# santi-pdp/segan_pytorch

Measured on AMD Instinct MI355X. Metric: 16384-sample waveform chunks/sec (GAN step), higher is better.
Workload: dtype f32

## Files before the change

include/segan_hip.h:

```cpp
#ifndef SEGAN_HIP_H
#define SEGAN_HIP_H

#include <stddef.h>
#include <stdint.h>

#ifdef __cplusplus
extern "C" {
#endif

#define SEGAN_ABI_VERSION 15

#define SEGAN_PAD_REFLECT 0
#define SEGAN_PAD_ZERO 1

#define SEGAN_ACT_NONE 0
#define SEGAN_ACT_TANH 1

typedef struct segan_src {
  const float* p0;
  const float* p1;
  int32_t C0;
  int32_t C1;
  const float* scale;
  const float* shift;
  const float* slope;
} segan_src;

int segan_abi_version(void);
const char* segan_last_error(void);

int segan_set_reserved_slots(int n);

size_t segan_packed_f_bytes(int M, int N, int S);
size_t segan_packed_t_bytes(int M, int N, int S);

int segan_pack_weights(const float* w, float* wf, float* wt, int M, int N, int K, int S,
                       int pad_t, void* stream);

#define SEGAN_PREC_FP32 0
#define SEGAN_PREC_BF16 1
#define SEGAN_PREC_BF16X3 3
#define SEGAN_PREC_FP32_BLOCKED 4
size_t segan_packed_bf_bytes(int M, int N, int S, int tform, int planes);
int segan_pack_weights_bf(const float* w, void* out, int M, int N, int K, int S, int tform,
                          int pad_t, int planes, void* stream);

size_t segan_bf16_scratch_bytes(int op, int B, int N, int M, int L, int K, int S, int pad, int planes);
size_t segan_corr_scratch_bytes(void);
void segan_debug_last_corr(int* out6);
void segan_debug_last_wgrad(int* out6);

int segan_conv1d_fwd(const segan_src* x, const void* wf, const float* bias, float* out, int B,
                     int N, int M, int L, int K, int S, int padL, int mode, int roll,
                     int precision, void* scratch, size_t scratch_bytes, void* stream);

int segan_conv1d_dgrad(const float* da, const void* wt, const float* w, float* dx, float* halo,
                       int B, int N, int M, int L, int K, int S, int padL, int roll, int precision,
                       void* scratch, size_t scratch_bytes, void* stream);

#define SEGAN_WGRAD_DETERMINISTIC 1
size_t segan_wgrad_scratch_bytes(int B, int M, int N, int Ls, int S, int precision, int flags);
int segan_wgrad(const segan_src* lo, const segan_src* hi, float* dw, int B, int M, int N, int Ls,
                int K, int S, int padL, int mode, int roll, int precision, int flags, void* scratch,
                size_t scratch_bytes, void* stream);

int segan_deconv1d_fwd(const segan_src* x, const void* wt, const float* w, const float* bias,
                       float* y, int B, int M, int N, int Ls, int K, int S, int pad, int act,
                       int precision, void* scratch, size_t scratch_bytes, void* stream);

int segan_deconv1d_dgrad(const float* dy, const void* wf, float* dx0, float* dx1, int B, int M,
                         int M0, int N, int Ls, int K, int S, int pad, int precision, void* scratch,
                         size_t scratch_bytes, void* stream);


int segan_bn_nsplit(int B, int C, int L);
int segan_bn_stats(const float* x, const float* gamma, const float* beta, float eps,
                   float momentum, float* running_mean, float* running_var, float* mean,
                   float* rstd, float* scale, float* shift, float* ws, int B, int C, int L,
                   void* stream);
int segan_bn_partial(const float* x, float* ws, int B, int C, int L, void* stream);
int segan_bn_final(const float* ws, int nsplit_total, const float* gamma, const float* beta,
                   float eps, float momentum, float* running_mean, float* running_var, float* mean,
                   float* rstd, float* scale, float* shift, int C, void* stream);

int segan_affine_tanh(const float* x, const float* scale, const float* shift, float* y, int B,
                      int C, int L, void* stream);
int segan_scale_mask(const float* x, const float* scale, const float* mask, float* y, int B, int C,
                     int L, void* stream);

int segan_affine_prelu(const float* x, const float* scale, const float* shift, const float* slope,
                       float* y, int B, int C, int L, void* stream);

int segan_sum_skip(const float* x0, const float* slope0, const float* x1, const float* alpha,
                   float* out, int B, int C, int L, void* stream);

int segan_act_bwd(const float* a, const float* dh, const float* dskip, const float* slope,
                  const float* alpha, const float* bn_mean, const float* bn_rstd,
                  const float* bn_gamma, const float* bn_beta, float* da, float* dslope,
                  float* dalpha, float* dgamma, float* dbeta, float* dbias, float* ws, int B, int C,
                  int L, void* stream);
int segan_act_bwd_bn_reduce(const float* a, const float* dh, const float* slope,
                            const float* bn_mean, const float* bn_rstd, const float* bn_gamma,
                            const float* bn_beta, float* dslope, float* dgamma, float* dbeta,
                            float* totals, float* ws, int B, int C, int L, void* stream);
int segan_act_bwd_bn_apply(const float* a, const float* dh, const float* slope,
                           const float* bn_mean, const float* bn_rstd, const float* bn_gamma,
                           const float* bn_beta, const float* totals, float* da, float* dbias,
                           float* ws, int B, int C, int L, double count_total, void* stream);

int segan_tanh_bwd(const float* y, const float* dy, const float* clean, float l1_scale, float* da,
                   float* dbias, float* ws, int B, int C, int L, void* stream);


#define SEGAN_GEMM_DETERMINISTIC 1
size_t segan_gemm_scratch_bytes(int M, int N, int K);
int segan_gemm(const float* A, int64_t sam, int64_t sak, const float* B, int64_t sbk, int64_t sbn,
               float* C, int64_t ldc, int M, int N, int K, int beta0, int flags, void* scratch,
               size_t scratch_bytes, void* stream);

int segan_bias_prelu_rows(const float* x, const float* bias, const float* slope, float* y,
                          int rows, int cols, void* stream);
int segan_bias_prelu_rows_bwd(const float* x, const float* bias, const float* slope,
                              const float* dy, float* dx, float* dslope, float* dbias, int rows,
                              int cols, void* stream);

int segan_mse_const(const float* x, float target, float* loss, float* grad, const float* gout,
                    float gscale, int n, void* stream);
int segan_bce_logits_const(const float* x, float target, float* loss, float* grad,
                           const float* gout, float gscale, int n, void* stream);
int segan_l1_mean(const float* x, const float* y, float* loss, float* ws, int64_t n,
                  void* stream);
int segan_l1_bwd(const float* x, const float* y, const float* gout, float gscale, float* grad,
                 int64_t n, void* stream);

size_t segan_packed_g_bytes(int M, int N, int S);
int segan_pack_weights_g(const float* w, float* wg, int M, int N, int K, int S, void* stream);
int segan_conv1d_dgrad_short(const float* da, const float* wg, float* dx, int B, int N, int M,
                             int L, int K, int S, int padL, int roll, void* stream);

int segan_pool_time_fwd(const float* x, float* y, int* idx, int rows, int L, int mode,
                        void* stream);
int segan_pool_time_bwd(const float* dy, const int* idx, float* dx, int rows, int L, int mode,
                        void* stream);

int segan_mse_mean(const float* x, const float* y, float* loss, float* ws, int64_t n,
                   void* stream);
int segan_mse_bwd(const float* x, const float* y, const float* gout, float gscale, float* grad,
                  int64_t n, void* stream);

size_t segan_snorm_ws_floats(int A, int Bd, int K, int dim);
int segan_snorm_fwd(const float* w, float* u, float* v, float* w_sn, float* sigma, float* ws, int A,
                    int Bd, int K, int dim, int power_iteration, float eps, void* stream);
int segan_snorm_bwd(const float* dw_sn, const float* w, const float* u, const float* v,
                    const float* sigma, float* dw, float* ws, int A, int Bd, int K, int dim,
                    void* stream);

int segan_stft_pitch(int n_fft);
int segan_stft_basis(float* basis, int n_fft, int win, void* stream);
int segan_stft_frames(const float* x, float* frames, int B, int T, int n_fft, int hop, int win,
                      void* stream);
int segan_powdb(const float* S, float* db, int64_t rows, int nbins, int pitch, float eps,
                void* stream);
int segan_powdb_bwd(const float* S, const float* ddb, float* dS, int64_t rows, int nbins, int pitch,
                    float eps, void* stream);
int segan_stft_overlap_add(const float* dframes, float* dx, int B, int T, int n_fft, int hop,
                           int win, void* stream);

int segan_pcm16_prep(const int16_t* pcm, const unsigned char* first, float* clean, float* noisy,
                     int B, int T, double coef, void* stream);

int segan_deemphasis(const float* y, float* x, int rows, int T, double coef, void* stream);
int segan_ssnr_frames(int T, int srate);
int segan_ssnr(const float* ref, const float* deg, float* seg, float* out, int rows, int T,
               int srate, double eps, void* stream);
int segan_wss(const float* ref, const float* deg, double* dist, int rows, int T, int srate,
              void* stream);
int segan_llr(const float* ref, const float* deg, double* dist, int rows, int T, int srate,
              void* stream);
int segan_stoi_plan(int srate, int* pq, int* ntaps, double* taps, int cap, int* bands);
int segan_stoi_dims(int T, int srate, int* dims);
int segan_stoi(const float* ref, const float* deg, const int* lengths, int rows, int T, int srate,
               double* xr, double* yr, double* energy, int* mask, int* kept, int* count,
               double* xs, double* ys, double* X, double* Y, double* rho, double* d, void* stream);

int segan_rmsprop_step(float* p, const float* g, float* sq, float lr, float alpha, float eps,
                       int64_t n, void* stream);
int segan_adam_step(float* p, const float* g, float* m, float* v, float lr, float beta1,
                    float beta2, float eps, int step, int64_t n, void* stream);
int segan_fill(float* p, float value, int64_t n, void* stream);
int segan_scale(float* p, float s, int64_t n, void* stream);

int segan_comm_id_bytes(void);
int segan_comm_unique_id(void* id_out);
int segan_comm_init(void** comm_out, int world, int rank, const void* id);
int segan_comm_destroy(void* comm);
int segan_comm_rank(void* comm);
int segan_comm_world(void* comm);
int segan_allreduce(void* comm, float* buf, size_t n, float scale, void* stream);
int segan_broadcast(void* comm, float* buf, size_t n, int root, void* stream);
int segan_allgather(void* comm, const float* send, float* recv, size_t n, void* stream);

#ifdef __cplusplus
}
#endif
#endif
```

segan_pytorch_amd/_lib.py:

```python
import ctypes
import os
from ctypes import POINTER, Structure, c_char_p, c_double, c_float, c_int, c_int32, c_int64, c_size_t, c_void_p

_HERE = os.path.dirname(os.path.abspath(__file__))
LIB_PATH = os.environ.get('SEGAN_HIP_LIB') or os.path.join(_HERE, 'libsegan_hip.so')

PAD_REFLECT = 0
PAD_ZERO = 1
ACT_NONE = 0
ACT_TANH = 1
ABI_VERSION = 15


class SeganSrc(Structure):
    _fields_ = [('p0', c_void_p), ('p1', c_void_p), ('C0', c_int32), ('C1', c_int32),
                ('scale', c_void_p), ('shift', c_void_p), ('slope', c_void_p)]


_P = c_void_p
_SRC = POINTER(SeganSrc)

SIGNATURES = {
    'segan_abi_version': (c_int, []),
    'segan_set_reserved_slots': (c_int, [c_int]),
    'segan_last_error': (c_char_p, []),
    'segan_packed_f_bytes': (c_size_t, [c_int, c_int, c_int]),
    'segan_packed_t_bytes': (c_size_t, [c_int, c_int, c_int]),
    'segan_pack_weights': (c_int, [_P, _P, _P, c_int, c_int, c_int, c_int, c_int, _P]),
    'segan_packed_bf_bytes': (c_size_t, [c_int, c_int, c_int, c_int, c_int]),
    'segan_pack_weights_bf': (c_int, [_P, _P, c_int, c_int, c_int, c_int, c_int, c_int, c_int, _P]),
    'segan_corr_scratch_bytes': (c_size_t, []),
    'segan_bf16_scratch_bytes': (c_size_t, [c_int] * 9),
    'segan_debug_last_corr': (None, [POINTER(c_int)]),
    'segan_debug_last_wgrad': (None, [POINTER(c_int)]),
    'segan_conv1d_fwd': (c_int, [_SRC, _P, _P, _P, c_int, c_int, c_int, c_int, c_int, c_int, c_int,
                                 c_int, c_int, c_int, _P, c_size_t, _P]),
    'segan_conv1d_dgrad': (c_int, [_P, _P, _P, _P, _P, c_int, c_int, c_int, c_int, c_int, c_int, c_int,
                                   c_int, c_int, _P, c_size_t, _P]),
    'segan_wgrad': (c_int, [_SRC, _SRC, _P, c_int, c_int, c_int, c_int, c_int, c_int, c_int, c_int,
                            c_int, c_int, c_int, _P, c_size_t, _P]),
    'segan_wgrad_scratch_bytes': (c_size_t, [c_int, c_int, c_int, c_int, c_int, c_int, c_int]),
    'segan_deconv1d_fwd': (c_int, [_SRC, _P, _P, _P, _P, c_int, c_int, c_int, c_int, c_int, c_int, c_int,
                                   c_int, c_int, _P, c_size_t, _P]),
    'segan_deconv1d_dgrad': (c_int, [_P, _P, _P, _P, c_int, c_int, c_int, c_int, c_int, c_int, c_int,
                                     c_int, c_int, _P, c_size_t, _P]),
    'segan_bn_nsplit': (c_int, [c_int, c_int, c_int]),
    'segan_bn_stats': (c_int, [_P, _P, _P, c_float, c_float, _P, _P, _P, _P, _P, _P, _P, c_int, c_int,
                               c_int, _P]),
    'segan_bn_partial': (c_int, [_P, _P, c_int, c_int, c_int, _P]),
    'segan_bn_final': (c_int, [_P, c_int, _P, _P, c_float, c_float, _P, _P, _P, _P, _P, _P, c_int, _P]),
    'segan_act_bwd_bn_reduce': (c_int, [_P] * 12 + [c_int, c_int, c_int, _P]),
    'segan_act_bwd_bn_apply': (c_int, [_P] * 11 + [c_int, c_int, c_int, c_double, _P]),
    'segan_affine_prelu': (c_int, [_P, _P, _P, _P, _P, c_int, c_int, c_int, _P]),
    'segan_affine_tanh': (c_int, [_P, _P, _P, _P, c_int, c_int, c_int, _P]),
    'segan_scale_mask': (c_int, [_P, _P, _P, _P, c_int, c_int, c_int, _P]),
    'segan_sum_skip': (c_int, [_P, _P, _P, _P, _P, c_int, c_int, c_int, _P]),
    'segan_bce_logits_const': (c_int, [_P, c_float, _P, _P, _P, c_float, c_int, _P]),
    'segan_act_bwd': (c_int, [_P] * 16 + [c_int, c_int, c_int, _P]),
    'segan_tanh_bwd': (c_int, [_P, _P, _P, c_float, _P, _P, _P, c_int, c_int, c_int, _P]),
    'segan_gemm_scratch_bytes': (c_size_t, [c_int, c_int, c_int]),
    'segan_gemm': (c_int, [_P, c_int64, c_int64, _P, c_int64, c_int64, _P, c_int64, c_int, c_int,
                           c_int, c_int, c_int, _P, c_size_t, _P]),
    'segan_bias_prelu_rows': (c_int, [_P, _P, _P, _P, c_int, c_int, _P]),
    'segan_bias_prelu_rows_bwd': (c_int, [_P, _P, _P, _P, _P, _P, _P, c_int, c_int, _P]),
    'segan_mse_const': (c_int, [_P, c_float, _P, _P, _P, c_float, c_int, _P]),
    'segan_l1_bwd': (c_int, [_P, _P, _P, c_float, _P, c_int64, _P]),
    'segan_l1_mean': (c_int, [_P, _P, _P, _P, c_int64, _P]),
    'segan_packed_g_bytes': (c_size_t, [c_int, c_int, c_int]),
    'segan_pack_weights_g': (c_int, [_P, _P, c_int, c_int, c_int, c_int, _P]),
    'segan_conv1d_dgrad_short': (c_int, [_P, _P, _P, c_int, c_int, c_int, c_int, c_int, c_int, c_int,
                                        c_int, _P]),
    'segan_pool_time_fwd': (c_int, [_P, _P, _P, c_int, c_int, c_int, _P]),
    'segan_pool_time_bwd': (c_int, [_P, _P, _P, c_int, c_int, c_int, _P]),
    'segan_mse_mean': (c_int, [_P, _P, _P, _P, c_int64, _P]),
    'segan_mse_bwd': (c_int, [_P, _P, _P, c_float, _P, c_int64, _P]),
    'segan_snorm_ws_floats': (c_size_t, [c_int, c_int, c_int, c_int]),
    'segan_snorm_fwd': (c_int, [_P, _P, _P, _P, _P, _P, c_int, c_int, c_int, c_int, c_int, c_float, _P]),
    'segan_snorm_bwd': (c_int, [_P, _P, _P, _P, _P, _P, _P, c_int, c_int, c_int, c_int, _P]),
    'segan_pcm16_prep': (c_int, [_P, _P, _P, _P, c_int, c_int, c_double, _P]),
    'segan_stft_basis': (c_int, [_P, c_int, c_int, _P]),
    'segan_stft_frames': (c_int, [_P, _P, c_int, c_int, c_int, c_int, c_int, _P]),
    'segan_stft_pitch': (c_int, [c_int]),
    'segan_powdb': (c_int, [_P, _P, c_int64, c_int, c_int, c_float, _P]),
    'segan_powdb_bwd': (c_int, [_P, _P, _P, c_int64, c_int, c_int, c_float, _P]),
    'segan_stft_overlap_add': (c_int, [_P, _P, c_int, c_int, c_int, c_int, c_int, _P]),
    'segan_deemphasis': (c_int, [_P, _P, c_int, c_int, c_double, _P]),
    'segan_ssnr_frames': (c_int, [c_int, c_int]),
    'segan_ssnr': (c_int, [_P, _P, _P, _P, c_int, c_int, c_int, c_double, _P]),
    'segan_wss': (c_int, [_P, _P, _P, c_int, c_int, c_int, _P]),
    'segan_llr': (c_int, [_P, _P, _P, c_int, c_int, c_int, _P]),
    'segan_stoi_plan': (c_int, [c_int, POINTER(c_int), POINTER(c_int), _P, c_int, POINTER(c_int)]),
    'segan_stoi_dims': (c_int, [c_int, c_int, POINTER(c_int)]),
    'segan_stoi': (c_int, [_P, _P, _P, c_int, c_int, c_int] + [_P] * 13),
    'segan_rmsprop_step': (c_int, [_P, _P, _P, c_float, c_float, c_float, c_int64, _P]),
    'segan_adam_step': (c_int, [_P, _P, _P, _P, c_float, c_float, c_float, c_float, c_int, c_int64,
                                _P]),
    'segan_fill': (c_int, [_P, c_float, c_int64, _P]),
    'segan_scale': (c_int, [_P, c_float, c_int64, _P]),
    'segan_comm_id_bytes': (c_int, []),
    'segan_comm_unique_id': (c_int, [_P]),
    'segan_comm_init': (c_int, [POINTER(c_void_p), c_int, c_int, _P]),
    'segan_comm_destroy': (c_int, [_P]),
    'segan_comm_rank': (c_int, [_P]),
    'segan_comm_world': (c_int, [_P]),
    'segan_allreduce': (c_int, [_P, _P, c_size_t, c_float, _P]),
    'segan_broadcast': (c_int, [_P, _P, c_size_t, c_int, _P]),
    'segan_allgather': (c_int, [_P, _P, _P, c_size_t, _P]),
}

_lib = None


def load():
    global _lib
    if _lib is not None:
        return _lib
    if not os.path.exists(LIB_PATH):
        raise RuntimeError(
            'segan_pytorch_amd: {} not found. Build it with `make` (or '
            '`python -c "import __graft_entry__ as g; g.build()"`) at the repo root. '
            'There is no non-HIP fallback.'.format(LIB_PATH))
    try:
        import torch
        if torch.cuda.is_available():
            torch.cuda.init()
    except ImportError:
        pass
    lib = ctypes.CDLL(LIB_PATH)
    for name, (res, args) in SIGNATURES.items():
        fn = getattr(lib, name)
        fn.restype = res
        fn.argtypes = args
    ver = lib.segan_abi_version()
    if ver != ABI_VERSION:
        raise RuntimeError('libsegan_hip ABI {} != expected {}'.format(ver, ABI_VERSION))
    _lib = lib
    return lib


def check(rc, what=''):
    if rc != 0:
        msg = load().segan_last_error()
        raise RuntimeError('libsegan_hip {} failed ({}): {}'.format(
            what, rc, msg.decode() if msg else '?'))
```

segan_pytorch_amd/csrc/segan_pack.hip:

```cpp
#include "segan_conv_shared.h"

__global__ __launch_bounds__(256) void pack_f_kernel(const float* __restrict__ w,
                                                     float* __restrict__ wf, int M, int N, int K,
                                                     int S, int U, int pitch, int rows, int pair) {
  __shared__ float t[64][33];
  const int n = blockIdx.y;
  const int m0 = blockIdx.x * 64;
  const int tid = threadIdx.x;
  {
    float v[8];
#pragma unroll
    for (int i = 0; i < 8; ++i) {
      const int e = tid + 256 * i;
      const int ml = e >> 5, k = e & 31;
      const int m = m0 + ml;
      v[i] = (m < M && n < N && k < K) ? w[((size_t)m * N + n) * K + k] : 0.0f;
    }
#pragma unroll
    for (int i = 0; i < 8; ++i) {
      const int e = tid + 256 * i;
      t[e >> 5][e & 31] = v[i];
    }
  }
  __syncthreads();
  if (pair && (n & 1) && n < N && tid < 64) {
    const int m = m0 + tid;
    t[tid][31] = m < M ? w[((size_t)m * N + n - 1) * K + (31 - S)] : 0.0f;
  }
  __syncthreads();
  for (int e = tid; e < 32 * 64; e += 256) {
    const int kk = e >> 6, ml = e & 63;
    const int r = kk / U, u = kk - r * U;
    const int row = (n * S + r) * U + u;
    if (row < rows && m0 + ml < pitch) wf[(size_t)row * pitch + m0 + ml] = t[ml][S * u + r];
  }
}

__global__ __launch_bounds__(256) void pack_t_kernel(const float* __restrict__ w,
                                                     float* __restrict__ wt, int M, int N, int K,
                                                     int S, int U, int NP, int pad, int pitch,
                                                     int rows) {
  __shared__ float t[64][33];
  const int m = blockIdx.y;
  const int n0 = blockIdx.x * 64;
  const int tid = threadIdx.x;
  {
    float v[8];
#pragma unroll
    for (int i = 0; i < 8; ++i) {
      const int e = tid + 256 * i;
      const int nl = e >> 5, k = e & 31;
      const int n = n0 + nl;
      v[i] = (m < M && n < N && k < K) ? w[((size_t)m * N + n) * K + k] : 0.0f;
    }
#pragma unroll
    for (int i = 0; i < 8; ++i) {
      const int e = tid + 256 * i;
      t[e >> 5][e & 31] = v[i];
    }
  }
  __syncthreads();
  for (int e = tid; e < 32 * 64; e += 256) {
    const int kk = e >> 6, nl = e & 63;
    const int up = kk / S, r = kk - up * S;
    const int rho = (r + pad) % S;
    const int k = S * (U - 1 - up) + rho;
    const int row = m * U + up;
    const int n = n0 + nl;
    if (row < rows && n < NP) wt[(size_t)row * pitch + r * NP + n] = t[nl][k];
  }
}

extern "C" size_t segan_packed_f_bytes(int M, int N, int S) {
  if (!stride_ok(S) || M <= 0 || N <= 0) return 0;
  return (size_t)f_rows(N) * f_pitch(M) * sizeof(float);
}
extern "C" size_t segan_packed_t_bytes(int M, int N, int S) {
  if (!stride_ok(S) || M <= 0 || N <= 0) return 0;
  return (size_t)t_rows(M, S) * t_pitch(N, S) * sizeof(float);
}

extern "C" int segan_pack_weights(const float* w, float* wf, float* wt, int M, int N, int K, int S,
                                  int pad_t, void* stream) {
  SEGAN_REQUIRE(w != nullptr, "pack_weights: w is NULL");
  SEGAN_REQUIRE(stride_ok(S), "pack_weights: stride %d not in {1,2,4}", S);
  SEGAN_REQUIRE(K >= 1 && K <= 32, "pack_weights: kernel width %d not in [1,32]", K);
  SEGAN_REQUIRE(M > 0 && N > 0, "pack_weights: bad channel counts %d,%d", M, N);
  SEGAN_REQUIRE(pad_t >= 0, "pack_weights: negative padding");
  hipStream_t st = (hipStream_t)stream;
  const int U = 32 / S;
  if (wf) {
    const int pitch = f_pitch(M), rows = f_rows(N);
    hipLaunchKernelGGL(pack_f_kernel, dim3(pitch / 64, ceil_div(rows, 32)), dim3(256), 0, st, w,
                       wf, M, N, K, S, U, pitch, rows, f_pair(N, K));
  }
  if (wt) {
    const int NP = t_np(N, S);
    const int pitch = t_pitch(N, S), rows = t_rows(M, S);
    hipLaunchKernelGGL(pack_t_kernel, dim3(ceil_div(NP, 64), ceil_div(rows, U)), dim3(256), 0, st,
                       w, wt, M, N, K, S, U, NP, pad_t, pitch, rows);
  }
  return segan_check_launch("pack_weights");
}
```

segan_pytorch_amd/csrc/segan_pointwise.hip:

```cpp
#include "segan_common.h"

#define PW_THREADS 256

static int pw_nsplit(int B, int C, int L) {
  int ns = ceil_div(2048, C);
  if (ns > B) ns = B;
  long per = (long)B * L / ns;
  while (ns > 1 && per < 2048) {
    ns = (ns + 1) / 2;
    per = (long)B * L / ns;
  }
  return ns < 1 ? 1 : ns;
}

extern "C" int segan_bn_nsplit(int B, int C, int L) {
  if (B <= 0 || C <= 0 || L <= 0) return 0;
  return pw_nsplit(B, C, L);
}

template <int NV>
__device__ __forceinline__ void block_sum(float (&v)[NV], float* sm) {
  const int lane = threadIdx.x & 63, wave = threadIdx.x >> 6;
#pragma unroll
  for (int k = 0; k < NV; ++k) v[k] = warp_sum(v[k]);
  if (lane == 0)
#pragma unroll
    for (int k = 0; k < NV; ++k) sm[wave * NV + k] = v[k];
  __syncthreads();
  if (threadIdx.x == 0) {
#pragma unroll
    for (int k = 0; k < NV; ++k) {
      float s = 0.f;
      for (int w = 0; w < PW_THREADS / 64; ++w) s += sm[w * NV + k];
      v[k] = s;
    }
  }
  __syncthreads();
}

struct ChanRange {
  int c, b_beg, b_end;
};
__device__ __forceinline__ ChanRange chan_range(int B, int nsplit) {
  ChanRange r;
  r.c = blockIdx.x;
  const int per = (B + nsplit - 1) / nsplit;
  r.b_beg = blockIdx.y * per;
  r.b_end = min(B, r.b_beg + per);
  return r;
}

__device__ __forceinline__ void chan_combine(float& n, float& mean, float& m2, float nb, float mb,
                                             float qb) {
  const float tot = n + nb;
  if (tot <= 0.0f) return;
  const float d = mb - mean;
  const float f = nb / tot;
  mean = fmaf(d, f, mean);
  m2 = m2 + qb + d * d * n * f;
  n = tot;
}

__global__ void bn_partial_kernel(const float* __restrict__ x, float* __restrict__ ws, int B, int C,
                                  int L, int nsplit) {
  __shared__ float sm[3 * (PW_THREADS / 64)];
  const ChanRange cr = chan_range(B, nsplit);
  const int nb = cr.b_end - cr.b_beg;
  const float* base = x + ((size_t)cr.b_beg * C + cr.c) * L;
  const size_t sstride = (size_t)C * L;
  const bool vec = (L & 3) == 0 && ((uintptr_t)x & 15) == 0;
  const int Lv = vec ? L >> 2 : L;
  int tr = PW_THREADS;
  while (tr > Lv && tr > 1) tr >>= 1;
  const int rp = PW_THREADS / tr;
  const int t0 = threadIdx.x % tr, r0 = threadIdx.x / tr;
  float K = 0.0f, s1 = 0.0f, s2 = 0.0f, n = 0.0f;
  if (r0 < nb && t0 < Lv) K = base[(size_t)r0 * sstride + (vec ? 4 * t0 : t0)];
  for (int b = r0; b < nb; b += rp) {
    const float* row = base + b * sstride;
    if (vec) {
      for (int t = t0; t < Lv; t += tr) {
        const f32x4 u = *reinterpret_cast<const f32x4*>(row + 4 * t);
#pragma unroll
        for (int e = 0; e < 4; ++e) {
          const float d = u[e] - K;
          s1 += d;
          s2 = fmaf(d, d, s2);
        }
        n += 4.0f;
      }
    } else {
      for (int t = t0; t < Lv; t += tr) {
        const float d = row[t] - K;
        s1 += d;
        s2 = fmaf(d, d, s2);
        n += 1.0f;
      }
    }
  }
  float mean = 0.0f, m2 = 0.0f;
  if (n > 0.0f) {
    const float r = s1 / n;
    mean = K + r;
    m2 = fmaxf(s2 - s1 * r, 0.0f);
  }
#pragma unroll
  for (int o = 32; o > 0; o >>= 1) {
    const float nb2 = __shfl_down(n, o, 64), mb2 = __shfl_down(mean, o, 64), qb2 = __shfl_down(m2, o, 64);
    chan_combine(n, mean, m2, nb2, mb2, qb2);
  }
  const int lane = threadIdx.x & 63, wave = threadIdx.x >> 6;
  if (lane == 0) {
    sm[3 * wave] = n; sm[3 * wave + 1] = mean; sm[3 * wave + 2] = m2;
  }
  __syncthreads();
  if (threadIdx.x == 0) {
    for (int w = 1; w < PW_THREADS / 64; ++w) chan_combine(n, mean, m2, sm[3 * w], sm[3 * w + 1], sm[3 * w + 2]);
    float* w = ws + ((size_t)blockIdx.y * C + cr.c) * 3;
    w[0] = n;
    w[1] = mean;
    w[2] = m2;
  }
}

__device__ __forceinline__ void bn_affine(float gamma, float beta, float mean, float rstd,
                                          float& scale, float& shift) {
  scale = gamma * rstd;
  shift = fmaf(-mean, scale, beta);
}

__global__ void bn_final_kernel(const float* __restrict__ ws, const float* gamma, const float* beta,
                                float eps, float momentum, float* running_mean, float* running_var,
                                float* mean_o, float* rstd_o, float* scale_o, float* shift_o, int C,
                                int nsplit) {
  const int c = blockIdx.x * blockDim.x + threadIdx.x;
  if (c >= C) return;
  double n = 0.0, mean = 0.0, m2 = 0.0;
  for (int s = 0; s < nsplit; ++s) {
    const float* w = ws + ((size_t)s * C + c) * 3;
    const double nb = w[0], mb = w[1], qb = w[2];
    if (nb <= 0.0) continue;
    const double tot = n + nb;
    const double d = mb - mean;
    mean += d * nb / tot;
    m2 += qb + d * d * n * nb / tot;
    n = tot;
  }
  const double var = n > 0 ? m2 / n : 0.0;
  const float rstd = (float)(1.0 / sqrt(var + (double)eps));
  const float g = gamma ? gamma[c] : 1.0f;
  const float bt = beta ? beta[c] : 0.0f;
  float sc, sh;
  bn_affine(g, bt, (float)mean, rstd, sc, sh);
  if (mean_o) mean_o[c] = (float)mean;
  if (rstd_o) rstd_o[c] = rstd;
  if (scale_o) scale_o[c] = sc;
  if (shift_o) shift_o[c] = sh;
  if (running_mean) running_mean[c] = (1.0f - momentum) * running_mean[c] + momentum * (float)mean;
  if (running_var) {
    const double unb = n > 1 ? m2 / (n - 1.0) : var;
    running_var[c] = (1.0f - momentum) * running_var[c] + momentum * (float)unb;
  }
}

extern "C" int segan_bn_stats(const float* x, const float* gamma, const float* beta, float eps,
                              float momentum, float* running_mean, float* running_var, float* mean,
                              float* rstd, float* scale, float* shift, float* ws, int B, int C,
                              int L, void* stream) {
  SEGAN_REQUIRE(x && ws, "bn_stats: NULL pointer");
  SEGAN_REQUIRE(B > 0 && C > 0 && L > 0, "bn_stats: bad sizes");
  hipStream_t st = (hipStream_t)stream;
  const int ns = pw_nsplit(B, C, L);
  hipLaunchKernelGGL(bn_partial_kernel, dim3(C, ns), dim3(PW_THREADS), 0, st, x, ws, B, C, L, ns);
  hipLaunchKernelGGL(bn_final_kernel, dim3(ceil_div(C, 64)), dim3(64), 0, st, ws, gamma, beta, eps,
                     momentum, running_mean, running_var, mean, rstd, scale, shift, C, ns);
  return segan_check_launch("bn_stats");
}

extern "C" int segan_bn_partial(const float* x, float* ws, int B, int C, int L, void* stream) {
  SEGAN_REQUIRE(x && ws, "bn_partial: NULL pointer");
  SEGAN_REQUIRE(B > 0 && C > 0 && L > 0, "bn_partial: bad sizes");
  const int ns = pw_nsplit(B, C, L);
  hipLaunchKernelGGL(bn_partial_kernel, dim3(C, ns), dim3(PW_THREADS), 0, (hipStream_t)stream, x, ws,
                     B, C, L, ns);
  return segan_check_launch("bn_partial");
}

extern "C" int segan_bn_final(const float* ws, int nsplit_total, const float* gamma,
                              const float* beta, float eps, float momentum, float* running_mean,
                              float* running_var, float* mean, float* rstd, float* scale,
                              float* shift, int C, void* stream) {
  SEGAN_REQUIRE(ws && nsplit_total > 0 && C > 0, "bn_final: bad arguments");
  hipLaunchKernelGGL(bn_final_kernel, dim3(ceil_div(C, 64)), dim3(64), 0, (hipStream_t)stream, ws,
                     gamma, beta, eps, momentum, running_mean, running_var, mean, rstd, scale, shift,
                     C, nsplit_total);
  return segan_check_launch("bn_final");
}

__global__ void affine_prelu_kernel(const float* __restrict__ x, const float* scale,
                                    const float* shift, const float* slope, float* __restrict__ y,
                                    size_t total, int C, int L) {
  for (size_t i = blockIdx.x * (size_t)blockDim.x + threadIdx.x; i < total;
       i += (size_t)gridDim.x * blockDim.x) {
    const int c = (int)((i / L) % C);
    float v = x[i];
    v = fmaf(v, scale ? scale[c] : 1.0f, shift ? shift[c] : 0.0f);
    if (slope) v = v > 0.f ? v : v * slope[c];
    y[i] = v;
  }
}

extern "C" int segan_affine_prelu(const float* x, const float* scale, const float* shift,
                                  const float* slope, float* y, int B, int C, int L, void* stream) {
  SEGAN_REQUIRE(x && y, "affine_prelu: NULL pointer");
  SEGAN_REQUIRE(B > 0 && C > 0 && L > 0, "affine_prelu: bad sizes");
  const size_t total = (size_t)B * C * L;
  const int blocks = (int)((total + 255) / 256 > 4096 ? 4096 : (total + 255) / 256);
  hipLaunchKernelGGL(affine_prelu_kernel, dim3(blocks), dim3(256), 0, (hipStream_t)stream, x, scale,
                     shift, slope, y, total, C, L);
  return segan_check_launch("affine_prelu");
}

__global__ void affine_tanh_kernel(const float* __restrict__ x, const float* scale,
                                   const float* shift, float* __restrict__ y, size_t total, int C,
                                   int L) {
  for (size_t i = blockIdx.x * (size_t)blockDim.x + threadIdx.x; i < total;
       i += (size_t)gridDim.x * blockDim.x) {
    const int c = (int)((i / L) % C);
    y[i] = tanhf(fmaf(x[i], scale ? scale[c] : 1.0f, shift ? shift[c] : 0.0f));
  }
}

extern "C" int segan_affine_tanh(const float* x, const float* scale, const float* shift, float* y,
                                 int B, int C, int L, void* stream) {
  SEGAN_REQUIRE(x && y, "affine_tanh: NULL pointer");
  SEGAN_REQUIRE(B > 0 && C > 0 && L > 0, "affine_tanh: bad sizes");
  const size_t total = (size_t)B * C * L;
  const int blocks = (int)((total + 255) / 256 > 4096 ? 4096 : (total + 255) / 256);
  hipLaunchKernelGGL(affine_tanh_kernel, dim3(blocks), dim3(256), 0, (hipStream_t)stream, x, scale,
                     shift, y, total, C, L);
  return segan_check_launch("affine_tanh");
}

__global__ void scale_mask_kernel(const float* __restrict__ x, const float* scale,
                                  const float* __restrict__ mask, float* __restrict__ y,
                                  size_t total, int C, int L) {
  for (size_t i = blockIdx.x * (size_t)blockDim.x + threadIdx.x; i < total;
       i += (size_t)gridDim.x * blockDim.x) {
    const int c = (int)((i / L) % C);
    y[i] = x[i] * (scale ? scale[c] : 1.0f) * mask[i];
  }
}

extern "C" int segan_scale_mask(const float* x, const float* scale, const float* mask, float* y,
                                int B, int C, int L, void* stream) {
  SEGAN_REQUIRE(x && mask && y, "scale_mask: NULL pointer");
  SEGAN_REQUIRE(B > 0 && C > 0 && L > 0, "scale_mask: bad sizes");
  const size_t total = (size_t)B * C * L;
  const int blocks = (int)((total + 255) / 256 > 4096 ? 4096 : (total + 255) / 256);
  hipLaunchKernelGGL(scale_mask_kernel, dim3(blocks), dim3(256), 0, (hipStream_t)stream, x, scale,
                     mask, y, total, C, L);
  return segan_check_launch("scale_mask");
}

__global__ void sum_skip_kernel(const float* __restrict__ x0, const float* slope0,
                                const float* __restrict__ x1, const float* alpha,
                                float* __restrict__ out, size_t total, int C, int L) {
  for (size_t i = blockIdx.x * (size_t)blockDim.x + threadIdx.x; i < total;
       i += (size_t)gridDim.x * blockDim.x) {
    const int c = (int)((i / L) % C);
    float v = x0[i];
    if (slope0) v = v > 0.f ? v : v * slope0[c];
    out[i] = fmaf(alpha[c], x1[i], v);
  }
}

extern "C" int segan_sum_skip(const float* x0, const float* slope0, const float* x1,
                              const float* alpha, float* out, int B, int C, int L, void* stream) {
  SEGAN_REQUIRE(x0 && x1 && alpha && out, "sum_skip: NULL pointer");
  SEGAN_REQUIRE(B > 0 && C > 0 && L > 0, "sum_skip: bad sizes");
  const size_t total = (size_t)B * C * L;
  const int blocks = (int)((total + 255) / 256 > 4096 ? 4096 : (total + 255) / 256);
  hipLaunchKernelGGL(sum_skip_kernel, dim3(blocks), dim3(256), 0, (hipStream_t)stream, x0, slope0,
                     x1, alpha, out, total, C, L);
  return segan_check_launch("sum_skip");
}

struct ActBwdArgs {
  const float* a;
  const float* dh;
  const float* dskip;
  const float* slope;
  const float* alpha;
  const float* mean;
  const float* rstd;
  const float* gamma;
  const float* beta;
  float* da;
  float* ws;
  int B, C, L, nsplit;
  float inv_count;
};

template <int PHASE>
__global__ void act_bwd_kernel(const ActBwdArgs p) {
  __shared__ float sm[16];
  const ChanRange cr = chan_range(p.B, p.nsplit);
  const int c = cr.c;
  const int nb = cr.b_end - cr.b_beg;
  const float sl = p.slope ? p.slope[c] : 1.0f;
  const float al = p.alpha ? p.alpha[c] : 0.0f;
  float mu = 0.f, rs = 1.f, ga = 1.f, be = 0.f, dbeta_m = 0.f, dgamma_m = 0.f, sc = 1.f, sh = 0.f;
  if (PHASE != 0) {
    mu = p.mean[c];
    rs = p.rstd[c];
    ga = p.gamma ? p.gamma[c] : 1.0f;
    be = p.beta ? p.beta[c] : 0.0f;
    bn_affine(ga, be, mu, rs, sc, sh);
  }
  if (PHASE == 2) {
    const float* tot = p.ws + (size_t)p.nsplit * p.C * 4 + (size_t)c * 2;
    dbeta_m = tot[0] * p.inv_count;
    dgamma_m = tot[1] * p.inv_count;
  }
  float r[3] = {0.f, 0.f, 0.f};
  const bool has_skip = p.dskip != nullptr;
  auto elem = [&](float av, float dh, float ds) -> float {
    if (PHASE == 0) {
      float g = dh * (av > 0.f ? 1.0f : sl);
      r[0] += dh * (av > 0.f ? 0.0f : av);
      if (has_skip) {
        g = fmaf(al, ds, g);
        r[1] = fmaf(ds, av, r[1]);
      }
      r[2] += g;
      return g;
    }
    const float xh = (av - mu) * rs;
    const float v = fmaf(av, sc, sh);
    const float g = dh * (v > 0.f ? 1.0f : sl);
    if (PHASE == 1) {
      r[0] += dh * (v > 0.f ? 0.0f : v);
      r[1] += g;
      r[2] = fmaf(g, xh, r[2]);
      return 0.0f;
    }
    const float d = ga * rs * (g - dbeta_m - xh * dgamma_m);
    r[0] += d;
    return d;
  };
  const size_t base = ((size_t)cr.b_beg * p.C + c) * p.L;
  const size_t sstride = (size_t)p.C * p.L;
  const bool vec = (p.L & 3) == 0 &&
                   (((uintptr_t)p.a | (uintptr_t)p.dh | (uintptr_t)p.dskip | (uintptr_t)p.da) & 15) == 0;
  const int Lv = vec ? p.L >> 2 : p.L;
  int tr = PW_THREADS;
  while (tr > Lv && tr > 1) tr >>= 1;
  const int rp = PW_THREADS / tr;
  const int t0 = threadIdx.x % tr, r0 = threadIdx.x / tr;
  const f32x4 z4 = {0.f, 0.f, 0.f, 0.f};
  for (int b = r0; b < nb; b += rp) {
    const size_t ro = base + b * sstride;
    if (vec) {
      for (int t = t0; t < Lv; t += tr) {
        const size_t i = ro + 4 * (size_t)t;
        const f32x4 av = *reinterpret_cast<const f32x4*>(p.a + i);
        const f32x4 dh = p.dh ? *reinterpret_cast<const f32x4*>(p.dh + i) : z4;
        const f32x4 ds = has_skip ? *reinterpret_cast<const f32x4*>(p.dskip + i) : z4;
        f32x4 o;
#pragma unroll
        for (int e = 0; e < 4; ++e) o[e] = elem(av[e], dh[e], ds[e]);
        if (PHASE != 1) *reinterpret_cast<f32x4*>(p.da + i) = o;
      }
    } else {
      for (int t = t0; t < Lv; t += tr) {
        const size_t i = ro + t;
        const float o = elem(p.a[i], p.dh ? p.dh[i] : 0.0f, has_skip ? p.dskip[i] : 0.0f);
        if (PHASE != 1) p.da[i] = o;
      }
    }
  }
  block_sum<3>(r, sm);
  if (threadIdx.x == 0) {
    float* w = p.ws + ((size_t)blockIdx.y * p.C + c) * 4;
    w[0] = r[0];
    w[1] = r[1];
    w[2] = r[2];
  }
}

template <int PHASE>
__global__ void act_bwd_final_kernel(const ActBwdArgs p, float* dslope, float* dalpha,
                                     float* dgamma, float* dbeta, float* dbias) {
  const int c = blockIdx.x * blockDim.x + threadIdx.x;
  if (c >= p.C) return;
  float s0 = 0.f, s1 = 0.f, s2 = 0.f;
  for (int s = 0; s < p.nsplit; ++s) {
    const float* w = p.ws + ((size_t)s * p.C + c) * 4;
    s0 += w[0];
    s1 += w[1];
    s2 += w[2];
  }
  if (PHASE == 0) {
    if (dslope) dslope[c] += s0;
    if (dalpha) dalpha[c] += s1;
    if (dbias) dbias[c] += s2;
  } else if (PHASE == 1) {
    if (dslope) dslope[c] += s0;
    if (dbeta) dbeta[c] += s1;
    if (dgamma) dgamma[c] += s2;
    float* tot = p.ws + (size_t)p.nsplit * p.C * 4 + (size_t)c * 2;
    tot[0] = s1;
    tot[1] = s2;
  } else {
    if (dbias) dbias[c] += s0;
  }
}

extern "C" int segan_act_bwd(const float* a, const float* dh, const float* dskip,
                             const float* slope, const float* alpha, const float* bn_mean,
                             const float* bn_rstd, const float* bn_gamma, const float* bn_beta,
                             float* da, float* dslope, float* dalpha, float* dgamma, float* dbeta,
                             float* dbias, float* ws, int B, int C, int L, void* stream) {
  SEGAN_REQUIRE(a && da && ws, "act_bwd: NULL pointer");
  SEGAN_REQUIRE(dh || dskip, "act_bwd: no incoming gradient");
  SEGAN_REQUIRE(B > 0 && C > 0 && L > 0, "act_bwd: bad sizes");
  SEGAN_REQUIRE((bn_mean == nullptr) == (bn_rstd == nullptr), "act_bwd: mean/rstd must pair");
  SEGAN_REQUIRE(!(dskip && !alpha), "act_bwd: dskip needs alpha");
  SEGAN_REQUIRE(!(bn_mean && dskip), "act_bwd: BN layers have no skip tap");
  hipStream_t st = (hipStream_t)stream;
  ActBwdArgs p;
  p.a = a; p.dh = dh; p.dskip = dskip; p.slope = slope; p.alpha = alpha;
  p.mean = bn_mean; p.rstd = bn_rstd; p.gamma = bn_gamma; p.beta = bn_beta;
  p.da = da; p.ws = ws; p.B = B; p.C = C; p.L = L;
  p.nsplit = pw_nsplit(B, C, L);
  p.inv_count = 1.0f / ((float)B * (float)L);
  const dim3 grid(C, p.nsplit), fgrid(ceil_div(C, 64));
  if (!bn_mean) {
    hipLaunchKernelGGL(act_bwd_kernel<0>, grid, dim3(PW_THREADS), 0, st, p);
    hipLaunchKernelGGL(act_bwd_final_kernel<0>, fgrid, dim3(64), 0, st, p, dslope, dalpha, dgamma,
                       dbeta, dbias);
  } else {
    hipLaunchKernelGGL(act_bwd_kernel<1>, grid, dim3(PW_THREADS), 0, st, p);
    hipLaunchKernelGGL(act_bwd_final_kernel<1>, fgrid, dim3(64), 0, st, p, dslope, dalpha, dgamma,
                       dbeta, dbias);
    hipLaunchKernelGGL(act_bwd_kernel<2>, grid, dim3(PW_THREADS), 0, st, p);
    hipLaunchKernelGGL(act_bwd_final_kernel<2>, fgrid, dim3(64), 0, st, p, dslope, dalpha, dgamma,
                       dbeta, dbias);
  }
  return segan_check_launch("act_bwd");
}

extern "C" int segan_act_bwd_bn_reduce(const float* a, const float* dh, const float* slope,
                                       const float* bn_mean, const float* bn_rstd,
                                       const float* bn_gamma, const float* bn_beta, float* dslope,
                                       float* dgamma, float* dbeta, float* totals, float* ws, int B,
                                       int C, int L, void* stream) {
  SEGAN_REQUIRE(a && dh && bn_mean && bn_rstd && totals && ws, "act_bwd_bn_reduce: NULL pointer");
  SEGAN_REQUIRE(B > 0 && C > 0 && L > 0, "act_bwd_bn_reduce: bad sizes");
  hipStream_t st = (hipStream_t)stream;
  ActBwdArgs p;
  p.a = a; p.dh = dh; p.dskip = nullptr; p.slope = slope; p.alpha = nullptr;
  p.mean = bn_mean; p.rstd = bn_rstd; p.gamma = bn_gamma; p.beta = bn_beta;
  p.da = nullptr; p.ws = ws; p.B = B; p.C = C; p.L = L;
  p.nsplit = pw_nsplit(B, C, L);
  p.inv_count = 1.0f / ((float)B * (float)L);
  hipLaunchKernelGGL(act_bwd_kernel<1>, dim3(C, p.nsplit), dim3(PW_THREADS), 0, st, p);
  hipLaunchKernelGGL(act_bwd_final_kernel<1>, dim3(ceil_div(C, 64)), dim3(64), 0, st, p, dslope,
                     (float*)nullptr, dgamma, dbeta, (float*)nullptr);
  if (hipMemcpyAsync(totals, ws + (size_t)p.nsplit * C * 4, (size_t)C * 2 * sizeof(float),
                     hipMemcpyDeviceToDevice, st) != hipSuccess) {
    segan_set_error("act_bwd_bn_reduce: copy of the totals failed");
    return SEGAN_ELAUNCH;
  }
  return segan_check_launch("act_bwd_bn_reduce");
}

extern "C" int segan_act_bwd_bn_apply(const float* a, const float* dh, const float* slope,
                                      const float* bn_mean, const float* bn_rstd,
                                      const float* bn_gamma, const float* bn_beta,
                                      const float* totals, float* da, float* dbias, float* ws, int B,
                                      int C, int L, double count_total, void* stream) {
  SEGAN_REQUIRE(a && dh && bn_mean && bn_rstd && totals && da && ws, "act_bwd_bn_apply: NULL pointer");
  SEGAN_REQUIRE(B > 0 && C > 0 && L > 0 && count_total >= (double)B * L, "act_bwd_bn_apply: bad sizes");
  hipStream_t st = (hipStream_t)stream;
  ActBwdArgs p;
  p.a = a; p.dh = dh; p.dskip = nullptr; p.slope = slope; p.alpha = nullptr;
  p.mean = bn_mean; p.rstd = bn_rstd; p.gamma = bn_gamma; p.beta = bn_beta;
  p.da = da; p.ws = ws; p.B = B; p.C = C; p.L = L;
  p.nsplit = pw_nsplit(B, C, L);
  p.inv_count = (float)(1.0 / count_total);
  if (hipMemcpyAsync(ws + (size_t)p.nsplit * C * 4, totals, (size_t)C * 2 * sizeof(float),
                     hipMemcpyDeviceToDevice, st) != hipSuccess) {
    segan_set_error("act_bwd_bn_apply: copy of the totals failed");
    return SEGAN_ELAUNCH;
  }
  hipLaunchKernelGGL(act_bwd_kernel<2>, dim3(C, p.nsplit), dim3(PW_THREADS), 0, st, p);
  hipLaunchKernelGGL(act_bwd_final_kernel<2>, dim3(ceil_div(C, 64)), dim3(64), 0, st, p,
                     (float*)nullptr, (float*)nullptr, (float*)nullptr, (float*)nullptr, dbias);
  return segan_check_launch("act_bwd_bn_apply");
}

__global__ void tanh_bwd_kernel(const float* __restrict__ y, const float* dy, const float* clean,
                                float l1_scale, float* __restrict__ da, float* ws, int B, int C,
                                int L, int nsplit) {
  __shared__ float sm[16];
  const ChanRange cr = chan_range(B, nsplit);
  const int nb = cr.b_end - cr.b_beg;
  const long cnt = (long)(nb > 0 ? nb : 0) * L;
  float r[1] = {0.f};
  for (long e = threadIdx.x; e < cnt; e += PW_THREADS) {
    const int b = cr.b_beg + (int)(e / L);
    const int t = (int)(e % L);
    const size_t i = ((size_t)b * C + cr.c) * L + t;
    const float yv = y[i];
    float g = dy ? dy[i] : 0.0f;
    if (clean) {
      const float d = yv - clean[i];
      g += l1_scale * (d > 0.f ? 1.0f : (d < 0.f ? -1.0f : 0.0f));
    }
    const float d = g * (1.0f - yv * yv);
    da[i] = d;
    r[0] += d;
  }
  block_sum<1>(r, sm);
  if (threadIdx.x == 0) ws[(size_t)blockIdx.y * C + cr.c] = r[0];
}

__global__ void sum_splits_add_kernel(const float* ws, float* out, int C, int nsplit) {
  const int c = blockIdx.x * blockDim.x + threadIdx.x;
  if (c >= C) return;
  float s = 0.f;
  for (int k = 0; k < nsplit; ++k) s += ws[(size_t)k * C + c];
  out[c] += s;
}

extern "C" int segan_tanh_bwd(const float* y, const float* dy, const float* clean, float l1_scale,
                              float* da, float* dbias, float* ws, int B, int C, int L,
                              void* stream) {
  SEGAN_REQUIRE(y && da && ws, "tanh_bwd: NULL pointer");
  SEGAN_REQUIRE(dy || clean, "tanh_bwd: no incoming gradient");
  SEGAN_REQUIRE(B > 0 && C > 0 && L > 0, "tanh_bwd: bad sizes");
  hipStream_t st = (hipStream_t)stream;
  const int ns = pw_nsplit(B, C, L);
  hipLaunchKernelGGL(tanh_bwd_kernel, dim3(C, ns), dim3(PW_THREADS), 0, st, y, dy, clean, l1_scale,
                     da, ws, B, C, L, ns);
  if (dbias)
    hipLaunchKernelGGL(sum_splits_add_kernel, dim3(ceil_div(C, 64)), dim3(64), 0, st, ws, dbias, C,
                       ns);
  return segan_check_launch("tanh_bwd");
}

__global__ void bias_prelu_rows_kernel(const float* __restrict__ x, const float* bias,
                                       const float* slope, float* __restrict__ y, int rows,
                                       int cols) {
  const size_t total = (size_t)rows * cols;
  for (size_t i = blockIdx.x * (size_t)blockDim.x + threadIdx.x; i < total;
       i += (size_t)gridDim.x * blockDim.x) {
    const int c = (int)(i % cols);
    float v = x[i] + (bias ? bias[c] : 0.0f);
    if (slope) v = v > 0.f ? v : v * slope[c];
    y[i] = v;
  }
}

extern "C" int segan_bias_prelu_rows(const float* x, const float* bias, const float* slope,
                                     float* y, int rows, int cols, void* stream) {
  SEGAN_REQUIRE(x && y && rows > 0 && cols > 0, "bias_prelu_rows: bad arguments");
  const size_t total = (size_t)rows * cols;
  const int blocks = (int)((total + 255) / 256 > 2048 ? 2048 : (total + 255) / 256);
  hipLaunchKernelGGL(bias_prelu_rows_kernel, dim3(blocks), dim3(256), 0, (hipStream_t)stream, x,
                     bias, slope, y, rows, cols);
  return segan_check_launch("bias_prelu_rows");
}

__global__ __launch_bounds__(256) void bias_prelu_rows_bwd_kernel(
    const float* __restrict__ x, const float* bias, const float* slope,
    const float* __restrict__ dy, float* __restrict__ dx, float* dslope, float* dbias, int rows,
    int cols) {
  __shared__ float sm[2][4][64];
  const int cl = threadIdx.x & 63, rg = threadIdx.x >> 6;
  const int c = blockIdx.x * 64 + cl;
  float s_sl = 0.f, s_b = 0.f;
  if (c < cols) {
    const float bs = bias ? bias[c] : 0.0f;
    const float sl = slope ? slope[c] : 1.0f;
    for (int r = rg; r < rows; r += 4) {
      const size_t i = (size_t)r * cols + c;
      const float v = x[i] + bs;
      const float g = dy[i];
      const float d = g * (v > 0.f ? 1.0f : sl);
      s_sl += g * (v > 0.f ? 0.0f : v);
      s_b += d;
      dx[i] = d;
    }
  }
  sm[0][rg][cl] = s_sl;
  sm[1][rg][cl] = s_b;
  __syncthreads();
  if (rg == 0 && c < cols) {
    const float a = sm[0][0][cl] + sm[0][1][cl] + sm[0][2][cl] + sm[0][3][cl];
    const float b = sm[1][0][cl] + sm[1][1][cl] + sm[1][2][cl] + sm[1][3][cl];
    if (dslope && slope) dslope[c] += a;
    if (dbias) dbias[c] += b;
  }
}

extern "C" int segan_bias_prelu_rows_bwd(const float* x, const float* bias, const float* slope,
                                         const float* dy, float* dx, float* dslope, float* dbias,
                                         int rows, int cols, void* stream) {
  SEGAN_REQUIRE(x && dy && dx && rows > 0 && cols > 0, "bias_prelu_rows_bwd: bad arguments");
  hipLaunchKernelGGL(bias_prelu_rows_bwd_kernel, dim3(ceil_div(cols, 64)), dim3(256), 0,
                     (hipStream_t)stream, x, bias, slope, dy, dx, dslope, dbias, rows, cols);
  return segan_check_launch("bias_prelu_rows_bwd");
}

__global__ void mse_const_kernel(const float* __restrict__ x, float target, float* loss,
                                 float* grad, const float* gout, float gscale, int n) {
  __shared__ float sm[16];
  float r[1] = {0.f};
  const float inv = 1.0f / (float)n;
  if (gout) gscale *= gout[0];
  for (int i = threadIdx.x; i < n; i += PW_THREADS) {
    const float d = x[i] - target;
    r[0] = fmaf(d, d, r[0]);
    if (grad) grad[i] = 2.0f * d * inv * gscale;
  }
  block_sum<1>(r, sm);
  if (threadIdx.x == 0 && loss) loss[0] = r[0] * inv;
}

extern "C" int segan_mse_const(const float* x, float target, float* loss, float* grad,
                               const float* gout, float gscale, int n, void* stream) {
  SEGAN_REQUIRE(x && n > 0 && (loss || grad), "mse_const: bad arguments");
  hipLaunchKernelGGL(mse_const_kernel, dim3(1), dim3(PW_THREADS), 0, (hipStream_t)stream, x, target,
                     loss, grad, gout, gscale, n);
  return segan_check_launch("mse_const");
}

__global__ void bce_const_kernel(const float* __restrict__ x, float target, float* loss,
                                 float* grad, const float* gout, float gscale, int n) {
  __shared__ float sm[16];
  float r[1] = {0.f};
  const float inv = 1.0f / (float)n;
  if (gout) gscale *= gout[0];
  for (int i = threadIdx.x; i < n; i += PW_THREADS) {
    const float v = x[i];
    r[0] += fmaxf(v, 0.f) - v * target + log1pf(expf(-fabsf(v)));
    if (grad) grad[i] = (1.0f / (1.0f + expf(-v)) - target) * inv * gscale;
  }
  block_sum<1>(r, sm);
  if (threadIdx.x == 0 && loss) loss[0] = r[0] * inv;
}

extern "C" int segan_bce_logits_const(const float* x, float target, float* loss, float* grad,
                                      const float* gout, float gscale, int n, void* stream) {
  SEGAN_REQUIRE(x && n > 0 && (loss || grad), "bce_logits_const: bad arguments");
  hipLaunchKernelGGL(bce_const_kernel, dim3(1), dim3(PW_THREADS), 0, (hipStream_t)stream, x, target,
                     loss, grad, gout, gscale, n);
  return segan_check_launch("bce_logits_const");
}

template <bool SQ>
__global__ void l1_partial_kernel(const float* __restrict__ x, const float* __restrict__ y,
                                  float* ws, size_t n) {
  __shared__ float sm[16];
  float r[1] = {0.f};
  for (size_t i = blockIdx.x * (size_t)blockDim.x + threadIdx.x; i < n;
       i += (size_t)gridDim.x * blockDim.x) {
    const float d = x[i] - y[i];
    r[0] += SQ ? d * d : fabsf(d);
  }
  block_sum<1>(r, sm);
  if (threadIdx.x == 0) ws[blockIdx.x] = r[0];
}
__global__ void l1_final_kernel(const float* ws, float* loss, int nblocks, float inv) {
  __shared__ float sm[16];
  float r[1] = {0.f};
  for (int i = threadIdx.x; i < nblocks; i += PW_THREADS) r[0] += ws[i];
  block_sum<1>(r, sm);
  if (threadIdx.x == 0) loss[0] = r[0] * inv;
}

extern "C" int segan_l1_mean(const float* x, const float* y, float* loss, float* ws, int64_t n,
                             void* stream) {
  SEGAN_REQUIRE(x && y && loss && ws && n > 0, "l1_mean: bad arguments");
  hipStream_t st = (hipStream_t)stream;
  int blocks = (int)((n + 255) / 256 > 1024 ? 1024 : (n + 255) / 256);
  hipLaunchKernelGGL(l1_partial_kernel<false>, dim3(blocks), dim3(PW_THREADS), 0, st, x, y, ws, (size_t)n);
  hipLaunchKernelGGL(l1_final_kernel, dim3(1), dim3(PW_THREADS), 0, st, ws, loss, blocks,
                     1.0f / (float)n);
  return segan_check_launch("l1_mean");
}

extern "C" int segan_mse_mean(const float* x, const float* y, float* loss, float* ws, int64_t n,
                              void* stream) {
  SEGAN_REQUIRE(x && y && loss && ws && n > 0, "mse_mean: bad arguments");
  hipStream_t st = (hipStream_t)stream;
  int blocks = (int)((n + 255) / 256 > 1024 ? 1024 : (n + 255) / 256);
  hipLaunchKernelGGL(l1_partial_kernel<true>, dim3(blocks), dim3(PW_THREADS), 0, st, x, y, ws, (size_t)n);
  hipLaunchKernelGGL(l1_final_kernel, dim3(1), dim3(PW_THREADS), 0, st, ws, loss, blocks,
                     1.0f / (float)n);
  return segan_check_launch("mse_mean");
}

__global__ void mse_bwd_kernel(const float* __restrict__ x, const float* __restrict__ y,
                               const float* gout, float gscale, float* __restrict__ grad, size_t n) {
  const float g = 2.0f * gscale * (gout ? gout[0] : 1.0f) / (float)n;
  for (size_t i = blockIdx.x * (size_t)blockDim.x + threadIdx.x; i < n;
       i += (size_t)gridDim.x * blockDim.x)
    grad[i] = g * (x[i] - y[i]);
}

extern "C" int segan_mse_bwd(const float* x, const float* y, const float* gout, float gscale,
                             float* grad, int64_t n, void* stream) {
  SEGAN_REQUIRE(x && y && grad && n > 0, "mse_bwd: bad arguments");
  int blocks = (int)((n + 255) / 256 > 4096 ? 4096 : (n + 255) / 256);
  hipLaunchKernelGGL(mse_bwd_kernel, dim3(blocks), dim3(256), 0, (hipStream_t)stream, x, y, gout,
                     gscale, grad, (size_t)n);
  return segan_check_launch("mse_bwd");
}

__global__ void l1_bwd_kernel(const float* __restrict__ x, const float* __restrict__ y,
                              const float* gout, float gscale, float* __restrict__ grad, size_t n) {
  const float g = gscale * (gout ? gout[0] : 1.0f) / (float)n;
  for (size_t i = blockIdx.x * (size_t)blockDim.x + threadIdx.x; i < n;
       i += (size_t)gridDim.x * blockDim.x) {
    const float d = x[i] - y[i];
    grad[i] = d > 0.f ? g : (d < 0.f ? -g : 0.0f);
  }
}

extern "C" int segan_l1_bwd(const float* x, const float* y, const float* gout, float gscale,
                            float* grad, int64_t n, void* stream) {
  SEGAN_REQUIRE(x && y && grad && n > 0, "l1_bwd: bad arguments");
  int blocks = (int)((n + 255) / 256 > 4096 ? 4096 : (n + 255) / 256);
  hipLaunchKernelGGL(l1_bwd_kernel, dim3(blocks), dim3(256), 0, (hipStream_t)stream, x, y, gout,
                     gscale, grad, (size_t)n);
  return segan_check_launch("l1_bwd");
}

__global__ void rmsprop_kernel(float* __restrict__ p, const float* __restrict__ g,
                               float* __restrict__ sq, float lr, float alpha, float eps, size_t n) {
  const size_t n4 = n / 4;
  float4* p4 = reinterpret_cast<float4*>(p);
  const float4* g4 = reinterpret_cast<const float4*>(g);
  float4* s4 = reinterpret_cast<float4*>(sq);
  const float oma = 1.0f - alpha;
  for (size_t i = blockIdx.x * (size_t)blockDim.x + threadIdx.x; i < n4;
       i += (size_t)gridDim.x * blockDim.x) {
    float4 pv = p4[i], gv = g4[i], sv = s4[i];
#define RMS1(f)                                       \
  sv.f = alpha * sv.f + oma * gv.f * gv.f;            \
  pv.f = pv.f - lr * (gv.f / (sqrtf(sv.f) + eps));
    RMS1(x) RMS1(y) RMS1(z) RMS1(w)
#undef RMS1
    p4[i] = pv;
    s4[i] = sv;
  }
  if (blockIdx.x == 0 && threadIdx.x < (n & 3)) {
    const size_t i = n4 * 4 + threadIdx.x;
    const float gv = g[i];
    const float sv = alpha * sq[i] + oma * gv * gv;
    sq[i] = sv;
    p[i] = p[i] - lr * (gv / (sqrtf(sv) + eps));
  }
}

extern "C" int segan_rmsprop_step(float* p, const float* g, float* sq, float lr, float alpha,
                                  float eps, int64_t n, void* stream) {
  SEGAN_REQUIRE(p && g && sq && n > 0, "rmsprop_step: bad arguments");
  SEGAN_REQUIRE(((uintptr_t)p % 16 == 0) && ((uintptr_t)g % 16 == 0) && ((uintptr_t)sq % 16 == 0),
                "rmsprop_step: arenas must be 16-byte aligned");
  int blocks = (int)((n / 4 + 255) / 256 > 2048 ? 2048 : (n / 4 + 255) / 256);
  if (blocks < 1) blocks = 1;
  hipLaunchKernelGGL(rmsprop_kernel, dim3(blocks), dim3(256), 0, (hipStream_t)stream, p, g, sq, lr,
                     alpha, eps, (size_t)n);
  return segan_check_launch("rmsprop_step");
}

__global__ void adam_kernel(float* __restrict__ p, const float* __restrict__ g,
                            float* __restrict__ m, float* __restrict__ v, float step_size,
                            float beta1, float beta2, float eps, float inv_sqrt_bc2, size_t n) {
  for (size_t i = blockIdx.x * (size_t)blockDim.x + threadIdx.x; i < n;
       i += (size_t)gridDim.x * blockDim.x) {
    const float gv = g[i];
    const float mv = m[i] + (gv - m[i]) * (1.0f - beta1);
    const float vv = beta2 * v[i] + (1.0f - beta2) * gv * gv;
    m[i] = mv;
    v[i] = vv;
    const float denom = sqrtf(vv) * inv_sqrt_bc2 + eps;
    p[i] = p[i] - step_size * (mv / denom);
  }
}

extern "C" int segan_adam_step(float* p, const float* g, float* m, float* v, float lr, float beta1,
                               float beta2, float eps, int step, int64_t n, void* stream) {
  SEGAN_REQUIRE(p && g && m && v && n > 0 && step >= 1, "adam_step: bad arguments");
  const double bc1 = 1.0 - pow((double)beta1, (double)step);
  const double bc2 = 1.0 - pow((double)beta2, (double)step);
  const float step_size = (float)((double)lr / bc1);
  const float inv_sqrt_bc2 = (float)(1.0 / sqrt(bc2));
  int blocks = (int)((n + 255) / 256 > 4096 ? 4096 : (n + 255) / 256);
  hipLaunchKernelGGL(adam_kernel, dim3(blocks), dim3(256), 0, (hipStream_t)stream, p, g, m, v,
                     step_size, beta1, beta2, eps, inv_sqrt_bc2, (size_t)n);
  return segan_check_launch("adam_step");
}

template <int MODE>
__global__ void pool_time_kernel(const float* __restrict__ x, float* __restrict__ y,
                                 int* __restrict__ idx, int rows, int L) {
  const int lane = threadIdx.x & 63;
  const int row = blockIdx.x * (blockDim.x >> 6) + (threadIdx.x >> 6);
  if (row >= rows) return;
  const float* xr = x + (size_t)row * L;
  if (MODE == 0) {
    float best = -INFINITY;
    int bi = 0x7fffffff;
    for (int t = lane; t < L; t += 64) {
      const float v = xr[t];
      if (v > best || bi == 0x7fffffff) { best = v; bi = t; }
    }
#pragma unroll
    for (int o = 32; o > 0; o >>= 1) {
      const float ov = __shfl_xor(best, o);
      const int oi = __shfl_xor(bi, o);
      if (oi != 0x7fffffff && (bi == 0x7fffffff || ov > best || (ov == best && oi < bi))) {
        best = ov;
        bi = oi;
      }
    }
    if (lane == 0) {
      y[row] = best;
      idx[row] = bi;
    }
  } else {
    float s = 0.0f;
    for (int t = lane; t < L; t += 64) s += xr[t];
#pragma unroll
    for (int o = 32; o > 0; o >>= 1) s += __shfl_xor(s, o);
    if (lane == 0) y[row] = s / (float)L;
  }
}

template <int MODE>
__global__ void pool_time_bwd_kernel(const float* __restrict__ dy, const int* __restrict__ idx,
                                     float* __restrict__ dx, int rows, int L) {
  const size_t n = (size_t)rows * L;
  const float invL = 1.0f / (float)L;
  for (size_t i = blockIdx.x * (size_t)blockDim.x + threadIdx.x; i < n;
       i += (size_t)gridDim.x * blockDim.x) {
    const int row = (int)(i / L);
    const int t = (int)(i - (size_t)row * L);
    dx[i] = MODE == 0 ? (t == idx[row] ? dy[row] : 0.0f) : dy[row] * invL;
  }
}

extern "C" int segan_pool_time_fwd(const float* x, float* y, int* idx, int rows, int L, int mode,
                                   void* stream) {
  SEGAN_REQUIRE(x && y && rows > 0 && L > 0, "pool_time_fwd: bad arguments");
  SEGAN_REQUIRE(mode == 0 || mode == 1, "pool_time_fwd: mode must be 0 (max) or 1 (mean)");
  SEGAN_REQUIRE(mode == 1 || idx, "pool_time_fwd: max pooling needs idx");
  const dim3 grid(ceil_div(rows, 4));
  if (mode == 0)
    hipLaunchKernelGGL(pool_time_kernel<0>, grid, dim3(256), 0, (hipStream_t)stream, x, y, idx,
                       rows, L);
  else
    hipLaunchKernelGGL(pool_time_kernel<1>, grid, dim3(256), 0, (hipStream_t)stream, x, y, idx,
                       rows, L);
  return segan_check_launch("pool_time_fwd");
}

extern "C" int segan_pool_time_bwd(const float* dy, const int* idx, float* dx, int rows, int L,
                                   int mode, void* stream) {
  SEGAN_REQUIRE(dy && dx && rows > 0 && L > 0, "pool_time_bwd: bad arguments");
  SEGAN_REQUIRE(mode == 0 || mode == 1, "pool_time_bwd: mode must be 0 (max) or 1 (mean)");
  SEGAN_REQUIRE(mode == 1 || idx, "pool_time_bwd: max pooling needs idx");
  const size_t n = (size_t)rows * L;
  const int blocks = (int)((n + 255) / 256 > 4096 ? 4096 : (n + 255) / 256);
  if (mode == 0)
    hipLaunchKernelGGL(pool_time_bwd_kernel<0>, dim3(blocks), dim3(256), 0, (hipStream_t)stream,
                       dy, idx, dx, rows, L);
  else
    hipLaunchKernelGGL(pool_time_bwd_kernel<1>, dim3(blocks), dim3(256), 0, (hipStream_t)stream,
                       dy, idx, dx, rows, L);
  return segan_check_launch("pool_time_bwd");
}

__global__ void fill_kernel(float* p, float value, size_t n) {
  for (size_t i = blockIdx.x * (size_t)blockDim.x + threadIdx.x; i < n;
       i += (size_t)gridDim.x * blockDim.x)
    p[i] = value;
}
__global__ void scale_kernel(float* p, float s, size_t n) {
  for (size_t i = blockIdx.x * (size_t)blockDim.x + threadIdx.x; i < n;
       i += (size_t)gridDim.x * blockDim.x)
    p[i] *= s;
}
extern "C" int segan_fill(float* p, float value, int64_t n, void* stream) {
  SEGAN_REQUIRE(p && n > 0, "fill: bad arguments");
  int blocks = (int)((n + 255) / 256 > 4096 ? 4096 : (n + 255) / 256);
  hipLaunchKernelGGL(fill_kernel, dim3(blocks), dim3(256), 0, (hipStream_t)stream, p, value,
                     (size_t)n);
  return segan_check_launch("fill");
}
extern "C" int segan_scale(float* p, float s, int64_t n, void* stream) {
  SEGAN_REQUIRE(p && n > 0, "scale: bad arguments");
  int blocks = (int)((n + 255) / 256 > 4096 ? 4096 : (n + 255) / 256);
  hipLaunchKernelGGL(scale_kernel, dim3(blocks), dim3(256), 0, (hipStream_t)stream, p, s,
                     (size_t)n);
  return segan_check_launch("scale");
}
```

segan_pytorch_amd/functional.py:

```python
import os

import torch

from . import ops
from .ops import ACT_NONE, ACT_TANH, PAD_REFLECT, PAD_ZERO, Src


def grad_buf(p):
    if p.grad is None:
        p.grad = torch.zeros_like(p, memory_format=torch.contiguous_format)
    elif not p.grad.is_contiguous():
        p.grad = p.grad.contiguous()
    return p.grad


def _gb(p, needed=True):
    if p is None or not needed or not p.requires_grad:
        return None
    return grad_buf(p)


def _bn_batch_stats(bn, training):
    return training or bn.running_mean is None or bn.running_var is None


def _bn_train_stats(c, bn, training=True):
    from . import distributed as sdist
    fn = sdist.bn_stats_sync if sdist.sync_bn_enabled() else ops.bn_stats
    track = training and bn.running_mean is not None and bn.running_var is not None
    momentum = 0.0
    if track:
        if bn.num_batches_tracked is not None:
            bn.num_batches_tracked += 1
        if bn.momentum is not None:
            momentum = bn.momentum
        else:
            momentum = 1.0 / float(bn.num_batches_tracked) if bn.num_batches_tracked is not None else 0.0
    return fn(c, bn.weight, bn.bias, bn.eps, momentum, bn.running_mean if track else None,
              bn.running_var if track else None)


def _bn_eval_affine(bn):
    rstd = torch.rsqrt(bn.running_var + bn.eps)
    gamma = bn.weight.detach() if bn.weight is not None else torch.ones_like(rstd)
    beta = bn.bias.detach() if bn.bias is not None else torch.zeros_like(rstd)
    scale = (gamma * rstd).contiguous()
    shift = (beta - bn.running_mean * scale).contiguous()
    return scale, shift, rstd.contiguous()


def _eval_bn_act_bwd(c, bn, scale, shift, rstd, dh, slope, dslope, y_tanh=None, dbias=None):
    if y_tanh is not None:
        g = ops.tanh_bwd(y_tanh, dh, dbias=_gb(bn.bias))
    else:
        v = ops.affine_prelu(c, scale, shift, None)
        g = ops.act_bwd(v, dh, slope=slope, dslope=dslope, dbias=_gb(bn.bias))
    if bn.weight is not None and bn.weight.requires_grad:
        xhat = ops.affine_prelu(c, rstd, (-bn.running_mean * rstd).contiguous(), None)
        grad_buf(bn.weight).add_((g * xhat).sum((0, 2)))
    dc = ops.affine_prelu(g, scale, None, None)
    if dbias is not None:
        ops.act_bwd(dc, dc, dbias=dbias)
    return dc


def _act_bwd_bn(a, dh, slope, bn, dslope, dgamma, dbeta, dbias):
    from . import distributed as sdist
    if sdist.sync_bn_enabled():
        return sdist.act_bwd_bn_sync(a, dh, slope, bn, dslope, dgamma, dbeta, dbias)
    return ops.act_bwd(a, dh, slope=slope, bn=bn, dslope=dslope, dgamma=dgamma, dbeta=dbeta,
                       dbias=dbias)


_WGRAD_OVERLAP = os.environ.get('SEGAN_WGRAD_OVERLAP', '0') == '1'
_side_streams = {}


class _SideStream(object):

    def __init__(self, *tensors):
        flat = []
        for t in tensors:
            if isinstance(t, Src):
                flat.extend((t.t0, t.t1, t.scale, t.shift, t.slope))
            else:
                flat.append(t)
        self.tensors = [t for t in flat if torch.is_tensor(t) and t.is_cuda]
        self.on = _WGRAD_OVERLAP and bool(self.tensors)

    def __enter__(self):
        if not self.on:
            return self
        dev = self.tensors[0].device
        main = torch.cuda.current_stream(dev)
        key = (dev.index, main.cuda_stream)
        side = _side_streams.get(key)
        if side is None:
            side = _side_streams[key] = torch.cuda.Stream(device=dev)
        side.wait_stream(main)
        self.side = side
        self.ctx = torch.cuda.stream(side)
        self.ctx.__enter__()
        return self

    def __exit__(self, *exc):
        if not self.on:
            return False
        self.ctx.__exit__(*exc)
        for t in self.tensors:
            t.record_stream(self.side)
        return False


def _join_side(ref):
    if not _WGRAD_OVERLAP or ref is None or not ref.is_cuda:
        return
    main = torch.cuda.current_stream(ref.device)
    side = _side_streams.get((ref.device.index, main.cuda_stream))
    if side is not None:
        main.wait_stream(side)


def _ready(*mods_or_params):
    from . import distributed as sdist
    if sdist._active is None:
        return
    ps = []
    for m in mods_or_params:
        if m is None:
            continue
        if isinstance(m, torch.nn.Module):
            ps.extend(torch.nn.Module.parameters(m))
        else:
            ps.append(m)
    sdist.grad_ready(*ps)


def _ones(n, ref):
    return torch.ones(n, device=ref.device, dtype=torch.float32)


def _cat(a, b):
    return torch.cat((a.detach().reshape(-1), b.detach().reshape(-1)))


import itertools as _it

_sn_epoch = _it.count(1 << 40)


def _is_sn(mod):
    return hasattr(mod, 'weight_orig')


class _Weights(object):

    def __init__(self):
        self._sn = {}

    def get(self, mod):
        if not _is_sn(mod):
            return mod.weight
        st = self._sn.get(id(mod))
        if st is None:
            dim = 1 if isinstance(mod, torch.nn.ConvTranspose1d) else 0
            w_sn, sigma = ops.snorm_fwd(mod.weight_orig.detach(), mod.weight_u, mod.weight_v, dim,
                                        mod.training)
            w_sn._segan_epoch = next(_sn_epoch)
            st = (w_sn, mod.weight_u.clone(), mod.weight_v.clone(), sigma, dim)
            self._sn[id(mod)] = st
        return st[0]

    @staticmethod
    def param(mod):
        return mod.weight_orig if _is_sn(mod) else mod.weight

    def needs_grad(self, mod):
        return self.param(mod).requires_grad

    def grad_target(self, mod):
        if not _is_sn(mod):
            return grad_buf(mod.weight)
        return torch.zeros_like(self._sn[id(mod)][0])

    def finish(self, mod, tmp):
        if not _is_sn(mod):
            return
        w_sn, u, v, sigma, dim = self._sn[id(mod)]
        ops.snorm_bwd(tmp, mod.weight_orig.detach(), u, v, sigma, dim, grad_buf(mod.weight_orig))


def _skip_conv_bwd(gskip, dsk, src_j, W):
    mod = gskip.skip_k
    kw = mod.kernel_size[0]
    w = W.get(mod)
    if mod.bias is not None and mod.bias.requires_grad:
        ops.act_bwd(dsk, dsk, dbias=grad_buf(mod.bias))
    if W.needs_grad(mod):
        gw = W.grad_target(mod)
        ops.wgrad(Src(dsk), src_j, gw, kw, 1, kw // 2, PAD_ZERO)
        W.finish(mod, gw)
    key = (w.data_ptr(), w._version, ops._weights_epoch, getattr(w, '_segan_epoch', 0))
    cached = gskip.__dict__.get('_wt_cache')
    if cached is None or cached[0] != key:
        wt = w.detach().transpose(0, 1).flip(2).contiguous()
        wt._segan_epoch = next(_sn_epoch)
        cached = (key, wt)
        gskip.__dict__['_wt_cache'] = cached
    return ops.conv1d_fwd(Src(dsk), cached[1], None, 1, pad_mode=PAD_ZERO, padL=kw - 1 - kw // 2,
                          pack=gskip._pack_t)


def _block_norm(blk, c, training):
    bn = getattr(blk, 'norm', None)
    if bn is None:
        return None, None, None
    if _bn_batch_stats(bn, training):
        mean, rstd, scale, shift = _bn_train_stats(c, bn, training)
        return scale, shift, (mean, rstd, bn.weight, bn.bias)
    scale, shift, _rstd = _bn_eval_affine(bn)
    return scale, shift, 'eval'


def _vec2(v0, n0, v1, n1, fill, ref):
    if v0 is None and v1 is None:
        return None
    parts = []
    for v, n in ((v0, n0), (v1, n1)):
        parts.append(v.detach().reshape(-1) if v is not None else
                     torch.full((n,), fill, device=ref.device, dtype=torch.float32))
    return torch.cat(parts)


def _dropout_mask(shape, p, device):
    noise = torch.nn.functional.dropout(torch.ones(shape), p, True)
    return noise.to(device)


class GeneratorFn(torch.autograd.Function):

    @staticmethod
    def forward(ctx, gen, want_hid, x, z, *params):
        x = x.contiguous()
        enc, dec = list(gen.enc_blocks), list(gen.dec_blocks)
        n_enc = len(enc)
        training = gen.training
        a_enc, src_enc, xf_enc, bn_enc = [], [], [], []
        src = Src(x)
        W = _Weights()
        for blk in enc:
            a = ops.conv1d_fwd(src, W.get(blk.conv), blk.conv.bias, blk.stride, pack=blk._pack)
            sc, sh, bnsv = _block_norm(blk, a, training)
            src_enc.append(src)
            a_enc.append(a)
            xf_enc.append((sc, sh))
            bn_enc.append(bnsv)
            src = Src(a, scale=sc, shift=sh, slope=blk.act.weight)
        last = a_enc[-1]
        s_last = enc[-1].act.weight
        sc_l, sh_l = xf_enc[-1]
        if not gen.no_z:
            z = z.contiguous()
            nz, nl = z.shape[1], last.shape[1]
            src = Src(z, last, scale=_vec2(None, nz, sc_l, nl, 1.0, z),
                      shift=_vec2(None, nz, sh_l, nl, 0.0, z), slope=_cat(_ones(nz, z), s_last))
        else:
            src = Src(last, scale=sc_l, shift=sh_l, slope=s_last)
        a_dec, src_dec, xf_dec, bn_dec = [], [], [], []
        skip_saved = {}
        enc_idx = n_enc - 1
        for li, blk in enumerate(dec):
            is_conv = hasattr(blk, 'conv')
            if li > 0:
                prev = a_dec[-1]
                s_prev = dec[li - 1].act.weight
                sc_p, sh_p = xf_dec[-1]
                np_ = prev.shape[1]
                if gen.skip and enc_idx in gen.skips and gen.dec_poolings[li] > 1:
                    gskip = gen.skips[enc_idx]['alpha']
                    aj = a_enc[enc_idx]
                    sc_j, sh_j = xf_enc[enc_idx]
                    nj = aj.shape[1]
                    ones_j = _ones(nj, aj)
                    drop_p = gskip.skip_dropout.p if (training and hasattr(gskip, 'skip_dropout')) \
                        else 0.0
                    a_norm = None
                    if gskip.skip_type == 'conv':
                        kw = gskip.skip_k.kernel_size[0]
                        sk = ops.conv1d_fwd(Src(aj, scale=sc_j, shift=sh_j), W.get(gskip.skip_k),
                                            gskip.skip_k.bias, 1, pad_mode=PAD_ZERO, padL=kw // 2,
                                            pack=gskip._pack)
                        scale_j = ones_j
                    else:
                        if sc_j is not None:
                            a_norm = ops.affine_prelu(aj, sc_j, sh_j, None)
                        sk = aj if a_norm is None else a_norm
                        scale_j = gskip.skip_k
                    mask = None
                    if drop_p > 0:
                        mask = _dropout_mask(tuple(sk.shape), drop_p, sk.device)
                        fold = None if gskip.skip_type == 'conv' else \
                            scale_j.detach().reshape(-1).contiguous()
                        sk = ops.scale_mask(sk, fold, mask)
                        scale_j = ones_j
                    skip_saved[enc_idx] = (mask, a_norm)
                    if gskip.merge_mode == 'concat':
                        src = Src(prev, sk,
                                  scale=_cat(sc_p if sc_p is not None else _ones(np_, prev), scale_j),
                                  shift=_vec2(sh_p, np_, None, nj, 0.0, prev),
                                  slope=_cat(s_prev, ones_j))
                    else:
                        hp, sl0 = prev, s_prev
                        if sc_p is not None:
                            hp, sl0 = ops.affine_prelu(prev, sc_p, sh_p, s_prev), None
                        src = Src(ops.sum_skip(hp, sl0, sk, scale_j.detach().reshape(-1)))
                        src.sum_of = True
                else:
                    src = Src(prev, scale=sc_p, shift=sh_p, slope=s_prev)
            has_bn = getattr(blk, 'norm', None) is not None
            if is_conv:
                a = ops.conv1d_fwd(src, W.get(blk.conv), blk.conv.bias, blk.stride,
                                   pack=blk._pack)
            else:
                act = ACT_TANH if (blk.is_tanh and not has_bn) else ACT_NONE
                a = ops.deconv1d_fwd(src, W.get(blk.deconv), blk.deconv.bias, blk.stride, act,
                                     pack=blk._pack)
            sc, sh, bnsv = _block_norm(blk, a, training)
            src_dec.append(src)
            a_dec.append(a)
            xf_dec.append((sc, sh))
            bn_dec.append(bnsv)
            enc_idx -= 1
        lastb = dec[-1]
        last_conv = hasattr(lastb, 'conv')
        sc, sh = xf_dec[-1]
        if last_conv:
            y = ops.affine_prelu(a_dec[-1], sc, sh, lastb.act.weight)
        elif bn_dec[-1] is not None:
            y = ops.affine_tanh(a_dec[-1], sc, sh) if lastb.is_tanh else \
                ops.affine_prelu(a_dec[-1], sc, sh, lastb.act.weight)
        else:
            y = a_dec[-1]
        keep_last = y is not a_dec[-1]
        ctx.gen = gen
        ctx.set_materialize_grads(False)
        ctx.x_needs = x.requires_grad
        ctx.save_for_backward(y)
        ctx.keep_last = keep_last
        ctx.state = (x, z, a_enc, src_enc, xf_enc, bn_enc, a_dec if keep_last else a_dec[:-1],
                     src_dec, bn_dec, skip_saved, W)
        hid = None
        if want_hid:
            hid = {}
            for i, blk in enumerate(enc):
                hid['enc_{}'.format(i)] = ops.affine_prelu(a_enc[i], xf_enc[i][0], xf_enc[i][1],
                                                           blk.act.weight)
            if not gen.no_z:
                hid['enc_zc'] = torch.cat((z, hid['enc_{}'.format(n_enc - 1)]), dim=1)
            for i, blk in enumerate(dec):
                if i == len(dec) - 1:
                    hid['dec_{}'.format(i)] = y
                else:
                    hid['dec_{}'.format(i)] = ops.affine_prelu(a_dec[i], xf_dec[i][0],
                                                               xf_dec[i][1], blk.act.weight)
        ctx.mark_non_differentiable(*([] if hid is None else list(hid.values())))
        if hid is None:
            return y
        return (y,) + tuple(hid.values())

    @staticmethod
    def backward(ctx, dy, *unused):
        gen = ctx.gen
        x, z, a_enc, src_enc, xf_enc, bn_enc, a_dec, src_dec, bn_dec, skip_saved, W = ctx.state
        y = ctx.saved_tensors[0]
        a_dec = list(a_dec) if ctx.keep_last else list(a_dec) + [y]
        enc, dec = list(gen.enc_blocks), list(gen.dec_blocks)
        n_enc, n_dec = len(enc), len(dec)
        if dy is None:
            ctx.state = None
            return (None,) * len(ctx.needs_input_grad)
        if 'eval' in bn_enc or 'eval' in bn_dec:
            raise RuntimeError('Generator backward in eval() mode with BatchNorm is not supported; '
                               'call .train()')
        dy = dy.contiguous()
        dh = dy
        dskip = {}
        dh_last_enc = None
        da = None
        for li in range(n_dec - 1, -1, -1):
            blk = dec[li]
            is_conv = hasattr(blk, 'conv')
            mod = blk.conv if is_conv else blk.deconv
            w = W.get(mod)
            K, S = blk.kwidth, blk.stride
            bnsv = bn_dec[li]
            bnm = getattr(blk, 'norm', None)
            if not is_conv and blk.is_tanh:
                if bnsv is None:
                    da = ops.tanh_bwd(a_dec[li], dy, dbias=_gb(mod.bias))
                else:
                    da = _act_bwd_bn(a_dec[li], ops.tanh_bwd(y, dy), None, bnsv, None,
                                     _gb(bnm.weight), _gb(bnm.bias), _gb(mod.bias))
            elif bnsv is None:
                da = ops.act_bwd(a_dec[li], dh, slope=blk.act.weight,
                                 dslope=_gb(blk.act.weight), dbias=_gb(mod.bias))
            else:
                da = _act_bwd_bn(a_dec[li], dh, blk.act.weight, bnsv, _gb(blk.act.weight),
                                 _gb(bnm.weight), _gb(bnm.bias), _gb(mod.bias))
            src = src_dec[li]
            with _SideStream(da, src):
                if W.needs_grad(mod):
                    gw = W.grad_target(mod)
                    if is_conv:
                        ops.wgrad(Src(da), src, gw, K, S, ops.conv_pad(K, S)[0], PAD_REFLECT)
                    else:
                        ops.wgrad(src, Src(da), gw, K, S, ops.deconv_pad(K, S), PAD_ZERO)
                    W.finish(mod, gw)
                _ready(blk)
            if is_conv:
                d_in = ops.conv1d_dgrad(da, w, src.L, S, pack=blk._pack)
                if li == 0:
                    dh_last_enc = d_in if gen.no_z else d_in[:, src.C0:].contiguous()
                else:
                    dh = d_in
            elif li == 0:
                if gen.no_z:
                    _d0, dh_last_enc = ops.deconv1d_dgrad(da, w, S, 0, pack=blk._pack)
                else:
                    _d0, dh_last_enc = ops.deconv1d_dgrad(da, w, S, src.C0, need0=False,
                                                          pack=blk._pack)
            else:
                if src.C1 > 0:
                    dh, dsk = ops.deconv1d_dgrad(da, w, S, src.C0, pack=blk._pack)
                    dskip[n_enc - 1 - li] = dsk
                else:
                    _d0, dh = ops.deconv1d_dgrad(da, w, S, 0, pack=blk._pack)
                    if getattr(src, 'sum_of', False):
                        dskip[n_enc - 1 - li] = dh
        dh = dh_last_enc
        dx = None
        for l in range(n_enc - 1, -1, -1):
            blk = enc[l]
            w = W.get(blk.conv)
            K, S = blk.kwidth, blk.stride
            bnsv = bn_enc[l]
            bnm = getattr(blk, 'norm', None)
            sc, sh = xf_enc[l]
            gskip = gen.skips[l]['alpha'] if (gen.skip and l in gen.skips) else None
            dsk = dskip.get(l)
            mask, a_norm = skip_saved.get(l, (None, None))
            if dsk is not None and mask is not None:
                dsk = ops.scale_mask(dsk, None, mask)
            alpha_p = None
            if gskip is not None and gskip.skip_type == 'conv':
                if dsk is not None:
                    dsk = _skip_conv_bwd(gskip, dsk, Src(a_enc[l], scale=sc, shift=sh), W)
                alpha_v = _ones(a_enc[l].shape[1], a_enc[l]) if dsk is not None else None
                ready_extra = gskip.skip_k
            else:
                alpha_p = gskip.skip_k if gskip is not None else None
                alpha_v = alpha_p if dsk is not None else None
                ready_extra = alpha_p
            if bnsv is None:
                da = ops.act_bwd(a_enc[l], dh, dskip=dsk, slope=blk.act.weight, alpha=alpha_v,
                                 dslope=_gb(blk.act.weight),
                                 dalpha=_gb(alpha_p, dsk is not None),
                                 dbias=_gb(blk.conv.bias))
            elif dsk is None:
                da = _act_bwd_bn(a_enc[l], dh, blk.act.weight, bnsv, _gb(blk.act.weight),
                                 _gb(bnm.weight), _gb(bnm.bias), _gb(blk.conv.bias))
            else:
                if a_norm is None:
                    a_norm = ops.affine_prelu(a_enc[l], sc, sh, None)
                g = ops.act_bwd(a_norm, dh, dskip=dsk, slope=blk.act.weight, alpha=alpha_v,
                                dslope=_gb(blk.act.weight), dalpha=_gb(alpha_p, True))
                da = _act_bwd_bn(a_enc[l], g, None, bnsv, None, _gb(bnm.weight), _gb(bnm.bias),
                                 _gb(blk.conv.bias))
            padL = ops.conv_pad(K, S)[0]
            with _SideStream(da, src_enc[l]):
                if W.needs_grad(blk.conv):
                    gw = W.grad_target(blk.conv)
                    ops.wgrad(Src(da), src_enc[l], gw, K, S, padL, PAD_REFLECT)
                    W.finish(blk.conv, gw)
                _ready(blk, ready_extra)
            if l > 0:
                dh = ops.conv1d_dgrad(da, w, src_enc[l].L, S, pack=blk._pack)
            elif ctx.x_needs:
                dx = ops.conv1d_dgrad(da, w, src_enc[l].L, S, pack=blk._pack)
        _join_side(dy)
        ctx.state = None
        return (None, None, dx, None) + (None,) * (len(ctx.needs_input_grad) - 4)


class DiscriminatorFn(torch.autograd.Function):

    @staticmethod
    def forward(ctx, disc, rolls, x, x1, *params):
        x = x.contiguous()
        blocks = list(disc.enc_blocks)
        training = disc.training
        src = Src(x) if x1 is None else Src(x, x1.contiguous())
        cs, srcs, bns, xfs = [], [], [], []
        W = _Weights()
        for l, blk in enumerate(blocks):
            c = ops.conv1d_fwd(src, W.get(blk.conv), blk.conv.bias, blk.stride, roll=rolls[l],
                               pack=blk._pack)
            srcs.append(src)
            cs.append(c)
            if blk.norm is not None:
                bn = blk.norm
                if _bn_batch_stats(bn, training):
                    mean, rstd, scale, shift = _bn_train_stats(c, bn, training)
                    bns.append((mean, rstd, bn.weight, bn.bias))
                else:
                    scale, shift, _rstd = _bn_eval_affine(bn)
                    bns.append('eval')
                xfs.append((scale, shift))
                src = Src(c, scale=scale, shift=shift, slope=blk.act.weight)
            else:
                bns.append(None)
                xfs.append((None, None))
                src = Src(c, slope=blk.act.weight)
        h = ops.affine_prelu(cs[-1], xfs[-1][0], xfs[-1][1], blocks[-1].act.weight)
        B = h.shape[0]
        fc = disc.fc
        pt = disc.pool_type
        extra = {}
        if pt == 'none':
            hf = h.view(B, -1)
            y1 = ops.linear_fwd(hf, W.get(fc[0]))
            a1 = ops.bias_prelu_rows(y1, fc[0].bias, W.get(fc[1]))
            y2 = ops.linear_fwd(a1, W.get(fc[2]))
            a2 = ops.bias_prelu_rows(y2, fc[2].bias, W.get(fc[3]))
            y3 = ops.linear_fwd(a2, W.get(fc[4]))
            out = ops.bias_prelu_rows(y3, fc[4].bias, None)
            head = (hf, y1, a1, y2, a2, y3)
        else:
            if pt == 'conv':
                pc = ops.conv1d_fwd(Src(h), W.get(disc.pool_conv), disc.pool_conv.bias, 1,
                                    pad_mode=PAD_ZERO, padL=0, pack=disc._pool_pack)
                hp, idx = pc.view(B, -1), None
                extra['avg_conv_h'] = hp
            else:
                hp, idx = ops.pool_time_fwd(h, 'max' if pt == 'gmax' else 'avg')
            y3 = ops.linear_fwd(hp, W.get(fc))
            out = ops.bias_prelu_rows(y3, fc.bias, None)
            head = (h, hp, idx, y3)
        ctx.disc = disc
        ctx.rolls = tuple(rolls)
        ctx.x_needs = x.requires_grad or (x1 is not None and x1.requires_grad)
        ctx.split = None if x1 is None else (x.shape[1], x.requires_grad, x1.requires_grad)
        ctx.state = (cs, srcs, bns, head, W)
        disc._last_fwd = (cs, xfs)
        disc._last_extra = extra
        disc._last_head = head
        return out

    @staticmethod
    def backward(ctx, dout):
        disc = ctx.disc
        cs, srcs, bns, head, W = ctx.state
        blocks = list(disc.enc_blocks)
        fc = disc.fc
        dout = dout.contiguous()
        def lin_wgrad(mod, dy, xin):
            if W.needs_grad(mod):
                gw = W.grad_target(mod)
                ops.linear_wgrad(dy, xin, gw)
                W.finish(mod, gw)

        def prelu_bwd(y, lin, act, dact):
            gs = W.grad_target(act) if W.needs_grad(act) else None
            d = ops.bias_prelu_rows_bwd(y, lin.bias, W.get(act), dact, gs, _gb(lin.bias))
            if gs is not None:
                W.finish(act, gs)
            return d

        if disc.pool_type == 'none':
            hf, y1, a1, y2, a2, y3 = head
            dy3 = ops.bias_prelu_rows_bwd(y3, fc[4].bias, None, dout, None, _gb(fc[4].bias))
            lin_wgrad(fc[4], dy3, a2)
            da2 = ops.linear_dgrad(dy3, W.get(fc[4]))
            dy2 = prelu_bwd(y2, fc[2], fc[3], da2)
            lin_wgrad(fc[2], dy2, a1)
            da1 = ops.linear_dgrad(dy2, W.get(fc[2]))
            dy1 = prelu_bwd(y1, fc[0], fc[1], da1)
            lin_wgrad(fc[0], dy1, hf)
            dh = ops.linear_dgrad(dy1, W.get(fc[0])).view(cs[-1].shape)
            _ready(fc)
        else:
            h, hp, idx, y3 = head
            Lh = h.shape[2]
            dy3 = ops.bias_prelu_rows_bwd(y3, fc.bias, None, dout, None, _gb(fc.bias))
            lin_wgrad(fc, dy3, hp)
            dhp = ops.linear_dgrad(dy3, W.get(fc))
            if disc.pool_type == 'conv':
                pcm = disc.pool_conv
                dpc = dhp.view(h.shape[0], 1, Lh)
                if pcm.bias is not None and pcm.bias.requires_grad:
                    ops.act_bwd(dpc, dpc, dbias=grad_buf(pcm.bias))
                if W.needs_grad(pcm):
                    gw = W.grad_target(pcm)
                    ops.wgrad(Src(dpc), Src(h), gw, 1, 1, 0, PAD_ZERO)
                    W.finish(pcm, gw)
                dh = ops.conv1d_dgrad(dpc, W.get(pcm), Lh, 1, padL=0, pack=disc._pool_pack)
                _ready(fc, pcm)
            else:
                dh = ops.pool_time_bwd(dhp, idx, Lh, 'max' if disc.pool_type == 'gmax' else 'avg')
                _ready(fc)
        dx = None
        for l in range(len(blocks) - 1, -1, -1):
            blk = blocks[l]
            w = W.get(blk.conv)
            K, S = blk.kwidth, blk.stride
            bn = bns[l]
            if bn == 'eval':
                raise RuntimeError('Discriminator backward in eval() mode with BatchNorm is not '
                                   'supported; call .train() (the reference never does this)')
            if bn is not None:
                dc = _act_bwd_bn(cs[l], dh, blk.act.weight, bn, _gb(blk.act.weight), _gb(bn[2]),
                                 _gb(bn[3]), _gb(blk.conv.bias))
            else:
                dc = ops.act_bwd(cs[l], dh, slope=blk.act.weight, dslope=_gb(blk.act.weight),
                                 dbias=_gb(blk.conv.bias))
            padL = ops.conv_pad(K, S)[0]
            with _SideStream(dc, srcs[l]):
                if W.needs_grad(blk.conv):
                    gw = W.grad_target(blk.conv)
                    ops.wgrad(Src(dc), srcs[l], gw, K, S, padL, PAD_REFLECT, roll=ctx.rolls[l])
                    W.finish(blk.conv, gw)
                _ready(blk)
            if l > 0:
                dh = ops.conv1d_dgrad(dc, w, srcs[l].L, S, roll=ctx.rolls[l], pack=blk._pack)
            elif ctx.x_needs:
                dx = ops.conv1d_dgrad(dc, w, srcs[l].L, S, roll=ctx.rolls[l], pack=blk._pack)
        _join_side(dout)
        ctx.state = None
        dx1 = None
        if dx is not None and ctx.split is not None:
            c0, need0, need1 = ctx.split
            dx1 = dx[:, c0:].contiguous() if need1 else None
            dx = dx[:, :c0].contiguous() if need0 else None
        return (None, None, dx, dx1) + (None,) * (len(ctx.needs_input_grad) - 4)


class ConvBlockFn(torch.autograd.Function):

    @staticmethod
    def forward(ctx, blk, x, *params):
        x = x.contiguous()
        src = Src(x)
        W = _Weights()
        c = ops.conv1d_fwd(src, W.get(blk.conv), blk.conv.bias, blk.stride, pack=blk._pack)
        bn_saved = None
        scale = shift = None
        if blk.norm is not None:
            bn = blk.norm
            if _bn_batch_stats(bn, blk.training):
                mean, rstd, scale, shift = _bn_train_stats(c, bn, blk.training)
                bn_saved = (mean, rstd, bn.weight, bn.bias)
            else:
                scale, shift, rstd = _bn_eval_affine(bn)
                bn_saved = ('eval', scale, shift, rstd)
        h = ops.affine_prelu(c, scale, shift, blk.act.weight)
        a = c if blk.norm is None else ops.affine_prelu(c, scale, shift, None)
        ctx.blk = blk
        ctx.set_materialize_grads(False)
        ctx.x_needs = x.requires_grad
        ctx.state = (src, c, bn_saved, W)
        return h, a

    @staticmethod
    def backward(ctx, dh, da_lin):
        blk = ctx.blk
        src, c, bn, W = ctx.state
        K, S = blk.kwidth, blk.stride
        w = W.get(blk.conv)
        if dh is None and da_lin is None:
            return (None,) * len(ctx.needs_input_grad)
        dh = dh.contiguous() if dh is not None else None
        if bn is None:
            lin = da_lin.contiguous() if da_lin is not None else None
            dc = ops.act_bwd(c, dh, dskip=lin, slope=blk.act.weight,
                             alpha=_ones(c.shape[1], c) if lin is not None else None,
                             dslope=_gb(blk.act.weight), dbias=_gb(blk.conv.bias))
        else:
            if da_lin is not None or dh is None:
                raise RuntimeError('gradient through the linear output of a normalised '
                                   'GConv1DBlock is unsupported')
            if isinstance(bn[0], str):
                dc = _eval_bn_act_bwd(c, blk.norm, bn[1], bn[2], bn[3], dh, blk.act.weight,
                                      _gb(blk.act.weight), dbias=_gb(blk.conv.bias))
            else:
                dc = _act_bwd_bn(c, dh, blk.act.weight, bn, _gb(blk.act.weight), _gb(bn[2]), _gb(bn[3]),
                                 _gb(blk.conv.bias))
        padL = ops.conv_pad(K, S)[0]
        if W.needs_grad(blk.conv):
            gw = W.grad_target(blk.conv)
            ops.wgrad(Src(dc), src, gw, K, S, padL, PAD_REFLECT)
            W.finish(blk.conv, gw)
        dx = ops.conv1d_dgrad(dc, w, src.L, S, pack=blk._pack) if ctx.x_needs else None
        ctx.state = None
        return (None, dx) + (None,) * (len(ctx.needs_input_grad) - 2)


class DeconvBlockFn(torch.autograd.Function):

    @staticmethod
    def forward(ctx, blk, x, *params):
        x = x.contiguous()
        src = Src(x)
        W = _Weights()
        bn = blk.norm if isinstance(blk.norm, torch.nn.BatchNorm1d) else None
        act = ACT_TANH if (blk.is_tanh and bn is None) else ACT_NONE
        c = ops.deconv1d_fwd(src, W.get(blk.deconv), blk.deconv.bias, blk.stride, act,
                             pack=blk._pack)
        bn_saved = None
        if bn is None:
            h = c if blk.is_tanh else ops.affine_prelu(c, slope=blk.act.weight)
        else:
            if _bn_batch_stats(bn, blk.training):
                mean, rstd, scale, shift = _bn_train_stats(c, bn, blk.training)
                bn_saved = (mean, rstd, bn.weight, bn.bias)
            else:
                scale, shift, rstd = _bn_eval_affine(bn)
                bn_saved = ('eval', scale, shift, rstd)
            h = ops.affine_tanh(c, scale, shift) if blk.is_tanh else \
                ops.affine_prelu(c, scale, shift, blk.act.weight)
        ctx.blk = blk
        ctx.x_needs = x.requires_grad
        ctx.state = (src, c, h if (blk.is_tanh and bn is not None) else None, bn_saved, W)
        return h

    @staticmethod
    def backward(ctx, dh):
        blk = ctx.blk
        src, c, y, bn, W = ctx.state
        K, S = blk.kwidth, blk.stride
        w = W.get(blk.deconv)
        dh = dh.contiguous()
        bnm = blk.norm if bn is not None else None
        if bn is not None and isinstance(bn[0], str):
            da = _eval_bn_act_bwd(c, bnm, bn[1], bn[2], bn[3], dh,
                                  None if blk.is_tanh else blk.act.weight,
                                  None if blk.is_tanh else _gb(blk.act.weight),
                                  y_tanh=y if blk.is_tanh else None, dbias=_gb(blk.deconv.bias))
        elif blk.is_tanh:
            if bn is None:
                da = ops.tanh_bwd(c, dh, dbias=_gb(blk.deconv.bias))
            else:
                da = _act_bwd_bn(c, ops.tanh_bwd(y, dh), None, bn, None, _gb(bnm.weight),
                                 _gb(bnm.bias), _gb(blk.deconv.bias))
        elif bn is None:
            da = ops.act_bwd(c, dh, slope=blk.act.weight, dslope=_gb(blk.act.weight),
                             dbias=_gb(blk.deconv.bias))
        else:
            da = _act_bwd_bn(c, dh, blk.act.weight, bn, _gb(blk.act.weight), _gb(bnm.weight),
                             _gb(bnm.bias), _gb(blk.deconv.bias))
        if W.needs_grad(blk.deconv):
            gw = W.grad_target(blk.deconv)
            ops.wgrad(src, Src(da), gw, K, S, ops.deconv_pad(K, S), PAD_ZERO)
            W.finish(blk.deconv, gw)
        dx = None
        if ctx.x_needs:
            _d0, dx = ops.deconv1d_dgrad(da, w, S, 0, pack=blk._pack)
        ctx.state = None
        return (None, dx) + (None,) * (len(ctx.needs_input_grad) - 2)


class MSEConstFn(torch.autograd.Function):

    @staticmethod
    def forward(ctx, x, target):
        x = x.contiguous()
        ctx.save_for_backward(x)
        ctx.target = float(target)
        return ops.mse_const(x, target)

    @staticmethod
    def backward(ctx, g):
        (x,) = ctx.saved_tensors
        return ops.mse_const_bwd(x, ctx.target, gout=g.contiguous()), None


class BCELogitsConstFn(torch.autograd.Function):

    @staticmethod
    def forward(ctx, x, target):
        x = x.contiguous()
        ctx.save_for_backward(x)
        ctx.target = float(target)
        return ops.bce_logits_const(x, target)

    @staticmethod
    def backward(ctx, g):
        (x,) = ctx.saved_tensors
        return ops.bce_logits_const_bwd(x, ctx.target, gout=g.contiguous()), None


class L1MeanFn(torch.autograd.Function):

    @staticmethod
    def forward(ctx, x, y):
        x, y = x.contiguous(), y.contiguous()
        ctx.save_for_backward(x, y)
        return ops.l1_mean(x, y)

    @staticmethod
    def backward(ctx, g):
        x, y = ctx.saved_tensors
        gx = gy = None
        if ctx.needs_input_grad[0]:
            gx = ops.l1_bwd(x, y, gout=g.contiguous())
        if ctx.needs_input_grad[1]:
            gy = ops.l1_bwd(y, x, gout=g.contiguous())
        return gx, gy


class MSEMeanFn(torch.autograd.Function):

    @staticmethod
    def forward(ctx, x, y):
        x, y = x.contiguous(), y.contiguous()
        ctx.save_for_backward(x, y)
        return ops.mse_mean(x, y)

    @staticmethod
    def backward(ctx, g):
        x, y = ctx.saved_tensors
        gx = gy = None
        if ctx.needs_input_grad[0]:
            gx = ops.mse_bwd(x, y, gout=g.contiguous())
        if ctx.needs_input_grad[1]:
            gy = ops.mse_bwd(y, x, gout=g.contiguous())
        return gx, gy


class STFTPowL1Fn(torch.autograd.Function):

    @staticmethod
    def forward(ctx, x, y, n_fft, hop, win):
        shape = x.shape
        x2 = x.reshape(shape[0], shape[-1]).contiguous()
        y2 = y.reshape(shape[0], shape[-1]).contiguous()
        basis = ops.stft_basis(n_fft, win, x2.device)
        Sx = ops.stft_spectrum(ops.stft_frames(x2, n_fft, hop, win), basis)
        nb = n_fft // 2 + 1
        dbx = ops.powdb(Sx, nb)
        dby = ops.powdb(ops.stft_spectrum(ops.stft_frames(y2, n_fft, hop, win), basis), nb)
        ctx.save_for_backward(Sx, dbx, dby, basis)
        ctx.geom = (shape, n_fft, hop, win)
        return ops.l1_mean(dbx, dby)

    @staticmethod
    def backward(ctx, g):
        Sx, dbx, dby, basis = ctx.saved_tensors
        shape, n_fft, hop, win = ctx.geom
        ddb = ops.l1_bwd(dbx, dby, gout=g.contiguous())
        dfr = ops.stft_spectrum_bwd(ops.powdb_bwd(Sx, ddb, n_fft // 2 + 1), basis)
        dx = ops.stft_overlap_add(dfr, shape[0], shape[-1], n_fft, hop, win)
        return dx.view(shape), None, None, None, None
```

segan_pytorch_amd/ops.py:

```python
import ctypes
import operator

import torch

from . import _lib
from . import layout
from ._lib import ACT_NONE, ACT_TANH, PAD_REFLECT, PAD_ZERO, SeganSrc, check


import os as _os

PREC_FP32, PREC_BF16, PREC_BF16X3 = 0, 1, 3
_PREC_NAMES = {'fp32': PREC_FP32, 'bf16': PREC_BF16, 'bf16x3': PREC_BF16X3}
_precision = _PREC_NAMES[_os.environ.get('SEGAN_PRECISION', 'fp32')]
_EUNSUPPORTED = -3


_deterministic = _os.environ.get('SEGAN_DETERMINISTIC', '0') == '1'


def set_deterministic(on):
    global _deterministic
    _deterministic = bool(on)


def get_deterministic():
    return _deterministic


_ACC_NAMES = ('plain', 'blocked')
_accumulation = _os.environ.get('SEGAN_ACCUMULATION', 'plain')
if _accumulation not in _ACC_NAMES:
    raise ValueError('SEGAN_ACCUMULATION must be one of {}'.format(_ACC_NAMES))
PREC_FP32_BLOCKED = 4


def set_accumulation(mode):
    global _accumulation
    if mode not in _ACC_NAMES:
        raise ValueError('accumulation must be one of {}'.format(_ACC_NAMES))
    _accumulation = mode


def get_accumulation():
    return _accumulation


def _fp32():
    return PREC_FP32_BLOCKED if _accumulation == 'blocked' else PREC_FP32


def set_precision(mode):
    global _precision
    if mode not in _PREC_NAMES:
        raise ValueError('precision must be one of {}'.format(sorted(_PREC_NAMES)))
    _precision = _PREC_NAMES[mode]


def get_precision():
    return [k for k, v in _PREC_NAMES.items() if v == _precision][0]


def _stream():
    return ctypes.c_void_p(torch._C._cuda_getCurrentRawStream(torch._C._cuda_getDevice()))


def _ptr(t):
    if t is None:
        return None
    return ctypes.c_void_p(t.data_ptr())


def _chk(t, name, ndim=None):
    if not isinstance(t, torch.Tensor):
        raise TypeError('{} must be a tensor, got {}'.format(name, type(t)))
    if not t.is_cuda:
        raise RuntimeError(
            '{} is on {}: segan_pytorch_amd runs only on an MI355X (HIP) device; '
            'there is no CPU path'.format(name, t.device))
    if t.dtype != torch.float32:
        raise TypeError('{} must be float32, got {}'.format(name, t.dtype))
    if not t.is_contiguous():
        raise ValueError('{} must be contiguous'.format(name))
    if ndim is not None and t.dim() != ndim:
        raise ValueError('{} must have {} dims, got {}'.format(name, ndim, tuple(t.shape)))
    return t


class Src(object):

    def __init__(self, t0, t1=None, scale=None, shift=None, slope=None):
        _chk(t0, 'src.t0', 3)
        self.t0, self.t1 = t0, t1
        self.C0 = t0.shape[1]
        self.C1 = 0
        if t1 is not None:
            _chk(t1, 'src.t1', 3)
            if t1.shape[0] != t0.shape[0] or t1.shape[2] != t0.shape[2]:
                raise ValueError('src segments disagree: {} vs {}'.format(
                    tuple(t0.shape), tuple(t1.shape)))
            self.C1 = t1.shape[1]
        self.C = self.C0 + self.C1
        for name, v in (('scale', scale), ('shift', shift), ('slope', slope)):
            if v is not None:
                _chk(v, 'src.' + name)
                if v.numel() != self.C:
                    raise ValueError('src.{} has {} entries for {} channels'.format(
                        name, v.numel(), self.C))
        self.scale, self.shift, self.slope = scale, shift, slope
        self.B, self.L = t0.shape[0], t0.shape[2]

    def c_struct(self):
        s = SeganSrc()
        s.p0 = self.t0.data_ptr()
        s.p1 = self.t1.data_ptr() if self.t1 is not None else None
        s.C0, s.C1 = self.C0, self.C1
        s.scale = self.scale.data_ptr() if self.scale is not None else None
        s.shift = self.shift.data_ptr() if self.shift is not None else None
        s.slope = self.slope.data_ptr() if self.slope is not None else None
        return s


_corr_scratch = {}


def _scratch():
    dev = torch._C._cuda_getDevice()
    key = (dev, torch._C._cuda_getCurrentRawStream(dev))
    buf = _corr_scratch.get(key)
    if buf is None:
        nbytes = _lib.load().segan_corr_scratch_bytes()
        buf = torch.empty(nbytes, device=torch.device('cuda', dev), dtype=torch.uint8)
        _corr_scratch[key] = buf
    return ctypes.c_void_p(buf.data_ptr()), buf.numel()


def last_corr_launch():
    arr = (ctypes.c_int * 6)()
    _lib.load().segan_debug_last_corr(arr)
    k = ('kernel', 'workgroups', 'tiles', 'tiles_whole', 'streamk_units', 'xf_mode')
    d = dict(zip(k, list(arr)))
    d['streamk'] = d['streamk_units'] > 0
    return d


def last_wgrad_launch():
    arr = (ctypes.c_int * 6)()
    _lib.load().segan_debug_last_wgrad(arr)
    return dict(zip(('kernel', 'tiles', 'splits', 'chunks_per_split', 'resident_per_cu', 'hi_loads'),
                    list(arr)))


_call_scratch = {}


def _stream_scratch(nbytes, device):
    dev = torch.device(device).index
    if dev is None:
        dev = torch._C._cuda_getDevice()
    key = (dev, torch._C._cuda_getCurrentRawStream(dev))
    buf = _call_scratch.get(key)
    if buf is None or buf.numel() < nbytes:
        buf = None
        _call_scratch.pop(key, None)
        buf = torch.empty(int(nbytes), device=torch.device('cuda', dev), dtype=torch.uint8)
        _call_scratch[key] = buf
    return buf


def set_reserved_slots(n):
    return int(_lib.load().segan_set_reserved_slots(int(n)))


def release_scratch(device=None):
    dev = None if device is None else torch.device(device).index
    for d in (_corr_scratch, _call_scratch):
        for key in [k for k in d if dev is None or k[0] == dev]:
            del d[key]


def scratch_bytes():
    return sum(b.numel() for d in (_corr_scratch, _call_scratch) for b in d.values())


def _bf_scratch(op, B, N, M, L, K, S, pad, device):
    planes = 3 if _precision == PREC_BF16X3 else 1
    nbytes = _lib.load().segan_bf16_scratch_bytes(op, B, N, M, L, K, S, pad, planes)
    if nbytes == 0:
        return None, None, 0
    buf = _stream_scratch(nbytes, device)
    return buf, ctypes.c_void_p(buf.data_ptr()), nbytes


def conv_pad(K, S):
    return layout.conv_pad(K, S)


def deconv_pad(K, S):
    return layout.deconv_pad(K, S)


_weights_epoch = 0


def bump_weights_epoch(params=None):
    global _weights_epoch
    if params is None:
        _weights_epoch += 1
        return
    for p in params:
        p._segan_epoch = getattr(p, '_segan_epoch', 0) + 1


class WeightPack(object):

    def __init__(self):
        self._buf = {}
        self._key = {}

    def _get(self, w, S, pad_t, want):
        _chk(w, 'weight', 3)
        key = (w.data_ptr(), w._version, _weights_epoch, getattr(w, '_segan_epoch', 0),
               tuple(w.shape), S, pad_t)
        if self._key.get(want) == key:
            return self._buf[want]
        lib = _lib.load()
        M, N, K = w.shape
        nbytes = (lib.segan_packed_f_bytes if want == 'f' else lib.segan_packed_t_bytes)(M, N, S)
        if nbytes == 0:
            raise ValueError('unsupported stride {} (must be 1, 2 or 4)'.format(S))
        buf = self._buf.get(want)
        if buf is None or buf.numel() * 4 != nbytes or buf.device != w.device:
            buf = torch.empty(nbytes // 4, device=w.device, dtype=torch.float32)
        check(lib.segan_pack_weights(_ptr(w), _ptr(buf) if want == 'f' else None,
                                     _ptr(buf) if want == 't' else None, M, N, K, S, pad_t,
                                     _stream()), 'pack_weights')
        self._buf[want] = buf
        self._key[want] = key
        return buf

    def f(self, w, S):
        return self._get(w, S, 0, 'f')

    def g(self, w, S):
        _chk(w, 'weight', 3)
        key = (w.data_ptr(), w._version, _weights_epoch, getattr(w, '_segan_epoch', 0),
               tuple(w.shape), S)
        if self._key.get('g') == key:
            return self._buf['g']
        lib = _lib.load()
        M, N, K = w.shape
        nbytes = lib.segan_packed_g_bytes(M, N, S)
        if nbytes == 0:
            raise ValueError('G packing: stride {} not supported'.format(S))
        buf = self._buf.get('g')
        if buf is None or buf.numel() * 4 != nbytes or buf.device != w.device:
            buf = torch.empty(nbytes // 4, device=w.device, dtype=torch.float32)
        check(lib.segan_pack_weights_g(_ptr(w), _ptr(buf), M, N, K, S, _stream()), 'pack_weights_g')
        self._buf['g'] = buf
        self._key['g'] = key
        return buf

    def t(self, w, S, pad_t):
        return self._get(w, S, pad_t, 't')

    def bf(self, w, S, pad_t, tform, planes):
        _chk(w, 'weight', 3)
        want = ('bf', tform, planes)
        key = (w.data_ptr(), w._version, _weights_epoch, getattr(w, '_segan_epoch', 0),
               tuple(w.shape), S, pad_t)
        if self._key.get(want) == key:
            return self._buf[want]
        lib = _lib.load()
        M, N, K = w.shape
        nbytes = lib.segan_packed_bf_bytes(M, N, S, tform, planes)
        if nbytes == 0:
            raise ValueError('unsupported geometry for bf16 packing')
        buf = self._buf.get(want)
        if buf is None or buf.numel() * 2 != nbytes or buf.device != w.device:
            buf = torch.empty(nbytes // 2, device=w.device, dtype=torch.bfloat16)
        check(lib.segan_pack_weights_bf(_ptr(w), _ptr(buf), M, N, K, S, tform, pad_t, planes,
                                        _stream()), 'pack_weights_bf')
        self._buf[want] = buf
        self._key[want] = key
        return buf


def conv1d_fwd(src, w, bias, S, roll=0, pad_mode=PAD_REFLECT, padL=None, pack=None):
    M, N, K = w.shape
    if src.C != N:
        raise ValueError('conv1d_fwd: input has {} channels, weight expects {}'.format(src.C, N))
    B, L = src.B, src.L
    if L % S != 0:
        raise ValueError('conv1d_fwd: length {} not divisible by stride {}'.format(L, S))
    if padL is None:
        padL = conv_pad(K, S)[0]
    out = torch.empty((B, M, L // S), device=w.device, dtype=torch.float32)
    cs = src.c_struct()
    pack = pack or WeightPack()
    lib = _lib.load()
    if _precision and pad_mode == PAD_REFLECT:
        keep, sp, sn = _bf_scratch(0, B, N, M, L, K, S, padL, w.device)
        rc = lib.segan_conv1d_fwd(ctypes.byref(cs), _ptr(pack.bf(w, S, 0, 0, _precision)),
                                  _ptr(bias), _ptr(out), B, N, M, L, K, S, padL, pad_mode, roll,
                                  _precision, sp, sn, _stream())
        if rc != _EUNSUPPORTED:
            check(rc, 'conv1d_fwd')
            return out
    check(lib.segan_conv1d_fwd(ctypes.byref(cs), _ptr(pack.f(w, S)), _ptr(bias), _ptr(out), B, N,
                               M, L, K, S, padL, pad_mode, roll, _fp32(), *_scratch(), _stream()),
          'conv1d_fwd')
    return out


def conv1d_dgrad(da, w, L, S, roll=0, padL=None, pack=None):
    _chk(da, 'da', 3)
    M, N, K = w.shape
    B = da.shape[0]
    if da.shape[1] != M or da.shape[2] * S != L:
        raise ValueError('conv1d_dgrad: da {} inconsistent with weight {} / L {}'.format(
            tuple(da.shape), tuple(w.shape), L))
    if padL is None:
        padL = conv_pad(K, S)[0]
    small = N <= 2
    _chk(w, 'weight', 3)
    pack = pack or WeightPack()
    if not small and not _precision and short_rows_ok(N, M, L, S):
        return conv1d_dgrad_short(da, w, L, S, roll=roll, padL=padL, pack=pack)
    dx = torch.empty((B, N, L), device=da.device, dtype=torch.float32)
    halo = torch.empty((B * N * max(K - 1, 1),), device=da.device, dtype=torch.float32)
    lib = _lib.load()
    if small:
        check(lib.segan_conv1d_dgrad(_ptr(da), None, _ptr(w.detach()), _ptr(dx), _ptr(halo), B, N,
                                     M, L, K, S, padL, roll, PREC_FP32, None, 0, _stream()),
              'conv1d_dgrad')
        return dx
    if _precision:
        keep, sp, sn = _bf_scratch(1, B, N, M, L, K, S, padL, da.device)
        rc = lib.segan_conv1d_dgrad(_ptr(da), _ptr(pack.bf(w, S, 0, 1, _precision)), None, _ptr(dx),
                                    _ptr(halo), B, N, M, L, K, S, padL, roll, _precision, sp, sn,
                                    _stream())
        if rc != _EUNSUPPORTED:
            check(rc, 'conv1d_dgrad')
            return dx
    if short_rows_ok(N, M, L, S):
        return conv1d_dgrad_short(da, w, L, S, roll=roll, padL=padL, pack=pack)
    check(lib.segan_conv1d_dgrad(_ptr(da), _ptr(pack.t(w, S, 0)), None, _ptr(dx), _ptr(halo), B, N,
                                 M, L, K, S, padL, roll, _fp32(), *_scratch(), _stream()),
          'conv1d_dgrad')
    return dx


def conv1d_dgrad_short(da, w, L, S, roll=0, padL=None, pack=None):
    _chk(da, 'da', 3)
    _chk(w, 'weight', 3)
    M, N, K = w.shape
    B = da.shape[0]
    if padL is None:
        padL = conv_pad(K, S)[0]
    dx = torch.empty((B, N, L), device=da.device, dtype=torch.float32)
    pack = pack or WeightPack()
    check(_lib.load().segan_conv1d_dgrad_short(_ptr(da), _ptr(pack.g(w, S)), _ptr(dx), B, N,
                                               M, L, K, S, padL, roll, _stream()),
          'conv1d_dgrad_short')
    return dx


_SHORT_LS = (4, 8, 16, 32, 64)


def short_rows_ok(N, M, L, S):
    return S in (2, 4) and L % S == 0 and (L // S) in _SHORT_LS and N % 4 == 0 and M % 16 == 0


def wgrad(lo, hi, dw, K, S, padL, pad_mode, roll=0):
    _chk(dw, 'dw', 3)
    M, N = lo.C, hi.C
    if tuple(dw.shape) != (M, N, K):
        raise ValueError('wgrad: dw {} != ({}, {}, {})'.format(tuple(dw.shape), M, N, K))
    if lo.B != hi.B or lo.L * S != hi.L:
        raise ValueError('wgrad: lo [{}x{}] / hi [{}x{}] inconsistent for stride {}'.format(
            lo.B, lo.L, hi.B, hi.L, S))
    cl, ch = lo.c_struct(), hi.c_struct()
    lib = _lib.load()
    if _precision != PREC_FP32:
        nbytes = lib.segan_wgrad_scratch_bytes(lo.B, M, N, lo.L, S, _precision, 0)
        scratch = _stream_scratch(nbytes, dw.device)
        rc = lib.segan_wgrad(ctypes.byref(cl), ctypes.byref(ch), _ptr(dw), lo.B, M, N, lo.L, K, S,
                             padL, pad_mode, roll, _precision, 0,
                             ctypes.c_void_p(scratch.data_ptr()) if scratch is not None else None,
                             nbytes if scratch is not None else 0, _stream())
        if rc != -3:
            check(rc, 'wgrad')
            return
    flags = 1 if _deterministic else 0
    lo_plain = lo.t1 is None and lo.scale is None and lo.shift is None and lo.slope is None
    scratch, nbytes = None, 0
    if flags or not lo_plain:
        nbytes = lib.segan_wgrad_scratch_bytes(lo.B, M, N, lo.L, S, PREC_FP32, flags)
        scratch = _stream_scratch(nbytes, dw.device)
    check(lib.segan_wgrad(ctypes.byref(cl), ctypes.byref(ch), _ptr(dw), lo.B, M, N, lo.L, K, S, padL,
                          pad_mode, roll, PREC_FP32, flags,
                          ctypes.c_void_p(scratch.data_ptr()) if scratch is not None else None, nbytes,
                          _stream()), 'wgrad')


def deconv1d_fwd(src, w, bias, S, act=ACT_NONE, pack=None):
    M, N, K = w.shape
    if src.C != M:
        raise ValueError('deconv1d_fwd: input has {} channels, weight expects {}'.format(src.C, M))
    pad = deconv_pad(K, S)
    B, Ls = src.B, src.L
    y = torch.empty((B, N, S * Ls), device=w.device, dtype=torch.float32)
    cs = src.c_struct()
    small = N <= 2
    _chk(w, 'weight', 3)
    pack = pack or WeightPack()
    lib = _lib.load()
    if small:
        check(lib.segan_deconv1d_fwd(ctypes.byref(cs), None, _ptr(w.detach()), _ptr(bias), _ptr(y),
                                     B, M, N, Ls, K, S, pad, act, PREC_FP32, None, 0, _stream()),
              'deconv1d_fwd')
        return y
    if _precision and act == ACT_NONE:
        keep, sp, sn = _bf_scratch(2, B, N, M, S * Ls, K, S, pad, w.device)
        rc = lib.segan_deconv1d_fwd(ctypes.byref(cs), _ptr(pack.bf(w, S, pad, 1, _precision)), None,
                                    _ptr(bias), _ptr(y), B, M, N, Ls, K, S, pad, act, _precision,
                                    sp, sn, _stream())
        if rc != _EUNSUPPORTED:
            check(rc, 'deconv1d_fwd')
            return y
    check(lib.segan_deconv1d_fwd(ctypes.byref(cs), _ptr(pack.t(w, S, pad)), None, _ptr(bias),
                                 _ptr(y), B, M, N, Ls, K, S, pad, act, _fp32(), *_scratch(),
                                 _stream()), 'deconv1d_fwd')
    return y


def deconv1d_dgrad(dy, w, S, M0=0, need0=True, need1=True, pack=None):
    _chk(dy, 'dy', 3)
    M, N, K = w.shape
    B = dy.shape[0]
    if dy.shape[1] != N or dy.shape[2] % S != 0:
        raise ValueError('deconv1d_dgrad: dy {} inconsistent with weight {}'.format(
            tuple(dy.shape), tuple(w.shape)))
    Ls = dy.shape[2] // S
    pad = deconv_pad(K, S)
    dx0 = dx1 = None
    if M0 > 0 and need0:
        dx0 = torch.empty((B, M0, Ls), device=dy.device, dtype=torch.float32)
    if M - M0 > 0 and need1:
        dx1 = torch.empty((B, M - M0, Ls), device=dy.device, dtype=torch.float32)
    if dx0 is None and dx1 is None:
        return None, None
    pack = pack or WeightPack()
    lib = _lib.load()
    if _precision:
        keep, sp, sn = _bf_scratch(3, B, N, M, S * Ls, K, S, pad, dy.device)
        rc = lib.segan_deconv1d_dgrad(_ptr(dy), _ptr(pack.bf(w, S, 0, 0, _precision)), _ptr(dx0),
                                      _ptr(dx1), B, M, M0, N, Ls, K, S, pad, _precision, sp, sn,
                                      _stream())
        if rc != _EUNSUPPORTED:
            check(rc, 'deconv1d_dgrad')
            return dx0, dx1
    check(lib.segan_deconv1d_dgrad(_ptr(dy), _ptr(pack.f(w, S)), _ptr(dx0), _ptr(dx1), B, M, M0, N,
                                   Ls, K, S, pad, _fp32(), *_scratch(), _stream()), 'deconv1d_dgrad')
    return dx0, dx1


def _ws(B, C, L, per_split, extra, device):
    ns = _lib.load().segan_bn_nsplit(B, C, L)
    return torch.empty((per_split * ns * C + extra * C,), device=device, dtype=torch.float32)


def bn_stats(x, gamma, beta, eps, momentum, running_mean, running_var):
    _chk(x, 'x', 3)
    B, C, L = x.shape
    mean = torch.empty(C, device=x.device, dtype=torch.float32)
    rstd = torch.empty_like(mean)
    scale = torch.empty_like(mean)
    shift = torch.empty_like(mean)
    ws = _ws(B, C, L, 3, 0, x.device)
    check(_lib.load().segan_bn_stats(_ptr(x), _ptr(gamma), _ptr(beta), eps, momentum,
                                     _ptr(running_mean), _ptr(running_var), _ptr(mean), _ptr(rstd),
                                     _ptr(scale), _ptr(shift), _ptr(ws), B, C, L, _stream()),
          'bn_stats')
    return mean, rstd, scale, shift


def bn_partial(x):
    _chk(x, 'x', 3)
    B, C, L = x.shape
    ns = _lib.load().segan_bn_nsplit(B, C, L)
    ws = torch.empty((ns, C, 3), device=x.device, dtype=torch.float32)
    check(_lib.load().segan_bn_partial(_ptr(x), _ptr(ws), B, C, L, _stream()), 'bn_partial')
    return ws


def bn_final(ws_all, gamma, beta, eps, momentum, running_mean, running_var):
    _chk(ws_all, 'ws_all', 3)
    C = ws_all.shape[1]
    mean = torch.empty(C, device=ws_all.device, dtype=torch.float32)
    rstd, scale, shift = torch.empty_like(mean), torch.empty_like(mean), torch.empty_like(mean)
    check(_lib.load().segan_bn_final(_ptr(ws_all), ws_all.shape[0], _ptr(gamma), _ptr(beta), eps,
                                     momentum, _ptr(running_mean), _ptr(running_var), _ptr(mean),
                                     _ptr(rstd), _ptr(scale), _ptr(shift), C, _stream()), 'bn_final')
    return mean, rstd, scale, shift


def act_bwd_bn_reduce(a, dh, slope, bn, dslope=None, dgamma=None, dbeta=None):
    _chk(a, 'a', 3)
    B, C, L = a.shape
    mean, rstd, gamma, beta = bn
    totals = torch.empty((C, 2), device=a.device, dtype=torch.float32)
    ws = _ws(B, C, L, 4, 2, a.device)
    check(_lib.load().segan_act_bwd_bn_reduce(_ptr(a), _ptr(dh), _ptr(slope), _ptr(mean), _ptr(rstd),
                                              _ptr(gamma), _ptr(beta), _ptr(dslope), _ptr(dgamma),
                                              _ptr(dbeta), _ptr(totals), _ptr(ws), B, C, L, _stream()),
          'act_bwd_bn_reduce')
    return totals, ws


def act_bwd_bn_apply(a, dh, slope, bn, totals, count_total, dbias=None, ws=None):
    _chk(a, 'a', 3)
    B, C, L = a.shape
    mean, rstd, gamma, beta = bn
    da = torch.empty_like(a)
    if ws is None:
        ws = _ws(B, C, L, 4, 2, a.device)
    check(_lib.load().segan_act_bwd_bn_apply(_ptr(a), _ptr(dh), _ptr(slope), _ptr(mean), _ptr(rstd),
                                             _ptr(gamma), _ptr(beta), _ptr(totals), _ptr(da),
                                             _ptr(dbias), _ptr(ws), B, C, L, float(count_total),
                                             _stream()), 'act_bwd_bn_apply')
    return da


def affine_prelu(x, scale=None, shift=None, slope=None):
    _chk(x, 'x', 3)
    B, C, L = x.shape
    y = torch.empty_like(x)
    check(_lib.load().segan_affine_prelu(_ptr(x), _ptr(scale), _ptr(shift), _ptr(slope), _ptr(y),
                                         B, C, L, _stream()), 'affine_prelu')
    return y


def affine_tanh(x, scale=None, shift=None):
    _chk(x, 'x', 3)
    B, C, L = x.shape
    y = torch.empty_like(x)
    check(_lib.load().segan_affine_tanh(_ptr(x), _ptr(scale), _ptr(shift), _ptr(y), B, C, L,
                                        _stream()), 'affine_tanh')
    return y


def scale_mask(x, scale, mask):
    _chk(x, 'x', 3)
    _chk(mask, 'mask', 3)
    if mask.shape != x.shape:
        raise ValueError('scale_mask: mask {} vs x {}'.format(tuple(mask.shape), tuple(x.shape)))
    B, C, L = x.shape
    y = torch.empty_like(x)
    check(_lib.load().segan_scale_mask(_ptr(x), _ptr(scale), _ptr(mask), _ptr(y), B, C, L,
                                       _stream()), 'scale_mask')
    return y


def sum_skip(x0, slope0, x1, alpha):
    _chk(x0, 'x0', 3)
    _chk(x1, 'x1', 3)
    if x0.shape != x1.shape:
        raise ValueError('sum_skip: shapes differ {} vs {}'.format(tuple(x0.shape), tuple(x1.shape)))
    B, C, L = x0.shape
    out = torch.empty_like(x0)
    check(_lib.load().segan_sum_skip(_ptr(x0), _ptr(slope0), _ptr(x1), _ptr(alpha), _ptr(out), B, C,
                                     L, _stream()), 'sum_skip')
    return out


def act_bwd(a, dh, dskip=None, slope=None, alpha=None, bn=None, dslope=None, dalpha=None,
            dgamma=None, dbeta=None, dbias=None):
    _chk(a, 'a', 3)
    B, C, L = a.shape
    da = torch.empty_like(a)
    ws = _ws(B, C, L, 4, 2, a.device)
    mean = rstd = gamma = beta = None
    if bn is not None:
        mean, rstd, gamma, beta = bn
    check(_lib.load().segan_act_bwd(_ptr(a), _ptr(dh), _ptr(dskip), _ptr(slope), _ptr(alpha),
                                    _ptr(mean), _ptr(rstd), _ptr(gamma), _ptr(beta), _ptr(da),
                                    _ptr(dslope), _ptr(dalpha), _ptr(dgamma), _ptr(dbeta),
                                    _ptr(dbias), _ptr(ws), B, C, L, _stream()), 'act_bwd')
    return da


def tanh_bwd(y, dy, clean=None, l1_scale=0.0, dbias=None):
    _chk(y, 'y', 3)
    B, C, L = y.shape
    da = torch.empty_like(y)
    ws = _ws(B, C, L, 1, 0, y.device)
    check(_lib.load().segan_tanh_bwd(_ptr(y), _ptr(dy), _ptr(clean), float(l1_scale), _ptr(da),
                                     _ptr(dbias), _ptr(ws), B, C, L, _stream()), 'tanh_bwd')
    return da


def gemm(A, sam, sak, Bm, sbk, sbn, C, M, N, K, overwrite):
    lib = _lib.load()
    sp, sn = None, 0
    if _deterministic:
        sn = lib.segan_gemm_scratch_bytes(M, N, K)
        keep = torch.empty(sn, device=C.device, dtype=torch.uint8)
        sp = ctypes.c_void_p(keep.data_ptr())
    check(lib.segan_gemm(_ptr(A), sam, sak, _ptr(Bm), sbk, sbn, _ptr(C), C.stride(0), M, N,
                         K, 1 if overwrite else 0, 1 if _deterministic else 0, sp, sn, _stream()),
          'gemm')


def linear_fwd(x, w):
    _chk(x, 'x', 2)
    _chk(w, 'w', 2)
    Bn, I = x.shape
    O = w.shape[0]
    y = torch.empty((Bn, O), device=x.device, dtype=torch.float32)
    gemm(x, I, 1, w, 1, I, y, Bn, O, I, True)
    return y


def linear_dgrad(dy, w):
    Bn, O = dy.shape
    I = w.shape[1]
    dx = torch.empty((Bn, I), device=dy.device, dtype=torch.float32)
    gemm(dy, O, 1, w, I, 1, dx, Bn, I, O, True)
    return dx


def linear_wgrad(dy, x, dw):
    Bn, O = dy.shape
    I = x.shape[1]
    gemm(dy, 1, O, x, I, 1, dw, O, I, Bn, False)


def bias_prelu_rows(x, bias, slope):
    _chk(x, 'x', 2)
    y = torch.empty_like(x)
    check(_lib.load().segan_bias_prelu_rows(_ptr(x), _ptr(bias), _ptr(slope), _ptr(y), x.shape[0],
                                            x.shape[1], _stream()), 'bias_prelu_rows')
    return y


def bias_prelu_rows_bwd(x, bias, slope, dy, dslope, dbias):
    dx = torch.empty_like(x)
    check(_lib.load().segan_bias_prelu_rows_bwd(_ptr(x), _ptr(bias), _ptr(slope), _ptr(dy),
                                                _ptr(dx), _ptr(dslope), _ptr(dbias), x.shape[0],
                                                x.shape[1], _stream()), 'bias_prelu_rows_bwd')
    return dx


def pool_time_fwd(x, mode):
    _chk(x, 'x', 3)
    B, C, L = x.shape
    y = torch.empty((B, C), device=x.device, dtype=torch.float32)
    idx = torch.empty((B, C), device=x.device, dtype=torch.int32) if mode == 'max' else None
    check(_lib.load().segan_pool_time_fwd(_ptr(x), _ptr(y), _ptr(idx), B * C, L,
                                          0 if mode == 'max' else 1, _stream()), 'pool_time_fwd')
    return y, idx


def pool_time_bwd(dy, idx, L, mode):
    _chk(dy, 'dy', 2)
    B, C = dy.shape
    dx = torch.empty((B, C, L), device=dy.device, dtype=torch.float32)
    check(_lib.load().segan_pool_time_bwd(_ptr(dy), _ptr(idx), _ptr(dx), B * C, L,
                                          0 if mode == 'max' else 1, _stream()), 'pool_time_bwd')
    return dx


def mse_const(x, target):
    _chk(x, 'x')
    loss = torch.empty((), device=x.device, dtype=torch.float32)
    check(_lib.load().segan_mse_const(_ptr(x), float(target), _ptr(loss), None, None, 1.0,
                                      x.numel(), _stream()), 'mse_const')
    return loss


def mse_const_bwd(x, target, gout=None, gscale=1.0):
    _chk(x, 'x')
    grad = torch.empty_like(x)
    check(_lib.load().segan_mse_const(_ptr(x), float(target), None, _ptr(grad), _ptr(gout),
                                      float(gscale), x.numel(), _stream()), 'mse_const_bwd')
    return grad


def bce_logits_const(x, target):
    _chk(x, 'x')
    loss = torch.empty((), device=x.device, dtype=torch.float32)
    check(_lib.load().segan_bce_logits_const(_ptr(x), float(target), _ptr(loss), None, None, 1.0,
                                             x.numel(), _stream()), 'bce_logits_const')
    return loss


def bce_logits_const_bwd(x, target, gout=None, gscale=1.0):
    _chk(x, 'x')
    grad = torch.empty_like(x)
    check(_lib.load().segan_bce_logits_const(_ptr(x), float(target), None, _ptr(grad), _ptr(gout),
                                             float(gscale), x.numel(), _stream()),
          'bce_logits_const_bwd')
    return grad


def l1_bwd(x, y, gout=None, gscale=1.0):
    _chk(x, 'x')
    grad = torch.empty_like(x)
    check(_lib.load().segan_l1_bwd(_ptr(x), _ptr(y), _ptr(gout), float(gscale), _ptr(grad),
                                   x.numel(), _stream()), 'l1_bwd')
    return grad


def l1_mean(x, y):
    _chk(x, 'x')
    _chk(y, 'y')
    if x.shape != y.shape:
        raise ValueError('l1_mean: shapes differ {} vs {}'.format(tuple(x.shape), tuple(y.shape)))
    loss = torch.empty((), device=x.device, dtype=torch.float32)
    ws = torch.empty(1024, device=x.device, dtype=torch.float32)
    check(_lib.load().segan_l1_mean(_ptr(x), _ptr(y), _ptr(loss), _ptr(ws), x.numel(), _stream()),
          'l1_mean')
    return loss


def mse_mean(x, y):
    _chk(x, 'x')
    _chk(y, 'y')
    if x.shape != y.shape:
        raise ValueError('mse_mean: shapes differ {} vs {}'.format(tuple(x.shape), tuple(y.shape)))
    loss = torch.empty((), device=x.device, dtype=torch.float32)
    ws = torch.empty(1024, device=x.device, dtype=torch.float32)
    check(_lib.load().segan_mse_mean(_ptr(x), _ptr(y), _ptr(loss), _ptr(ws), x.numel(), _stream()),
          'mse_mean')
    return loss


def mse_bwd(x, y, gout=None, gscale=1.0):
    _chk(x, 'x')
    grad = torch.empty_like(x)
    check(_lib.load().segan_mse_bwd(_ptr(x), _ptr(y), _ptr(gout), float(gscale), _ptr(grad),
                                    x.numel(), _stream()), 'mse_bwd')
    return grad


_stft_basis_cache = {}


def stft_pitch(n_fft):
    return (2 * (n_fft // 2 + 1) + 3) // 4 * 4


def stft_basis(n_fft, win, device):
    key = (n_fft, win, str(device))
    if key not in _stft_basis_cache:
        bs = torch.empty((win, stft_pitch(n_fft)), device=device, dtype=torch.float32)
        check(_lib.load().segan_stft_basis(_ptr(bs), n_fft, win, _stream()), 'stft_basis')
        _stft_basis_cache[key] = bs
    return _stft_basis_cache[key]


def stft_frames(x, n_fft, hop, win):
    _chk(x, 'x', 2)
    B, T = x.shape
    NF = 1 + T // hop
    fr = torch.empty((B * NF, win), device=x.device, dtype=torch.float32)
    check(_lib.load().segan_stft_frames(_ptr(x), _ptr(fr), B, T, n_fft, hop, win, _stream()),
          'stft_frames')
    return fr


def stft_spectrum(frames, basis):
    R, win = frames.shape
    N2 = basis.shape[1]
    S = torch.empty((R, N2), device=frames.device, dtype=torch.float32)
    gemm(frames, win, 1, basis, N2, 1, S, R, N2, win, True)
    return S


def stft_spectrum_bwd(dS, basis):
    R, N2 = dS.shape
    win = basis.shape[0]
    df = torch.empty((R, win), device=dS.device, dtype=torch.float32)
    gemm(dS, N2, 1, basis, 1, N2, df, R, win, N2, True)
    return df


def powdb(S, nbins, eps=10e-20):
    _chk(S, 'S', 2)
    rows, pitch = S.shape
    db = torch.empty((rows, nbins), device=S.device, dtype=torch.float32)
    check(_lib.load().segan_powdb(_ptr(S), _ptr(db), rows, nbins, pitch, eps, _stream()), 'powdb')
    return db


def powdb_bwd(S, ddb, nbins, eps=10e-20):
    _chk(S, 'S', 2)
    _chk(ddb, 'ddb', 2)
    rows, pitch = S.shape
    dS = torch.empty_like(S)
    check(_lib.load().segan_powdb_bwd(_ptr(S), _ptr(ddb), _ptr(dS), rows, nbins, pitch, eps,
                                      _stream()), 'powdb_bwd')
    return dS


def stft_overlap_add(dframes, B, T, n_fft, hop, win):
    _chk(dframes, 'dframes', 2)
    dx = torch.empty((B, T), device=dframes.device, dtype=torch.float32)
    check(_lib.load().segan_stft_overlap_add(_ptr(dframes), _ptr(dx), B, T, n_fft, hop, win,
                                             _stream()), 'stft_overlap_add')
    return dx


def _sn_view(w, dim):
    shp = tuple(w.shape) + (1,) * (3 - w.dim())
    if w.dim() > 3 or dim not in (0, 1) or (dim == 1 and w.dim() < 2):
        raise ValueError('snorm: unsupported weight shape {} / dim {}'.format(tuple(w.shape), dim))
    return shp


def snorm_fwd(w, u, v, dim, power_iteration, eps=1e-12):
    _chk(w, 'w')
    _chk(u, 'u', 1)
    _chk(v, 'v', 1)
    A, Bd, K = _sn_view(w, dim)
    rows, cols = (A, Bd * K) if dim == 0 else (Bd, A * K)
    if u.numel() != rows or v.numel() != cols:
        raise ValueError('snorm: u[{}] / v[{}] do not match the {}x{} matrix view'.format(
            u.numel(), v.numel(), rows, cols))
    lib = _lib.load()
    w_sn = torch.empty_like(w)
    sigma = torch.empty(1, device=w.device, dtype=torch.float32)
    ws = torch.empty(lib.segan_snorm_ws_floats(A, Bd, K, dim), device=w.device, dtype=torch.float32)
    check(lib.segan_snorm_fwd(_ptr(w), _ptr(u), _ptr(v), _ptr(w_sn), _ptr(sigma), _ptr(ws), A, Bd, K,
                              dim, 1 if power_iteration else 0, float(eps), _stream()), 'snorm_fwd')
    return w_sn, sigma


def snorm_bwd(dw_sn, w, u, v, sigma, dim, dw):
    _chk(dw_sn, 'dw_sn')
    _chk(dw, 'dw')
    A, Bd, K = _sn_view(w, dim)
    lib = _lib.load()
    ws = torch.empty(lib.segan_snorm_ws_floats(A, Bd, K, dim), device=w.device, dtype=torch.float32)
    check(lib.segan_snorm_bwd(_ptr(dw_sn), _ptr(w), _ptr(u), _ptr(v), _ptr(sigma), _ptr(dw), _ptr(ws),
                              A, Bd, K, dim, _stream()), 'snorm_bwd')


def pcm16_prep(pcm, first, coef):
    if pcm.dtype != torch.int16 or first.dtype != torch.uint8 or not pcm.is_cuda or not first.is_cuda:
        raise TypeError('pcm16_prep: pcm must be a CUDA int16 tensor and first a CUDA uint8 tensor')
    if pcm.dim() != 3 or pcm.shape[1] != 2 or not pcm.is_contiguous() or first.numel() != pcm.shape[0]:
        raise ValueError('pcm16_prep: pcm must be contiguous [B, 2, T+1], first [B]')
    B, T = pcm.shape[0], pcm.shape[2] - 1
    clean = torch.empty((B, T), device=pcm.device, dtype=torch.float32)
    noisy = torch.empty((B, T), device=pcm.device, dtype=torch.float32)
    check(_lib.load().segan_pcm16_prep(ctypes.c_void_p(pcm.data_ptr()),
                                       ctypes.c_void_p(first.data_ptr()), _ptr(clean), _ptr(noisy),
                                       B, T, float(coef), _stream()), 'pcm16_prep')
    return clean, noisy


def de_emphasize(y, coef):
    _chk(y, 'y')
    T = y.shape[-1]
    x = torch.empty_like(y)
    check(_lib.load().segan_deemphasis(_ptr(y), _ptr(x), y.numel() // T, T, float(coef), _stream()),
          'deemphasis')
    return x


def ssnr(ref, deg, srate=16000, eps=1e-10):
    _chk(ref, 'ref', 2)
    _chk(deg, 'deg', 2)
    if ref.shape != deg.shape:
        raise ValueError('ssnr: shapes differ {} vs {}'.format(tuple(ref.shape), tuple(deg.shape)))
    rows, T = ref.shape
    lib = _lib.load()
    nf = lib.segan_ssnr_frames(T, srate)
    seg = torch.empty((rows, max(nf, 1)), device=ref.device, dtype=torch.float32)
    out = torch.empty((rows, 2), device=ref.device, dtype=torch.float32)
    check(lib.segan_ssnr(_ptr(ref), _ptr(deg), _ptr(seg), _ptr(out), rows, T, srate, float(eps),
                         _stream()), 'ssnr')
    return out[:, 0], out[:, 1], seg[:, :nf]


def _quality_frames(fn, what, ref, deg, srate):
    _chk(ref, 'ref', 2)
    _chk(deg, 'deg', 2)
    if ref.shape != deg.shape:
        raise ValueError('{}: shapes differ {} vs {}'.format(what, tuple(ref.shape), tuple(deg.shape)))
    rows, T = ref.shape
    nf = _lib.load().segan_ssnr_frames(T, srate)
    dist = torch.empty((rows, max(nf, 1)), device=ref.device, dtype=torch.float64)
    check(fn(_ptr(ref), _ptr(deg), _ptr(dist), rows, T, srate, _stream()), what)
    return dist[:, :nf]


def wss(ref, deg, srate=16000):
    return _quality_frames(_lib.load().segan_wss, 'wss', ref, deg, srate)


def llr(ref, deg, srate=16000):
    return _quality_frames(_lib.load().segan_llr, 'llr', ref, deg, srate)


STOI_SRATES = (4000, 48000)
STOI_BANDS = 15


def _stoi_srate(srate):
    srate_in = srate
    try:
        srate = None if isinstance(srate, bool) else operator.index(srate)
    except TypeError:
        srate = None
    if srate is None or not STOI_SRATES[0] <= srate <= STOI_SRATES[1]:
        raise ValueError('stoi: srate must be an integer from {} to {} Hz, got {!r}'.format(
            STOI_SRATES[0], STOI_SRATES[1], srate_in))
    return srate


def stoi_plan(srate):
    srate = _stoi_srate(srate)
    lib = _lib.load()
    pq, n, bands = (ctypes.c_int * 2)(), ctypes.c_int(), (ctypes.c_int * (2 * STOI_BANDS))()
    check(lib.segan_stoi_plan(srate, pq, ctypes.byref(n), None, 0, None), 'stoi_plan')
    taps = torch.empty(n.value, dtype=torch.float64)
    check(lib.segan_stoi_plan(srate, pq, ctypes.byref(n), _ptr(taps), n.value, bands), 'stoi_plan')
    return pq[0], pq[1], taps, torch.tensor(list(bands), dtype=torch.int64).view(STOI_BANDS, 2)


def _stoi_lengths(lengths, rows, T, device):
    lens = torch.as_tensor(lengths).detach().cpu()
    if lens.dim() != 1 or lens.numel() != rows or lens.dtype.is_floating_point or lens.dtype in (
            torch.bool, torch.complex64, torch.complex128):
        raise ValueError('stoi: lengths must hold {} integers, got {}'.format(rows, lengths))
    if rows and (int(lens.min()) < 0 or int(lens.max()) > T):
        raise ValueError('stoi: lengths must lie in 0 .. {}, got {}'.format(T, lens.tolist()))
    return lens.to(dtype=torch.int32).to(device)


def stoi_stages(ref, deg, srate=16000, lengths=None):
    _chk(ref, 'ref', 2)
    _chk(deg, 'deg', 2)
    if ref.shape != deg.shape:
        raise ValueError('stoi: shapes differ {} vs {}'.format(tuple(ref.shape), tuple(deg.shape)))
    srate = _stoi_srate(srate)
    rows, T = ref.shape
    lens = None if lengths is None else _stoi_lengths(lengths, rows, T, ref.device)
    lib = _lib.load()
    dims = (ctypes.c_int * 5)()
    check(lib.segan_stoi_dims(T, srate, dims), 'stoi')
    Ly, F, Lc, Fb, S = list(dims)
    f64 = dict(device=ref.device, dtype=torch.float64)
    i32 = dict(device=ref.device, dtype=torch.int32)
    xr = torch.empty((2, rows, max(Ly, 1)), **f64)
    energy = torch.empty((rows, max(F, 1)), **f64)
    mask = torch.empty((rows, max(F, 1)), **i32)
    kept = torch.empty((rows, max(F, 1)), **i32)
    count = torch.empty(rows, **i32)
    xs = torch.empty((2, rows, max(Lc, 1)), **f64)
    env = torch.empty((2, rows, STOI_BANDS, max(Fb, 1)), **f64)
    rho = torch.empty((rows, max(S, 1), STOI_BANDS), **f64)
    d = torch.empty(rows, **f64)
    check(lib.segan_stoi(_ptr(ref), _ptr(deg), _ptr(lens), rows, T, srate, _ptr(xr[0]), _ptr(xr[1]),
                         _ptr(energy), _ptr(mask), _ptr(kept), _ptr(count), _ptr(xs[0]),
                         _ptr(xs[1]), _ptr(env[0]), _ptr(env[1]), _ptr(rho), _ptr(d), _stream()),
          'stoi')
    return dict(xr=xr[0, :, :Ly], yr=xr[1, :, :Ly], energy=energy[:, :F], mask=mask[:, :F],
                kept=kept[:, :F], count=count, xs=xs[0, :, :Lc], ys=xs[1, :, :Lc],
                X=env[0, :, :, :Fb], Y=env[1, :, :, :Fb], rho=rho[:, :S], d=d,
                dims=(Ly, F, Lc, Fb, S))


def stoi(ref, deg, srate=16000, lengths=None):
    return stoi_stages(ref, deg, srate, lengths)['d']


def rmsprop_step(p, g, sq, lr, alpha, eps):
    check(_lib.load().segan_rmsprop_step(_ptr(p), _ptr(g), _ptr(sq), lr, alpha, eps, p.numel(),
                                         _stream()), 'rmsprop_step')


def adam_step(p, g, m, v, lr, beta1, beta2, eps, step):
    check(_lib.load().segan_adam_step(_ptr(p), _ptr(g), _ptr(m), _ptr(v), lr, beta1, beta2, eps,
                                      step, p.numel(), _stream()), 'adam_step')


def fill_(t, value):
    _chk(t, 't')
    check(_lib.load().segan_fill(_ptr(t), float(value), t.numel(), _stream()), 'fill')
    return t


def scale_(t, s):
    _chk(t, 't')
    check(_lib.load().segan_scale(_ptr(t), float(s), t.numel(), _stream()), 'scale')
    return t


def comm_unique_id():
    lib = _lib.load()
    buf = ctypes.create_string_buffer(lib.segan_comm_id_bytes())
    check(lib.segan_comm_unique_id(buf), 'comm_unique_id')
    return buf.raw


class Comm(object):

    def __init__(self, world, rank, unique_id):
        lib = _lib.load()
        if len(unique_id) != lib.segan_comm_id_bytes():
            raise ValueError('Comm: unique id must be {} bytes'.format(lib.segan_comm_id_bytes()))
        h = ctypes.c_void_p()
        check(lib.segan_comm_init(ctypes.byref(h), int(world), int(rank), unique_id), 'comm_init')
        self._h, self.world, self.rank = h, int(world), int(rank)

    def _s(self, stream):
        return ctypes.c_void_p((stream or torch.cuda.current_stream()).cuda_stream)

    def allreduce(self, t, scale=1.0, stream=None):
        _chk(t, 't')
        check(_lib.load().segan_allreduce(self._h, _ptr(t), t.numel(), float(scale), self._s(stream)),
              'allreduce')
        return t

    def broadcast(self, t, root=0, stream=None):
        _chk(t, 't')
        check(_lib.load().segan_broadcast(self._h, _ptr(t), t.numel(), int(root), self._s(stream)),
              'broadcast')
        return t

    def allgather(self, send, stream=None):
        _chk(send, 'send')
        recv = torch.empty((self.world,) + tuple(send.shape), device=send.device, dtype=torch.float32)
        check(_lib.load().segan_allgather(self._h, _ptr(send), _ptr(recv), send.numel(),
                                          self._s(stream)), 'allgather')
        return recv

    def destroy(self):
        if self._h is not None:
            check(_lib.load().segan_comm_destroy(self._h), 'comm_destroy')
            self._h = None
```

segan_pytorch_amd/optim.py:

```python
import torch

from . import ops

_ALIGN = 64


class _FlatOptimizer(torch.optim.Optimizer):
    _state_names = ()

    def __init__(self, params, defaults):
        super().__init__(params, defaults)
        self._params = [p for g in self.param_groups for p in g['params']]
        if not self._params:
            raise ValueError('optimizer got an empty parameter list')
        self._build_arenas()

    def _build_arenas(self):
        dev = self._params[0].device
        offs, off = [], 0
        for p in self._params:
            if p.device != dev or p.dtype != torch.float32:
                raise ValueError('all parameters must be fp32 on one device')
            offs.append(off)
            off += (p.numel() + _ALIGN - 1) // _ALIGN * _ALIGN
        self._offsets, self._total = offs, off
        self.flat_param = torch.zeros(off, device=dev, dtype=torch.float32)
        self.flat_grad = torch.zeros(off, device=dev, dtype=torch.float32)
        self._flat_state = {n: torch.zeros(off, device=dev, dtype=torch.float32)
                            for n in self._state_names}
        with torch.no_grad():
            for p, o in zip(self._params, offs):
                view = self.flat_param[o:o + p.numel()].view(p.shape)
                view.copy_(p.data)
                p.data = view
                g = self.flat_grad[o:o + p.numel()].view(p.shape)
                if p.grad is not None:
                    g.copy_(p.grad)
                p.grad = g
                st = self.state[p]
                st['step'] = torch.tensor(0.0, dtype=torch.float32)
                for n in self._state_names:
                    st[n] = self._flat_state[n][o:o + p.numel()].view(p.shape)
        ops.bump_weights_epoch()

    def _view(self, flat, i):
        p = self._params[i]
        o = self._offsets[i]
        return flat[o:o + p.numel()].view(p.shape)

    def _resync(self):
        dev = self.flat_param.device
        for i, p in enumerate(self._params):
            o = self._offsets[i]
            want_p = self.flat_param.data_ptr() + 4 * o
            if p.device != dev:
                self._build_arenas()
                return
            if p.data_ptr() != want_p:
                with torch.no_grad():
                    v = self._view(self.flat_param, i)
                    v.copy_(p.data)
                    p.data = v
            g = p.grad
            want_g = self.flat_grad.data_ptr() + 4 * o
            if g is None:
                v = self._view(self.flat_grad, i)
                v.zero_()
                p.grad = v
            elif g.data_ptr() != want_g:
                v = self._view(self.flat_grad, i)
                v.copy_(g)
                p.grad = v

    def zero_grad(self, set_to_none=False):
        self._resync()
        if self.flat_grad.is_cuda:
            ops.fill_(self.flat_grad, 0.0)
        else:
            self.flat_grad.zero_()

    def state_dict(self):
        return super().state_dict()

    def load_state_dict(self, state_dict):
        super().load_state_dict(state_dict)
        with torch.no_grad():
            for i, p in enumerate(self._params):
                st = self.state[p]
                for n in self._state_names:
                    v = self._view(self._flat_state[n], i)
                    if n in st:
                        v.copy_(st[n])
                    st[n] = v
                if 'step' not in st:
                    st['step'] = torch.tensor(0.0, dtype=torch.float32)
                elif not torch.is_tensor(st['step']):
                    st['step'] = torch.tensor(float(st['step']), dtype=torch.float32)

    def _bump_steps(self):
        for p in self._params:
            st = self.state[p]
            st['step'] = st['step'] + 1 if torch.is_tensor(st['step']) else st['step'] + 1

    def _require_cuda(self):
        if not self.flat_param.is_cuda:
            raise RuntimeError('segan_pytorch_amd optimizers step only on an MI355X (HIP) device; '
                               'parameters are on {}'.format(self.flat_param.device))


class RMSprop(_FlatOptimizer):
    _state_names = ('square_avg',)

    def __init__(self, params, lr=1e-2, alpha=0.99, eps=1e-8, weight_decay=0, momentum=0,
                 centered=False):
        if weight_decay != 0 or momentum != 0 or centered:
            raise NotImplementedError('only plain RMSprop (as model.py:221-222 builds it) is '
                                      'implemented')
        defaults = dict(lr=lr, momentum=momentum, alpha=alpha, eps=eps, centered=centered,
                        weight_decay=weight_decay, capturable=False, foreach=None,
                        maximize=False, differentiable=False)
        super().__init__(params, defaults)

    @torch.no_grad()
    def step(self, closure=None):
        loss = closure() if closure is not None else None
        self._require_cuda()
        self._resync()
        g = self.param_groups[0]
        if len(self.param_groups) != 1:
            raise NotImplementedError('a single param group is supported')
        ops.rmsprop_step(self.flat_param, self.flat_grad, self._flat_state['square_avg'],
                         float(g['lr']), float(g['alpha']), float(g['eps']))
        self._bump_steps()
        ops.bump_weights_epoch(self._params)
        return loss


class Adam(_FlatOptimizer):
    _state_names = ('exp_avg', 'exp_avg_sq')

    def __init__(self, params, lr=1e-3, betas=(0.9, 0.999), eps=1e-8, weight_decay=0,
                 amsgrad=False):
        if weight_decay != 0 or amsgrad:
            raise NotImplementedError('weight decay / amsgrad are not implemented')
        defaults = dict(lr=lr, betas=betas, eps=eps, weight_decay=weight_decay, amsgrad=amsgrad,
                        maximize=False, foreach=None, capturable=False, differentiable=False,
                        fused=None)
        super().__init__(params, defaults)
        self._nsteps = 0

    @torch.no_grad()
    def step(self, closure=None):
        loss = closure() if closure is not None else None
        self._require_cuda()
        self._resync()
        if len(self.param_groups) != 1:
            raise NotImplementedError('a single param group is supported')
        g = self.param_groups[0]
        st0 = self.state[self._params[0]]['step']
        self._nsteps = int(st0.item() if torch.is_tensor(st0) else st0) + 1
        ops.adam_step(self.flat_param, self.flat_grad, self._flat_state['exp_avg'],
                      self._flat_state['exp_avg_sq'], float(g['lr']), float(g['betas'][0]),
                      float(g['betas'][1]), float(g['eps']), self._nsteps)
        self._bump_steps()
        ops.bump_weights_epoch(self._params)
        return loss
```

Before: 3578.

## Fuse BN stats/backward reductions via ticket counters and batch weight repacking per step

```diff
diff --git a/include/segan_hip.h b/include/segan_hip.h
--- a/include/segan_hip.h
+++ b/include/segan_hip.h
@@ -8,7 +8,7 @@
 extern "C" {
 #endif
 
-#define SEGAN_ABI_VERSION 15
+#define SEGAN_ABI_VERSION 16
 
 #define SEGAN_PAD_REFLECT 0
 #define SEGAN_PAD_ZERO 1
@@ -82,6 +82,10 @@
 int segan_bn_final(const float* ws, int nsplit_total, const float* gamma, const float* beta,
                    float eps, float momentum, float* running_mean, float* running_var, float* mean,
                    float* rstd, float* scale, float* shift, int C, void* stream);
+int segan_bn_stats_fused(const float* x, const float* gamma, const float* beta, float eps,
+                         float momentum, float* running_mean, float* running_var,
+                         int64_t* num_batches_tracked, float* mean, float* rstd, float* scale,
+                         float* shift, float* ws, int* tickets, int B, int C, int L, void* stream);
 
 int segan_affine_tanh(const float* x, const float* scale, const float* shift, float* y, int B,
                       int C, int L, void* stream);
@@ -99,6 +103,11 @@
                   const float* bn_gamma, const float* bn_beta, float* da, float* dslope,
                   float* dalpha, float* dgamma, float* dbeta, float* dbias, float* ws, int B, int C,
                   int L, void* stream);
+int segan_act_bwd_fused(const float* a, const float* dh, const float* dskip, const float* slope,
+                        const float* alpha, const float* bn_mean, const float* bn_rstd,
+                        const float* bn_gamma, const float* bn_beta, float* da, float* dslope,
+                        float* dalpha, float* dgamma, float* dbeta, float* dbias, float* ws,
+                        int* tickets, int B, int C, int L, void* stream);
 int segan_act_bwd_bn_reduce(const float* a, const float* dh, const float* slope,
                             const float* bn_mean, const float* bn_rstd, const float* bn_gamma,
                             const float* bn_beta, float* dslope, float* dgamma, float* dbeta,
@@ -135,6 +144,20 @@
 
 size_t segan_packed_g_bytes(int M, int N, int S);
 int segan_pack_weights_g(const float* w, float* wg, int M, int N, int K, int S, void* stream);
+
+#define SEGAN_PACK_F 0
+#define SEGAN_PACK_T 1
+#define SEGAN_PACK_G 2
+typedef struct segan_pack_rec {
+  const float* w;
+  float* dst;
+  int32_t form, M, N, K, S, pad_t;
+  int32_t gx, gy, block0;
+  int32_t pitch, rows, aux;
+} segan_pack_rec;
+int segan_pack_table_plan(segan_pack_rec* recs, int n);
+int segan_pack_table(const segan_pack_rec* recs, int n, int nblocks, void* stream);
+
 int segan_conv1d_dgrad_short(const float* da, const float* wg, float* dx, int B, int N, int M,
                              int L, int K, int S, int padL, int roll, void* stream);
 
diff --git a/segan_pytorch_amd/_lib.py b/segan_pytorch_amd/_lib.py
--- a/segan_pytorch_amd/_lib.py
+++ b/segan_pytorch_amd/_lib.py
@@ -9,13 +9,22 @@
 PAD_ZERO = 1
 ACT_NONE = 0
 ACT_TANH = 1
-ABI_VERSION = 15
+ABI_VERSION = 16
 
 
 class SeganSrc(Structure):
     _fields_ = [('p0', c_void_p), ('p1', c_void_p), ('C0', c_int32), ('C1', c_int32),
                 ('scale', c_void_p), ('shift', c_void_p), ('slope', c_void_p)]
 
+
+class SeganPackRec(Structure):
+    _fields_ = [('w', c_void_p), ('dst', c_void_p), ('form', c_int32), ('M', c_int32),
+                ('N', c_int32), ('K', c_int32), ('S', c_int32), ('pad_t', c_int32),
+                ('gx', c_int32), ('gy', c_int32), ('block0', c_int32), ('pitch', c_int32),
+                ('rows', c_int32), ('aux', c_int32)]
+
+
+PACK_F, PACK_T, PACK_G = 0, 1, 2
 
 _P = c_void_p
 _SRC = POINTER(SeganSrc)
@@ -47,6 +56,10 @@
     'segan_bn_nsplit': (c_int, [c_int, c_int, c_int]),
     'segan_bn_stats': (c_int, [_P, _P, _P, c_float, c_float, _P, _P, _P, _P, _P, _P, _P, c_int, c_int,
                                c_int, _P]),
+    'segan_bn_stats_fused': (c_int, [_P, _P, _P, c_float, c_float] + [_P] * 9 + [c_int, c_int, c_int, _P]),
+    'segan_act_bwd_fused': (c_int, [_P] * 17 + [c_int, c_int, c_int, _P]),
+    'segan_pack_table_plan': (c_int, [POINTER(SeganPackRec), c_int]),
+    'segan_pack_table': (c_int, [_P, c_int, c_int, _P]),
     'segan_bn_partial': (c_int, [_P, _P, c_int, c_int, c_int, _P]),
     'segan_bn_final': (c_int, [_P, c_int, _P, _P, c_float, c_float, _P, _P, _P, _P, _P, _P, c_int, _P]),
     'segan_act_bwd_bn_reduce': (c_int, [_P] * 12 + [c_int, c_int, c_int, _P]),
diff --git a/segan_pytorch_amd/csrc/segan_pack.hip b/segan_pytorch_amd/csrc/segan_pack.hip
--- a/segan_pytorch_amd/csrc/segan_pack.hip
+++ b/segan_pytorch_amd/csrc/segan_pack.hip
@@ -1,11 +1,11 @@
 #include "segan_conv_shared.h"
 
-__global__ __launch_bounds__(256) void pack_f_kernel(const float* __restrict__ w,
-                                                     float* __restrict__ wf, int M, int N, int K,
-                                                     int S, int U, int pitch, int rows, int pair) {
-  __shared__ float t[64][33];
-  const int n = blockIdx.y;
-  const int m0 = blockIdx.x * 64;
+__device__ __forceinline__ void pack_f_body(float (&t)[64][33], int bx, int by,
+                                            const float* __restrict__ w, float* __restrict__ wf,
+                                            int M, int N, int K, int S, int U, int pitch, int rows,
+                                            int pair) {
+  const int n = by;
+  const int m0 = bx * 64;
   const int tid = threadIdx.x;
   {
     float v[8];
@@ -36,13 +36,19 @@
   }
 }
 
-__global__ __launch_bounds__(256) void pack_t_kernel(const float* __restrict__ w,
-                                                     float* __restrict__ wt, int M, int N, int K,
-                                                     int S, int U, int NP, int pad, int pitch,
-                                                     int rows) {
+__global__ __launch_bounds__(256) void pack_f_kernel(const float* __restrict__ w,
+                                                     float* __restrict__ wf, int M, int N, int K,
+                                                     int S, int U, int pitch, int rows, int pair) {
   __shared__ float t[64][33];
-  const int m = blockIdx.y;
-  const int n0 = blockIdx.x * 64;
+  pack_f_body(t, blockIdx.x, blockIdx.y, w, wf, M, N, K, S, U, pitch, rows, pair);
+}
+
+__device__ __forceinline__ void pack_t_body(float (&t)[64][33], int bx, int by,
+                                            const float* __restrict__ w, float* __restrict__ wt,
+                                            int M, int N, int K, int S, int U, int NP, int pad,
+                                            int pitch, int rows) {
+  const int m = by;
+  const int n0 = bx * 64;
   const int tid = threadIdx.x;
   {
     float v[8];
@@ -68,6 +74,43 @@
     const int row = m * U + up;
     const int n = n0 + nl;
     if (row < rows && n < NP) wt[(size_t)row * pitch + r * NP + n] = t[nl][k];
+  }
+}
+
+__global__ __launch_bounds__(256) void pack_t_kernel(const float* __restrict__ w,
+                                                     float* __restrict__ wt, int M, int N, int K,
+                                                     int S, int U, int NP, int pad, int pitch,
+                                                     int rows) {
+  __shared__ float t[64][33];
+  pack_t_body(t, blockIdx.x, blockIdx.y, w, wt, M, N, K, S, U, NP, pad, pitch, rows);
+}
+
+__global__ __launch_bounds__(256) void pack_table_kernel(const segan_pack_rec* __restrict__ recs,
+                                                         int nrec) {
+  __shared__ float t[64][33];
+  const int bid = blockIdx.x;
+  int lo = 0, hi = nrec - 1;
+  while (lo < hi) {
+    const int mid = (lo + hi + 1) >> 1;
+    if (recs[mid].block0 <= bid) lo = mid; else hi = mid - 1;
+  }
+  const segan_pack_rec r = recs[lo];
+  const int local = bid - r.block0;
+  if (local >= r.gx * r.gy) return;
+  const int bx = local % r.gx, by = local / r.gx;
+  const int U = 32 / r.S;
+  if (r.form == SEGAN_PACK_F) {
+    pack_f_body(t, bx, by, r.w, r.dst, r.M, r.N, r.K, r.S, U, r.pitch, r.rows, r.aux);
+  } else if (r.form == SEGAN_PACK_T) {
+    pack_t_body(t, bx, by, r.w, r.dst, r.M, r.N, r.K, r.S, U, r.aux, r.pad_t, r.pitch, r.rows);
+  } else {
+    const size_t total = (size_t)r.M * r.N * 32;
+    for (size_t i = bx * (size_t)256 + threadIdx.x; i < total; i += (size_t)r.gx * 256) {
+      const int c = (int)(i & 31);
+      const size_t mn = i >> 5;
+      const int k = r.S * (c % U) + c / U;
+      r.dst[i] = k < r.K ? r.w[mn * r.K + k] : 0.0f;
+    }
   }
 }
 
@@ -102,3 +145,48 @@
   }
   return segan_check_launch("pack_weights");
 }
+
+extern "C" int segan_pack_table_plan(segan_pack_rec* recs, int n) {
+  SEGAN_REQUIRE(recs && n > 0, "pack_table_plan: no records");
+  long long total = 0;
+  for (int i = 0; i < n; ++i) {
+    segan_pack_rec& r = recs[i];
+    SEGAN_REQUIRE(r.w && r.dst, "pack_table_plan: record %d has a NULL pointer", i);
+    SEGAN_REQUIRE(r.form == SEGAN_PACK_F || r.form == SEGAN_PACK_T || r.form == SEGAN_PACK_G,
+                  "pack_table_plan: record %d has form %d", i, r.form);
+    SEGAN_REQUIRE(stride_ok(r.S), "pack_table_plan: record %d: stride %d not in {1,2,4}", i, r.S);
+    SEGAN_REQUIRE(r.K >= 1 && r.K <= 32, "pack_table_plan: record %d: width %d not in [1,32]", i, r.K);
+    SEGAN_REQUIRE(r.M > 0 && r.N > 0 && r.pad_t >= 0, "pack_table_plan: record %d: bad sizes", i);
+    const int U = 32 / r.S;
+    if (r.form == SEGAN_PACK_F) {
+      r.pitch = f_pitch(r.M);
+      r.rows = f_rows(r.N);
+      r.aux = f_pair(r.N, r.K);
+      r.gx = r.pitch / 64;
+      r.gy = ceil_div(r.rows, 32);
+    } else if (r.form == SEGAN_PACK_T) {
+      r.aux = t_np(r.N, r.S);
+      r.pitch = t_pitch(r.N, r.S);
+      r.rows = t_rows(r.M, r.S);
+      r.gx = ceil_div(r.aux, 64);
+      r.gy = ceil_div(r.rows, U);
+    } else {
+      r.pitch = r.N * 32;
+      r.rows = r.M;
+      r.aux = 0;
+      const size_t tot = (size_t)r.M * r.N * 32;
+      r.gx = (int)((tot + 255) / 256 > 8192 ? 8192 : (tot + 255) / 256);
+      r.gy = 1;
+    }
+    r.block0 = (int)total;
+    total += (long long)r.gx * r.gy;
+    SEGAN_REQUIRE(total < (1ll << 30), "pack_table_plan: too many workgroups");
+  }
+  return (int)total;
+}
+
+extern "C" int segan_pack_table(const segan_pack_rec* recs, int n, int nblocks, void* stream) {
+  SEGAN_REQUIRE(recs && n > 0 && nblocks > 0, "pack_table: bad arguments");
+  hipLaunchKernelGGL(pack_table_kernel, dim3(nblocks), dim3(256), 0, (hipStream_t)stream, recs, n);
+  return segan_check_launch("pack_table");
+}
diff --git a/segan_pytorch_amd/csrc/segan_pointwise.hip b/segan_pytorch_amd/csrc/segan_pointwise.hip
--- a/segan_pytorch_amd/csrc/segan_pointwise.hip
+++ b/segan_pytorch_amd/csrc/segan_pointwise.hip
@@ -50,6 +50,49 @@
   return r;
 }
 
+#define PW_MAX_TICKETS 16384
+
+__device__ __forceinline__ void pw_publish(float* p, float v) {
+  __hip_atomic_store(p, v, __ATOMIC_RELAXED, __HIP_MEMORY_SCOPE_AGENT);
+}
+__device__ __forceinline__ float pw_consume(const float* p) {
+  return __hip_atomic_load(p, __ATOMIC_RELAXED, __HIP_MEMORY_SCOPE_AGENT);
+}
+
+__device__ __forceinline__ bool pw_arrive_last(int* ticket, int nsplit, int* flag) {
+  if (threadIdx.x == 0) asm volatile("s_waitcnt vmcnt(0)" ::: "memory");
+  if (nsplit == 1) return true;
+  if (threadIdx.x == 0) {
+    const int t = __hip_atomic_fetch_add(ticket, 1, __ATOMIC_RELAXED, __HIP_MEMORY_SCOPE_AGENT);
+    const int last = t == nsplit - 1;
+    if (last) __hip_atomic_store(ticket, 0, __ATOMIC_RELAXED, __HIP_MEMORY_SCOPE_AGENT);
+    *flag = last;
+  }
+  __syncthreads();
+  const bool last = *flag != 0;
+  __builtin_amdgcn_fence(__ATOMIC_ACQUIRE, "wavefront");
+  return last;
+}
+
+template <int NW, typename F>
+__device__ __forceinline__ void pw_walk_partials(const float* ws, int stride, int C, int c,
+                                                 int nsplit, float* stage, F add) {
+  for (int s0 = 0; s0 < nsplit; s0 += PW_THREADS) {
+    const int s = s0 + (int)threadIdx.x;
+    if (s < nsplit) {
+      const float* w = ws + ((size_t)s * C + c) * stride;
+#pragma unroll
+      for (int k = 0; k < NW; ++k) stage[threadIdx.x * NW + k] = pw_consume(w + k);
+    }
+    __syncthreads();
+    if (threadIdx.x == 0) {
+      const int n = min(PW_THREADS, nsplit - s0);
+      for (int i = 0; i < n; ++i) add(stage + i * NW);
+    }
+    __syncthreads();
+  }
+}
+
 __device__ __forceinline__ void chan_combine(float& n, float& mean, float& m2, float nb, float mb,
                                              float qb) {
   const float tot = n + nb;
@@ -61,9 +104,62 @@
   n = tot;
 }
 
-__global__ void bn_partial_kernel(const float* __restrict__ x, float* __restrict__ ws, int B, int C,
-                                  int L, int nsplit) {
-  __shared__ float sm[3 * (PW_THREADS / 64)];
+__device__ __forceinline__ void bn_affine(float gamma, float beta, float mean, float rstd,
+                                          float& scale, float& shift) {
+  scale = gamma * rstd;
+  shift = fmaf(-mean, scale, beta);
+}
+
+struct BnFinalArgs {
+  const float* gamma;
+  const float* beta;
+  float eps, momentum;
+  float* running_mean;
+  float* running_var;
+  float* mean_o;
+  float* rstd_o;
+  float* scale_o;
+  float* shift_o;
+  long long* counter;
+  int* tickets;
+};
+struct BnAcc {
+  double n, mean, m2;
+};
+__device__ __forceinline__ void bn_acc_add(BnAcc& a, const float* w) {
+  const double nb = w[0], mb = w[1], qb = w[2];
+  if (nb <= 0.0) return;
+  const double tot = a.n + nb;
+  const double d = mb - a.mean;
+  a.mean += d * nb / tot;
+  a.m2 += qb + d * d * a.n * nb / tot;
+  a.n = tot;
+}
+__device__ __forceinline__ void bn_finish(const BnAcc& a, const BnFinalArgs& f, int c) {
+  const double n = a.n, mean = a.mean, m2 = a.m2;
+  const double var = n > 0 ? m2 / n : 0.0;
+  const float rstd = (float)(1.0 / sqrt(var + (double)f.eps));
+  const float g = f.gamma ? f.gamma[c] : 1.0f;
+  const float bt = f.beta ? f.beta[c] : 0.0f;
+  float sc, sh;
+  bn_affine(g, bt, (float)mean, rstd, sc, sh);
+  if (f.mean_o) f.mean_o[c] = (float)mean;
+  if (f.rstd_o) f.rstd_o[c] = rstd;
+  if (f.scale_o) f.scale_o[c] = sc;
+  if (f.shift_o) f.shift_o[c] = sh;
+  if (f.running_mean)
+    f.running_mean[c] = (1.0f - f.momentum) * f.running_mean[c] + f.momentum * (float)mean;
+  if (f.running_var) {
+    const double unb = n > 1 ? m2 / (n - 1.0) : var;
+    f.running_var[c] = (1.0f - f.momentum) * f.running_var[c] + f.momentum * (float)unb;
+  }
+  if (f.counter && c == 0) *f.counter += 1;
+}
+
+__global__ void bn_partial_kernel(const float* __restrict__ x, float* ws, int B, int C, int L,
+                                  int nsplit, const BnFinalArgs f) {
+  __shared__ float sm[3 * PW_THREADS + 4];
+  const bool FUSED = f.tickets != nullptr;
   const ChanRange cr = chan_range(B, nsplit);
   const int nb = cr.b_end - cr.b_beg;
   const float* base = x + ((size_t)cr.b_beg * C + cr.c) * L;
@@ -117,50 +213,44 @@
   if (threadIdx.x == 0) {
     for (int w = 1; w < PW_THREADS / 64; ++w) chan_combine(n, mean, m2, sm[3 * w], sm[3 * w + 1], sm[3 * w + 2]);
     float* w = ws + ((size_t)blockIdx.y * C + cr.c) * 3;
-    w[0] = n;
-    w[1] = mean;
-    w[2] = m2;
-  }
-}
-
-__device__ __forceinline__ void bn_affine(float gamma, float beta, float mean, float rstd,
-                                          float& scale, float& shift) {
-  scale = gamma * rstd;
-  shift = fmaf(-mean, scale, beta);
-}
-
-__global__ void bn_final_kernel(const float* __restrict__ ws, const float* gamma, const float* beta,
-                                float eps, float momentum, float* running_mean, float* running_var,
-                                float* mean_o, float* rstd_o, float* scale_o, float* shift_o, int C,
+    if (FUSED) {
+      pw_publish(w, n);
+      pw_publish(w + 1, mean);
+      pw_publish(w + 2, m2);
+    } else {
+      w[0] = n;
+      w[1] = mean;
+      w[2] = m2;
+    }
+  }
+  if (FUSED) {
+    __syncthreads();
+    if (!pw_arrive_last(f.tickets + cr.c, nsplit, reinterpret_cast<int*>(sm + 3 * PW_THREADS)))
+      return;
+    BnAcc a = {0.0, 0.0, 0.0};
+    pw_walk_partials<3>(ws, 3, C, cr.c, nsplit, sm, [&](const float* w) { bn_acc_add(a, w); });
+    if (threadIdx.x == 0) bn_finish(a, f, cr.c);
+  }
+}
+
+__global__ void bn_final_kernel(const float* __restrict__ ws, const BnFinalArgs f, int C,
                                 int nsplit) {
   const int c = blockIdx.x * blockDim.x + threadIdx.x;
   if (c >= C) return;
-  double n = 0.0, mean = 0.0, m2 = 0.0;
-  for (int s = 0; s < nsplit; ++s) {
-    const float* w = ws + ((size_t)s * C + c) * 3;
-    const double nb = w[0], mb = w[1], qb = w[2];
-    if (nb <= 0.0) continue;
-    const double tot = n + nb;
-    const double d = mb - mean;
-    mean += d * nb / tot;
-    m2 += qb + d * d * n * nb / tot;
-    n = tot;
-  }
-  const double var = n > 0 ? m2 / n : 0.0;
-  const float rstd = (float)(1.0 / sqrt(var + (double)eps));
-  const float g = gamma ? gamma[c] : 1.0f;
-  const float bt = beta ? beta[c] : 0.0f;
-  float sc, sh;
-  bn_affine(g, bt, (float)mean, rstd, sc, sh);
-  if (mean_o) mean_o[c] = (float)mean;
-  if (rstd_o) rstd_o[c] = rstd;
-  if (scale_o) scale_o[c] = sc;
-  if (shift_o) shift_o[c] = sh;
-  if (running_mean) running_mean[c] = (1.0f - momentum) * running_mean[c] + momentum * (float)mean;
-  if (running_var) {
-    const double unb = n > 1 ? m2 / (n - 1.0) : var;
-    running_var[c] = (1.0f - momentum) * running_var[c] + momentum * (float)unb;
-  }
+  BnAcc a = {0.0, 0.0, 0.0};
+  for (int s = 0; s < nsplit; ++s) bn_acc_add(a, ws + ((size_t)s * C + c) * 3);
+  bn_finish(a, f, c);
+}
+
+static BnFinalArgs bn_final_args(const float* gamma, const float* beta, float eps, float momentum,
+                                 float* running_mean, float* running_var, float* mean, float* rstd,
+                                 float* scale, float* shift) {
+  BnFinalArgs f;
+  f.gamma = gamma; f.beta = beta; f.eps = eps; f.momentum = momentum;
+  f.running_mean = running_mean; f.running_var = running_var;
+  f.mean_o = mean; f.rstd_o = rstd; f.scale_o = scale; f.shift_o = shift;
+  f.counter = nullptr; f.tickets = nullptr;
+  return f;
 }
 
 extern "C" int segan_bn_stats(const float* x, const float* gamma, const float* beta, float eps,
@@ -171,18 +261,39 @@
   SEGAN_REQUIRE(B > 0 && C > 0 && L > 0, "bn_stats: bad sizes");
   hipStream_t st = (hipStream_t)stream;
   const int ns = pw_nsplit(B, C, L);
-  hipLaunchKernelGGL(bn_partial_kernel, dim3(C, ns), dim3(PW_THREADS), 0, st, x, ws, B, C, L, ns);
-  hipLaunchKernelGGL(bn_final_kernel, dim3(ceil_div(C, 64)), dim3(64), 0, st, ws, gamma, beta, eps,
-                     momentum, running_mean, running_var, mean, rstd, scale, shift, C, ns);
+  const BnFinalArgs f = bn_final_args(gamma, beta, eps, momentum, running_mean, running_var, mean,
+                                      rstd, scale, shift);
+  hipLaunchKernelGGL(bn_partial_kernel, dim3(C, ns), dim3(PW_THREADS), 0, st, x, ws, B, C, L,
+                     ns, f);
+  hipLaunchKernelGGL(bn_final_kernel, dim3(ceil_div(C, 64)), dim3(64), 0, st, ws, f, C, ns);
   return segan_check_launch("bn_stats");
+}
+
+extern "C" int segan_bn_stats_fused(const float* x, const float* gamma, const float* beta, float eps,
+                                    float momentum, float* running_mean, float* running_var,
+                                    int64_t* num_batches_tracked, float* mean, float* rstd,
+                                    float* scale, float* shift, float* ws, int* tickets, int B,
+                                    int C, int L, void* stream) {
+  SEGAN_REQUIRE(x && ws && tickets, "bn_stats_fused: NULL pointer");
+  SEGAN_REQUIRE(B > 0 && C > 0 && L > 0, "bn_stats_fused: bad sizes");
+  SEGAN_REQUIRE(C <= PW_MAX_TICKETS, "bn_stats_fused: more than %d channels", PW_MAX_TICKETS);
+  const int ns = pw_nsplit(B, C, L);
+  BnFinalArgs f = bn_final_args(gamma, beta, eps, momentum, running_mean, running_var, mean, rstd,
+                                scale, shift);
+  f.counter = (long long*)num_batches_tracked;
+  f.tickets = tickets;
+  hipLaunchKernelGGL(bn_partial_kernel, dim3(C, ns), dim3(PW_THREADS), 0, (hipStream_t)stream,
+                     x, ws, B, C, L, ns, f);
+  return segan_check_launch("bn_stats_fused");
 }
 
 extern "C" int segan_bn_partial(const float* x, float* ws, int B, int C, int L, void* stream) {
   SEGAN_REQUIRE(x && ws, "bn_partial: NULL pointer");
   SEGAN_REQUIRE(B > 0 && C > 0 && L > 0, "bn_partial: bad sizes");
   const int ns = pw_nsplit(B, C, L);
-  hipLaunchKernelGGL(bn_partial_kernel, dim3(C, ns), dim3(PW_THREADS), 0, (hipStream_t)stream, x, ws,
-                     B, C, L, ns);
+  hipLaunchKernelGGL(bn_partial_kernel, dim3(C, ns), dim3(PW_THREADS), 0, (hipStream_t)stream,
+                     x, ws, B, C, L, ns, bn_final_args(nullptr, nullptr, 0.f, 0.f, nullptr, nullptr, nullptr,
+                                                       nullptr, nullptr, nullptr));
   return segan_check_launch("bn_partial");
 }
 
@@ -192,7 +303,8 @@
                               float* shift, int C, void* stream) {
   SEGAN_REQUIRE(ws && nsplit_total > 0 && C > 0, "bn_final: bad arguments");
   hipLaunchKernelGGL(bn_final_kernel, dim3(ceil_div(C, 64)), dim3(64), 0, (hipStream_t)stream, ws,
-                     gamma, beta, eps, momentum, running_mean, running_var, mean, rstd, scale, shift,
+                     bn_final_args(gamma, beta, eps, momentum, running_mean, running_var, mean, rstd,
+                                   scale, shift),
                      C, nsplit_total);
   return segan_check_launch("bn_final");
 }
@@ -302,9 +414,45 @@
   float inv_count;
 };
 
+struct ActFinalArgs {
+  float* dslope;
+  float* dalpha;
+  float* dgamma;
+  float* dbeta;
+  float* dbias;
+  int* tickets;
+};
+struct ActAcc {
+  float s0, s1, s2;
+};
+__device__ __forceinline__ void act_acc_add(ActAcc& a, const float* w) {
+  a.s0 += w[0];
+  a.s1 += w[1];
+  a.s2 += w[2];
+}
 template <int PHASE>
-__global__ void act_bwd_kernel(const ActBwdArgs p) {
-  __shared__ float sm[16];
+__device__ __forceinline__ void act_finish(const ActAcc& a, const ActBwdArgs& p,
+                                           const ActFinalArgs& f, int c) {
+  if (PHASE == 0) {
+    if (f.dslope) f.dslope[c] += a.s0;
+    if (f.dalpha) f.dalpha[c] += a.s1;
+    if (f.dbias) f.dbias[c] += a.s2;
+  } else if (PHASE == 1) {
+    if (f.dslope) f.dslope[c] += a.s0;
+    if (f.dbeta) f.dbeta[c] += a.s1;
+    if (f.dgamma) f.dgamma[c] += a.s2;
+    float* tot = p.ws + (size_t)p.nsplit * p.C * 4 + (size_t)c * 2;
+    tot[0] = a.s1;
+    tot[1] = a.s2;
+  } else {
+    if (f.dbias) f.dbias[c] += a.s0;
+  }
+}
+
+template <int PHASE>
+__global__ void act_bwd_kernel(const ActBwdArgs p, const ActFinalArgs f) {
+  __shared__ float sm[3 * PW_THREADS + 4];
+  const bool FUSED = f.tickets != nullptr;
   const ChanRange cr = chan_range(p.B, p.nsplit);
   const int c = cr.c;
   const int nb = cr.b_end - cr.b_beg;
@@ -383,51 +531,47 @@
   block_sum<3>(r, sm);
   if (threadIdx.x == 0) {
     float* w = p.ws + ((size_t)blockIdx.y * p.C + c) * 4;
-    w[0] = r[0];
-    w[1] = r[1];
-    w[2] = r[2];
+    if (FUSED) {
+      pw_publish(w, r[0]);
+      pw_publish(w + 1, r[1]);
+      pw_publish(w + 2, r[2]);
+    } else {
+      w[0] = r[0];
+      w[1] = r[1];
+      w[2] = r[2];
+    }
+  }
+  if (FUSED) {
+    if (!pw_arrive_last(f.tickets + c, p.nsplit, reinterpret_cast<int*>(sm + 3 * PW_THREADS)))
+      return;
+    ActAcc a = {0.f, 0.f, 0.f};
+    pw_walk_partials<3>(p.ws, 4, p.C, c, p.nsplit, sm, [&](const float* w) { act_acc_add(a, w); });
+    if (threadIdx.x == 0) act_finish<PHASE>(a, p, f, c);
   }
 }
 
 template <int PHASE>
-__global__ void act_bwd_final_kernel(const ActBwdArgs p, float* dslope, float* dalpha,
-                                     float* dgamma, float* dbeta, float* dbias) {
+__global__ void act_bwd_final_kernel(const ActBwdArgs p, const ActFinalArgs f) {
   const int c = blockIdx.x * blockDim.x + threadIdx.x;
   if (c >= p.C) return;
-  float s0 = 0.f, s1 = 0.f, s2 = 0.f;
-  for (int s = 0; s < p.nsplit; ++s) {
-    const float* w = p.ws + ((size_t)s * p.C + c) * 4;
-    s0 += w[0];
-    s1 += w[1];
-    s2 += w[2];
-  }
-  if (PHASE == 0) {
-    if (dslope) dslope[c] += s0;
-    if (dalpha) dalpha[c] += s1;
-    if (dbias) dbias[c] += s2;
-  } else if (PHASE == 1) {
-    if (dslope) dslope[c] += s0;
-    if (dbeta) dbeta[c] += s1;
-    if (dgamma) dgamma[c] += s2;
-    float* tot = p.ws + (size_t)p.nsplit * p.C * 4 + (size_t)c * 2;
-    tot[0] = s1;
-    tot[1] = s2;
-  } else {
-    if (dbias) dbias[c] += s0;
-  }
-}
-
-extern "C" int segan_act_bwd(const float* a, const float* dh, const float* dskip,
-                             const float* slope, const float* alpha, const float* bn_mean,
-                             const float* bn_rstd, const float* bn_gamma, const float* bn_beta,
-                             float* da, float* dslope, float* dalpha, float* dgamma, float* dbeta,
-                             float* dbias, float* ws, int B, int C, int L, void* stream) {
-  SEGAN_REQUIRE(a && da && ws, "act_bwd: NULL pointer");
-  SEGAN_REQUIRE(dh || dskip, "act_bwd: no incoming gradient");
-  SEGAN_REQUIRE(B > 0 && C > 0 && L > 0, "act_bwd: bad sizes");
-  SEGAN_REQUIRE((bn_mean == nullptr) == (bn_rstd == nullptr), "act_bwd: mean/rstd must pair");
-  SEGAN_REQUIRE(!(dskip && !alpha), "act_bwd: dskip needs alpha");
-  SEGAN_REQUIRE(!(bn_mean && dskip), "act_bwd: BN layers have no skip tap");
+  ActAcc a = {0.f, 0.f, 0.f};
+  for (int s = 0; s < p.nsplit; ++s) act_acc_add(a, p.ws + ((size_t)s * p.C + c) * 4);
+  act_finish<PHASE>(a, p, f, c);
+}
+
+static int act_bwd_launch(const char* what, const float* a, const float* dh, const float* dskip,
+                          const float* slope, const float* alpha, const float* bn_mean,
+                          const float* bn_rstd, const float* bn_gamma, const float* bn_beta,
+                          float* da, float* dslope, float* dalpha, float* dgamma, float* dbeta,
+                          float* dbias, float* ws, int* tickets, int B, int C, int L,
+                          void* stream) {
+  SEGAN_REQUIRE(a && da && ws, "%s: NULL pointer", what);
+  SEGAN_REQUIRE(dh || dskip, "%s: no incoming gradient", what);
+  SEGAN_REQUIRE(B > 0 && C > 0 && L > 0, "%s: bad sizes", what);
+  SEGAN_REQUIRE((bn_mean == nullptr) == (bn_rstd == nullptr), "%s: mean/rstd must pair", what);
+  SEGAN_REQUIRE(!(dskip && !alpha), "%s: dskip needs alpha", what);
+  SEGAN_REQUIRE(!(bn_mean && dskip), "%s: BN layers have no skip tap", what);
+  SEGAN_REQUIRE(!tickets || C <= PW_MAX_TICKETS, "%s: more than %d channels", what, PW_MAX_TICKETS);
   hipStream_t st = (hipStream_t)stream;
   ActBwdArgs p;
   p.a = a; p.dh = dh; p.dskip = dskip; p.slope = slope; p.alpha = alpha;
@@ -435,20 +579,48 @@
   p.da = da; p.ws = ws; p.B = B; p.C = C; p.L = L;
   p.nsplit = pw_nsplit(B, C, L);
   p.inv_count = 1.0f / ((float)B * (float)L);
+  ActFinalArgs f;
+  f.dslope = dslope; f.dalpha = dalpha; f.dgamma = dgamma; f.dbeta = dbeta; f.dbias = dbias;
+  f.tickets = tickets;
   const dim3 grid(C, p.nsplit), fgrid(ceil_div(C, 64));
-  if (!bn_mean) {
-    hipLaunchKernelGGL(act_bwd_kernel<0>, grid, dim3(PW_THREADS), 0, st, p);
-    hipLaunchKernelGGL(act_bwd_final_kernel<0>, fgrid, dim3(64), 0, st, p, dslope, dalpha, dgamma,
-                       dbeta, dbias);
+  if (tickets) {
+    if (!bn_mean) {
+      hipLaunchKernelGGL(act_bwd_kernel<0>, grid, dim3(PW_THREADS), 0, st, p, f);
+    } else {
+      hipLaunchKernelGGL(act_bwd_kernel<1>, grid, dim3(PW_THREADS), 0, st, p, f);
+      hipLaunchKernelGGL(act_bwd_kernel<2>, grid, dim3(PW_THREADS), 0, st, p, f);
+    }
+  } else if (!bn_mean) {
+    hipLaunchKernelGGL(act_bwd_kernel<0>, grid, dim3(PW_THREADS), 0, st, p, f);
+    hipLaunchKernelGGL(act_bwd_final_kernel<0>, fgrid, dim3(64), 0, st, p, f);
   } else {
-    hipLaunchKernelGGL(act_bwd_kernel<1>, grid, dim3(PW_THREADS), 0, st, p);
-    hipLaunchKernelGGL(act_bwd_final_kernel<1>, fgrid, dim3(64), 0, st, p, dslope, dalpha, dgamma,
-                       dbeta, dbias);
-    hipLaunchKernelGGL(act_bwd_kernel<2>, grid, dim3(PW_THREADS), 0, st, p);
-    hipLaunchKernelGGL(act_bwd_final_kernel<2>, fgrid, dim3(64), 0, st, p, dslope, dalpha, dgamma,
-                       dbeta, dbias);
-  }
-  return segan_check_launch("act_bwd");
+    hipLaunchKernelGGL(act_bwd_kernel<1>, grid, dim3(PW_THREADS), 0, st, p, f);
+    hipLaunchKernelGGL(act_bwd_final_kernel<1>, fgrid, dim3(64), 0, st, p, f);
+    hipLaunchKernelGGL(act_bwd_kernel<2>, grid, dim3(PW_THREADS), 0, st, p, f);
+    hipLaunchKernelGGL(act_bwd_final_kernel<2>, fgrid, dim3(64), 0, st, p, f);
+  }
+  return segan_check_launch(what);
+}
+
+extern "C" int segan_act_bwd(const float* a, const float* dh, const float* dskip,
+                             const float* slope, const float* alpha, const float* bn_mean,
+                             const float* bn_rstd, const float* bn_gamma, const float* bn_beta,
+                             float* da, float* dslope, float* dalpha, float* dgamma, float* dbeta,
+                             float* dbias, float* ws, int B, int C, int L, void* stream) {
+  return act_bwd_launch("act_bwd", a, dh, dskip, slope, alpha, bn_mean, bn_rstd, bn_gamma, bn_beta,
+                        da, dslope, dalpha, dgamma, dbeta, dbias, ws, nullptr, B, C, L, stream);
+}
+
+extern "C" int segan_act_bwd_fused(const float* a, const float* dh, const float* dskip,
+                                   const float* slope, const float* alpha, const float* bn_mean,
+                                   const float* bn_rstd, const float* bn_gamma,
+                                   const float* bn_beta, float* da, float* dslope, float* dalpha,
+                                   float* dgamma, float* dbeta, float* dbias, float* ws,
+                                   int* tickets, int B, int C, int L, void* stream) {
+  SEGAN_REQUIRE(tickets, "act_bwd_fused: NULL tickets");
+  return act_bwd_launch("act_bwd_fused", a, dh, dskip, slope, alpha, bn_mean, bn_rstd, bn_gamma,
+                        bn_beta, da, dslope, dalpha, dgamma, dbeta, dbias, ws, tickets, B, C, L,
+                        stream);
 }
 
 extern "C" int segan_act_bwd_bn_reduce(const float* a, const float* dh, const float* slope,
@@ -465,9 +637,9 @@
   p.da = nullptr; p.ws = ws; p.B = B; p.C = C; p.L = L;
   p.nsplit = pw_nsplit(B, C, L);
   p.inv_count = 1.0f / ((float)B * (float)L);
-  hipLaunchKernelGGL(act_bwd_kernel<1>, dim3(C, p.nsplit), dim3(PW_THREADS), 0, st, p);
-  hipLaunchKernelGGL(act_bwd_final_kernel<1>, dim3(ceil_div(C, 64)), dim3(64), 0, st, p, dslope,
-                     (float*)nullptr, dgamma, dbeta, (float*)nullptr);
+  ActFinalArgs f = {dslope, nullptr, dgamma, dbeta, nullptr, nullptr};
+  hipLaunchKernelGGL(act_bwd_kernel<1>, dim3(C, p.nsplit), dim3(PW_THREADS), 0, st, p, f);
+  hipLaunchKernelGGL(act_bwd_final_kernel<1>, dim3(ceil_div(C, 64)), dim3(64), 0, st, p, f);
   if (hipMemcpyAsync(totals, ws + (size_t)p.nsplit * C * 4, (size_t)C * 2 * sizeof(float),
                      hipMemcpyDeviceToDevice, st) != hipSuccess) {
     segan_set_error("act_bwd_bn_reduce: copy of the totals failed");
@@ -495,9 +667,9 @@
     segan_set_error("act_bwd_bn_apply: copy of the totals failed");
     return SEGAN_ELAUNCH;
   }
-  hipLaunchKernelGGL(act_bwd_kernel<2>, dim3(C, p.nsplit), dim3(PW_THREADS), 0, st, p);
-  hipLaunchKernelGGL(act_bwd_final_kernel<2>, dim3(ceil_div(C, 64)), dim3(64), 0, st, p,
-                     (float*)nullptr, (float*)nullptr, (float*)nullptr, (float*)nullptr, dbias);
+  ActFinalArgs f = {nullptr, nullptr, nullptr, nullptr, dbias, nullptr};
+  hipLaunchKernelGGL(act_bwd_kernel<2>, dim3(C, p.nsplit), dim3(PW_THREADS), 0, st, p, f);
+  hipLaunchKernelGGL(act_bwd_final_kernel<2>, dim3(ceil_div(C, 64)), dim3(64), 0, st, p, f);
   return segan_check_launch("act_bwd_bn_apply");
 }
 
diff --git a/segan_pytorch_amd/functional.py b/segan_pytorch_amd/functional.py
--- a/segan_pytorch_amd/functional.py
+++ b/segan_pytorch_amd/functional.py
@@ -29,13 +29,22 @@
     fn = sdist.bn_stats_sync if sdist.sync_bn_enabled() else ops.bn_stats
     track = training and bn.running_mean is not None and bn.running_var is not None
     momentum = 0.0
+    counter = None
     if track:
-        if bn.num_batches_tracked is not None:
-            bn.num_batches_tracked += 1
         if bn.momentum is not None:
             momentum = bn.momentum
+            if bn.num_batches_tracked is not None:
+                if fn is ops.bn_stats and bn.num_batches_tracked.is_cuda:
+                    counter = bn.num_batches_tracked
+                else:
+                    bn.num_batches_tracked += 1
         else:
+            if bn.num_batches_tracked is not None:
+                bn.num_batches_tracked += 1
             momentum = 1.0 / float(bn.num_batches_tracked) if bn.num_batches_tracked is not None else 0.0
+    if counter is not None:
+        return fn(c, bn.weight, bn.bias, bn.eps, momentum, bn.running_mean, bn.running_var,
+                  counter=counter)
     return fn(c, bn.weight, bn.bias, bn.eps, momentum, bn.running_mean if track else None,
               bn.running_var if track else None)
 
@@ -136,8 +145,19 @@
     sdist.grad_ready(*ps)
 
 
+_const_vecs = {}
+
+
+def _const_vec(n, fill, device):
+    key = (int(n), float(fill), str(device))
+    v = _const_vecs.get(key)
+    if v is None:
+        v = _const_vecs[key] = torch.full((int(n),), float(fill), device=device, dtype=torch.float32)
+    return v
+
+
 def _ones(n, ref):
-    return torch.ones(n, device=ref.device, dtype=torch.float32)
+    return _const_vec(n, 1.0, ref.device)
 
 
 def _cat(a, b):
@@ -227,8 +247,7 @@
         return None
     parts = []
     for v, n in ((v0, n0), (v1, n1)):
-        parts.append(v.detach().reshape(-1) if v is not None else
-                     torch.full((n,), fill, device=ref.device, dtype=torch.float32))
+        parts.append(v.detach().reshape(-1) if v is not None else _const_vec(n, fill, ref.device))
     return torch.cat(parts)
 
 
diff --git a/segan_pytorch_amd/ops.py b/segan_pytorch_amd/ops.py
--- a/segan_pytorch_amd/ops.py
+++ b/segan_pytorch_amd/ops.py
@@ -1,5 +1,6 @@
 import ctypes
 import operator
+import weakref
 
 import torch
 
@@ -168,13 +169,27 @@
     return buf
 
 
+_tickets = {}
+MAX_TICKETS = 16384
+
+
+def _ticket_words():
+    dev = torch._C._cuda_getDevice()
+    key = (dev, torch._C._cuda_getCurrentRawStream(dev))
+    buf = _tickets.get(key)
+    if buf is None:
+        buf = torch.zeros(MAX_TICKETS, device=torch.device('cuda', dev), dtype=torch.int32)
+        _tickets[key] = buf
+    return ctypes.c_void_p(buf.data_ptr())
+
+
 def set_reserved_slots(n):
     return int(_lib.load().segan_set_reserved_slots(int(n)))
 
 
 def release_scratch(device=None):
     dev = None if device is None else torch.device(device).index
-    for d in (_corr_scratch, _call_scratch):
+    for d in (_corr_scratch, _call_scratch, _tickets):
         for key in [k for k in d if dev is None or k[0] == dev]:
             del d[key]
 
@@ -212,11 +227,22 @@
         p._segan_epoch = getattr(p, '_segan_epoch', 0) + 1
 
 
+_pack_launches = 0
+
+
 class WeightPack(object):
 
     def __init__(self):
         self._buf = {}
         self._key = {}
+
+    def _note(self, w):
+        global _pack_launches
+        _pack_launches += 1
+        reg = getattr(w, '_segan_packs', None)
+        if reg is None:
+            reg = w._segan_packs = weakref.WeakSet()
+        reg.add(self)
 
     def _get(self, w, S, pad_t, want):
         _chk(w, 'weight', 3)
@@ -237,6 +263,7 @@
                                      _stream()), 'pack_weights')
         self._buf[want] = buf
         self._key[want] = key
+        self._note(w)
         return buf
 
     def f(self, w, S):
@@ -259,6 +286,7 @@
         check(lib.segan_pack_weights_g(_ptr(w), _ptr(buf), M, N, K, S, _stream()), 'pack_weights_g')
         self._buf['g'] = buf
         self._key['g'] = key
+        self._note(w)
         return buf
 
     def t(self, w, S, pad_t):
@@ -284,6 +312,104 @@
         self._buf[want] = buf
         self._key[want] = key
         return buf
+
+
+_PACK_FORMS = {'f': _lib.PACK_F, 't': _lib.PACK_T, 'g': _lib.PACK_G}
+
+
+def pack_table_records(entries):
+    recs = (_lib.SeganPackRec * len(entries))()
+    for r, (w_ptr, dst_ptr, form, M, N, K, S, pad_t) in zip(recs, entries):
+        r.w, r.dst, r.form = w_ptr, dst_ptr, _PACK_FORMS[form]
+        r.M, r.N, r.K, r.S, r.pad_t = M, N, K, S, pad_t
+    nblocks = _lib.load().segan_pack_table_plan(recs, len(entries))
+    check(min(nblocks, 0), 'pack_table_plan')
+    return recs, nblocks
+
+
+class PackTable(object):
+
+    def __init__(self):
+        self._ident = None
+        self._dev = None
+        self._n = self._nblocks = 0
+        self._recs = None
+        self._seen_launches = -1
+
+    @staticmethod
+    def collect(params, prev_epochs):
+        out = []
+        for p, ep in zip(params, prev_epochs):
+            if p.dim() != 3:
+                continue
+            for pack in getattr(p, '_segan_packs', ()):
+                for want, key in pack._key.items():
+                    if want not in _PACK_FORMS:
+                        continue
+                    if key[:5] != (p.data_ptr(), p._version, _weights_epoch, ep, tuple(p.shape)):
+                        continue
+                    out.append((pack, want, p, key[5], key[6] if want == 't' else 0))
+        return out
+
+    def _steady(self):
+        if self._recs is None or self._seen_launches != _pack_launches:
+            return False
+        for pack, want, w, _tail, key in self._recs:
+            if pack._key.get(want) is not key or key[0] != w.data_ptr() or key[1] != w._version \
+                    or key[2] != _weights_epoch:
+                return False
+        return True
+
+    def _launch_and_rekey(self):
+        check(_lib.load().segan_pack_table(_ptr(self._dev), self._n, self._nblocks, _stream()),
+              'pack_table')
+        for rec in self._recs:
+            pack, want, w, tail, key = rec
+            rec[4] = pack._key[want] = (key[0], key[1], key[2], w._segan_epoch) + tail
+
+    def refresh(self, params, prev_epochs):
+        if self._steady():
+            self._launch_and_rekey()
+            return self._n
+        self._recs = None
+        live = self.collect(params, prev_epochs)
+        if not live:
+            return 0
+        entries = [(w.data_ptr(), pack._buf[want].data_ptr(), want) + tuple(w.shape) + (S, pad_t)
+                   for pack, want, w, S, pad_t in live]
+        ident = (tuple(entries), live[0][2].device)
+        if ident != self._ident:
+            recs, nblocks = pack_table_records(entries)
+            host = torch.frombuffer(bytearray(bytes(recs)), dtype=torch.uint8)
+            self._dev = host.to(live[0][2].device)
+            self._ident, self._n, self._nblocks = ident, len(entries), nblocks
+        self._recs = [[pack, want, w, (tuple(w.shape), S) if want == 'g' else (tuple(w.shape), S, pad_t),
+                       (w.data_ptr(), w._version, _weights_epoch)]
+                      for pack, want, w, S, pad_t in live]
+        self._launch_and_rekey()
+        self._seen_launches = _pack_launches
+        return len(live)
+
+
+def step_weights_changed(params, table=None):
+    prev = [getattr(p, '_segan_epoch', 0) for p in params]
+    bump_weights_epoch(params)
+    if table is not None and _tail_fusion:
+        return table.refresh(params, prev)
+    return 0
+
+
+_tail_fusion = True
+
+
+def set_step_tail_fusion(on):
+    global _tail_fusion
+    prev, _tail_fusion = _tail_fusion, bool(on)
+    return prev
+
+
+def get_step_tail_fusion():
+    return _tail_fusion
 
 
 def conv1d_fwd(src, w, bias, S, roll=0, pad_mode=PAD_REFLECT, padL=None, pack=None):
@@ -472,7 +598,7 @@
     return torch.empty((per_split * ns * C + extra * C,), device=device, dtype=torch.float32)
 
 
-def bn_stats(x, gamma, beta, eps, momentum, running_mean, running_var):
+def bn_stats(x, gamma, beta, eps, momentum, running_mean, running_var, counter=None, fused=None):
     _chk(x, 'x', 3)
     B, C, L = x.shape
     mean = torch.empty(C, device=x.device, dtype=torch.float32)
@@ -480,6 +606,19 @@
     scale = torch.empty_like(mean)
     shift = torch.empty_like(mean)
     ws = _ws(B, C, L, 3, 0, x.device)
+    if fused is None:
+        fused = _tail_fusion
+    if fused and C <= MAX_TICKETS:
+        if counter is not None and (counter.dtype != torch.int64 or not counter.is_cuda
+                                    or counter.numel() != 1):
+            raise TypeError('bn_stats: counter must be one int64 on the device')
+        check(_lib.load().segan_bn_stats_fused(
+            _ptr(x), _ptr(gamma), _ptr(beta), eps, momentum, _ptr(running_mean), _ptr(running_var),
+            _ptr(counter), _ptr(mean), _ptr(rstd), _ptr(scale), _ptr(shift), _ptr(ws),
+            _ticket_words(), B, C, L, _stream()), 'bn_stats_fused')
+        return mean, rstd, scale, shift
+    if counter is not None:
+        counter += 1
     check(_lib.load().segan_bn_stats(_ptr(x), _ptr(gamma), _ptr(beta), eps, momentum,
                                      _ptr(running_mean), _ptr(running_var), _ptr(mean), _ptr(rstd),
                                      _ptr(scale), _ptr(shift), _ptr(ws), B, C, L, _stream()),
@@ -577,7 +716,7 @@
 
 
 def act_bwd(a, dh, dskip=None, slope=None, alpha=None, bn=None, dslope=None, dalpha=None,
-            dgamma=None, dbeta=None, dbias=None):
+            dgamma=None, dbeta=None, dbias=None, fused=None):
     _chk(a, 'a', 3)
     B, C, L = a.shape
     da = torch.empty_like(a)
@@ -585,6 +724,15 @@
     mean = rstd = gamma = beta = None
     if bn is not None:
         mean, rstd, gamma, beta = bn
+    if fused is None:
+        fused = _tail_fusion
+    if fused and C <= MAX_TICKETS:
+        check(_lib.load().segan_act_bwd_fused(
+            _ptr(a), _ptr(dh), _ptr(dskip), _ptr(slope), _ptr(alpha), _ptr(mean), _ptr(rstd),
+            _ptr(gamma), _ptr(beta), _ptr(da), _ptr(dslope), _ptr(dalpha), _ptr(dgamma),
+            _ptr(dbeta), _ptr(dbias), _ptr(ws), _ticket_words(), B, C, L, _stream()),
+            'act_bwd_fused')
+        return da
     check(_lib.load().segan_act_bwd(_ptr(a), _ptr(dh), _ptr(dskip), _ptr(slope), _ptr(alpha),
                                     _ptr(mean), _ptr(rstd), _ptr(gamma), _ptr(beta), _ptr(da),
                                     _ptr(dslope), _ptr(dalpha), _ptr(dgamma), _ptr(dbeta),
diff --git a/segan_pytorch_amd/optim.py b/segan_pytorch_amd/optim.py
--- a/segan_pytorch_amd/optim.py
+++ b/segan_pytorch_amd/optim.py
@@ -13,6 +13,7 @@
         self._params = [p for g in self.param_groups for p in g['params']]
         if not self._params:
             raise ValueError('optimizer got an empty parameter list')
+        self._pack_table = ops.PackTable()
         self._build_arenas()
 
     def _build_arenas(self):
@@ -132,7 +133,7 @@
         ops.rmsprop_step(self.flat_param, self.flat_grad, self._flat_state['square_avg'],
                          float(g['lr']), float(g['alpha']), float(g['eps']))
         self._bump_steps()
-        ops.bump_weights_epoch(self._params)
+        ops.step_weights_changed(self._params, self._pack_table)
         return loss
 
 
@@ -163,5 +164,5 @@
                       self._flat_state['exp_avg_sq'], float(g['lr']), float(g['betas'][0]),
                       float(g['betas'][1]), float(g['eps']), self._nsteps)
         self._bump_steps()
-        ops.bump_weights_epoch(self._params)
+        ops.step_weights_changed(self._params, self._pack_table)
         return loss
```

Measured after the change: 3591, median of 6. Within noise of the previous version (+0.4%).
